# bcaitech1/p4-fr-sorry-math-but-love-you

Hardware: NVIDIA B200
Metric: EfficientSATRN greedy-decode images/sec (higher is better)
Workload: dtype bf16

## Files before the change

p4-fr-sorry-math-but-love-you_b200/csrc/common.cuh:

```cuda
#pragma once
#include <cuda_runtime.h>
#include <cuda_bf16.h>
#include <cuda_fp16.h>
#include <stdint.h>

#if defined(__CUDA_ARCH__) && (__CUDA_ARCH__ < 1000)
#error "frx is written for sm_100a (B200) only"
#endif

namespace frx {

enum Act : int { ACT_NONE = 0, ACT_RELU = 1, ACT_SILU = 2, ACT_SIGMOID = 3, ACT_GELU = 4 };

__device__ __forceinline__ float act_apply(float v, int act) {
  switch (act) {
    case ACT_RELU: return fmaxf(v, 0.f);
    case ACT_SILU: return v / (1.f + expf(-v));
    case ACT_SIGMOID: return 1.f / (1.f + expf(-v));
    case ACT_GELU: return 0.5f * v * (1.f + erff(v * 0.70710678118654752440f));
    default: return v;
  }
}

struct SmemOptIn {
  size_t bytes[64] = {};
  template <class Kernel>
  cudaError_t ensure(Kernel kernel, size_t smem, bool always = false) {
    int dev = 0;
    cudaGetDevice(&dev);
    dev &= 63;
    if ((!always && smem <= 48 * 1024) || (bytes[dev] != 0 && smem <= bytes[dev])) return cudaSuccess;
    cudaError_t e = cudaFuncSetAttribute(kernel, cudaFuncAttributeMaxDynamicSharedMemorySize, (int)smem);
    if (e == cudaSuccess) bytes[dev] = smem;
    return e;
  }
};

#ifndef FRX_ENC_FP16
#define FRX_ENC_FP16 1
#endif
#if FRX_ENC_FP16
typedef __half eh_t;
typedef __half2 eh2_t;
#define FRX_EH_PTX "f16"
__device__ __forceinline__ uint32_t eh2_pack(float lo, float hi) {
  uint32_t r;
  asm("cvt.rn.satfinite.f16x2.f32 %0, %1, %2;\n" : "=r"(r) : "f"(hi), "f"(lo));
  return r;
}
__device__ __forceinline__ eh_t eh_from_float(float f) {
  const uint32_t r = eh2_pack(f, 0.f);
  return __ushort_as_half((unsigned short)(r & 0xffffu));
}
__device__ __forceinline__ float eh_to_float(eh_t v) { return __half2float(v); }
__device__ __forceinline__ float2 eh2_unpack(uint32_t w) { return __half22float2(*reinterpret_cast<const __half2*>(&w)); }
#else
typedef __nv_bfloat16 eh_t;
typedef __nv_bfloat162 eh2_t;
#define FRX_EH_PTX "bf16"
__device__ __forceinline__ uint32_t eh2_pack(float lo, float hi) {
  __nv_bfloat162 t = __floats2bfloat162_rn(lo, hi);
  return *reinterpret_cast<uint32_t*>(&t);
}
__device__ __forceinline__ eh_t eh_from_float(float f) { return __float2bfloat16_rn(f); }
__device__ __forceinline__ float eh_to_float(eh_t v) { return __bfloat162float(v); }
__device__ __forceinline__ float2 eh2_unpack(uint32_t w) { return make_float2(__uint_as_float(w << 16), __uint_as_float(w & 0xffff0000u)); }
#endif

__device__ __forceinline__ float warp_sum(float v) {
#pragma unroll
  for (int o = 16; o > 0; o >>= 1) v += __shfl_xor_sync(0xffffffffu, v, o);
  return v;
}
__device__ __forceinline__ float warp_max(float v) {
#pragma unroll
  for (int o = 16; o > 0; o >>= 1) v = fmaxf(v, __shfl_xor_sync(0xffffffffu, v, o));
  return v;
}

struct GemmP {
  const float* A;
  const float* W;
  float* C;
  int M, N, K;
  int lda, ldc;
  int conv;
  int H, Wd, Cin, OH, OW, KH, KW, stride, pad_t, pad_l;
  const float* gate;
  int rows_per_img;
  const float* scale;
  const float* shift;
  int act;
  const float* res;
  int ldr;
  float* ws;
  long long ws_floats;
  int splitk, k_chunk;
};

struct DwP {
  const float* in;
  const float* w;
  const float* scale;
  const float* shift;
  float* out;
  int B, H, Wd, C, OH, OW, stride, pad_t, pad_l, act;
};

struct Seg {
  int n_begin, n_end;
  float* dst;
  long long row_stride;
  long long slot_stride;
};

struct DecGemmP {
  const float* A;
  const float* Wt;
  const float* bias;
// ... 108 lines not shown
```

p4-fr-sorry-math-but-love-you_b200/csrc/kernels_bf16.cu:

```cuda
#include <cuda_fp16.h>

#include "common.cuh"
#include "kernels.h"

#ifndef FRX_DW_ACC32
#define FRX_DW_ACC32 2
#endif

namespace frx {

namespace {
__device__ __forceinline__ void unpack8(const uint4& u, float (&f)[8]) {
  const uint32_t w[4] = {u.x, u.y, u.z, u.w};
#pragma unroll
  for (int i = 0; i < 4; ++i) {
    const float2 t = eh2_unpack(w[i]);
    f[2 * i] = t.x;
    f[2 * i + 1] = t.y;
  }
}
__device__ __forceinline__ uint4 pack8(const float (&f)[8]) {
  uint32_t w[4];
#pragma unroll
  for (int i = 0; i < 4; ++i) w[i] = eh2_pack(f[2 * i], f[2 * i + 1]);
  return make_uint4(w[0], w[1], w[2], w[3]);
}
}

__global__ void __launch_bounds__(256) stem_conv_bf16_kernel(const float* __restrict__ in, const float* __restrict__ w,
                                                             const float* __restrict__ scale, const float* __restrict__ shift,
                                                             eh_t* __restrict__ out, int B, int Cin, int H, int W,
                                                             int OH, int OW, int Cout) {
  extern __shared__ float ws[];
  for (int i = threadIdx.x; i < Cout * Cin * 9; i += blockDim.x) ws[i] = w[i];
  float* ssc = ws + Cout * Cin * 9;
  float* ssh = ssc + Cout;
  for (int i = threadIdx.x; i < Cout; i += blockDim.x) { ssc[i] = scale[i]; ssh[i] = shift[i]; }
  __syncthreads();
  const int C8 = Cout / 8;
  long long total = (long long)B * OH * OW * C8;
  long long idx = (long long)blockIdx.x * blockDim.x + threadIdx.x;
  if (idx >= total) return;
  const int co0 = (int)(idx % C8) * 8;
  long long pix = idx / C8;
  const int ow = (int)(pix % OW), oh = (int)((pix / OW) % OH), n = (int)(pix / ((long long)OW * OH));
  float acc[8];
#pragma unroll
  for (int j = 0; j < 8; ++j) acc[j] = 0.f;
  for (int ci = 0; ci < Cin; ++ci) {
    const float* ip = in + (((long long)n * Cin + ci) * H + oh * 2) * W + ow * 2;
    float x[9];
#pragma unroll
    for (int kh = 0; kh < 3; ++kh)
#pragma unroll
      for (int kw = 0; kw < 3; ++kw) x[kh * 3 + kw] = __ldg(ip + kh * W + kw);
#pragma unroll
    for (int j = 0; j < 8; ++j) {
      const float* wp = ws + ((co0 + j) * Cin + ci) * 9;
#pragma unroll
      for (int t = 0; t < 9; ++t) acc[j] = fmaf(x[t], wp[t], acc[j]);
    }
  }
  float o[8];
#pragma unroll
  for (int j = 0; j < 8; ++j) o[j] = act_apply(acc[j] * ssc[co0 + j] + ssh[co0 + j], ACT_SILU);
  *reinterpret_cast<uint4*>(out + pix * Cout + co0) = pack8(o);
}

template <int COUT>
__global__ void __launch_bounds__(128) stem_conv_px_bf16_kernel(const float* __restrict__ in, const float* __restrict__ w,
                                                                const float* __restrict__ scale, const float* __restrict__ shift,
                                                                eh_t* __restrict__ out, int B, int Cin, int H, int W,
                                                                int OH, int OW) {
  extern __shared__ __align__(16) float ws[];
  const int taps = Cin * 9;
  for (int i = threadIdx.x; i < COUT * taps; i += blockDim.x) {
    const int co = i / taps, r = i - co * taps;
    ws[r * COUT + co] = w[i];
  }
  float* ssc = ws + COUT * taps;
  float* ssh = ssc + COUT;
  uint4* stage = reinterpret_cast<uint4*>(ws + ((COUT * taps + 2 * COUT + 3) & ~3));
  for (int i = threadIdx.x; i < COUT; i += blockDim.x) { ssc[i] = scale[i]; ssh[i] = shift[i]; }
  __syncthreads();
  const long long npix = (long long)B * OH * OW, pix0 = (long long)blockIdx.x * blockDim.x;
  const long long pix = min(pix0 + threadIdx.x, npix - 1);
  const int ow = (int)(pix % OW), oh = (int)((pix / OW) % OH), n = (int)(pix / ((long long)OW * OH));
  float acc[COUT];
#pragma unroll
  for (int j = 0; j < COUT; ++j) acc[j] = 0.f;
  for (int ci = 0; ci < Cin; ++ci) {
    const float* ip = in + (((long long)n * Cin + ci) * H + oh * 2) * W + ow * 2;
    float x[9];
#pragma unroll
    for (int kh = 0; kh < 3; ++kh)
#pragma unroll
      for (int kw = 0; kw < 3; ++kw) x[kh * 3 + kw] = __ldg(ip + kh * W + kw);
#pragma unroll
    for (int t = 0; t < 9; ++t) {
      const float4* wp = reinterpret_cast<const float4*>(ws + (ci * 9 + t) * COUT);
#pragma unroll
      for (int j = 0; j < COUT / 4; ++j) {
        const float4 wv = wp[j];
        acc[4 * j] = fmaf(x[t], wv.x, acc[4 * j]);
        acc[4 * j + 1] = fmaf(x[t], wv.y, acc[4 * j + 1]);
        acc[4 * j + 2] = fmaf(x[t], wv.z, acc[4 * j + 2]);
        acc[4 * j + 3] = fmaf(x[t], wv.w, acc[4 * j + 3]);
      }
    }
  }
#pragma unroll
  for (int g = 0; g < COUT / 8; ++g) {
    float o[8];
#pragma unroll
    for (int j = 0; j < 8; ++j) o[j] = act_apply(acc[g * 8 + j] * ssc[g * 8 + j] + ssh[g * 8 + j], ACT_SILU);
    stage[threadIdx.x * (COUT / 8) + g] = pack8(o);
  }
  __syncthreads();
  const long long cta_vecs = min((long long)blockDim.x, npix - pix0) * (COUT / 8);
  uint4* op = reinterpret_cast<uint4*>(out + pix0 * COUT);
  for (int i = threadIdx.x; i < cta_vecs; i += blockDim.x) op[i] = stage[i];
}

void launch_stem_conv_bf16(const float* in, const float* w, const float* scale, const float* shift,
                           eh_t* out, int B, int Cin, int H, int W, int OH, int OW, int Cout, cudaStream_t st) {
  if (Cout == 24) {
    const long long pixels = (long long)B * OH * OW;
    const int smem24 = ((24 * Cin * 9 + 2 * 24 + 3) & ~3) * sizeof(float) + 128 * 3 * 16;
    stem_conv_px_bf16_kernel<24><<<(unsigned)((pixels + 127) / 128), 128, smem24, st>>>(in, w, scale, shift, out, B, Cin, H, W, OH, OW);
    return;
  }
  long long total = (long long)B * OH * OW * (Cout / 8);
  int smem = (Cout * Cin * 9 + 2 * Cout) * sizeof(float);
  stem_conv_bf16_kernel<<<(unsigned)((total + 255) / 256), 256, smem, st>>>(in, w, scale, shift, out, B, Cin, H, W, OH, OW, Cout);
}

__global__ void __launch_bounds__(256) dwconv3x3_bf16_kernel(const eh_t* __restrict__ in, const float* __restrict__ w,
                                                             const float* __restrict__ scale, const float* __restrict__ shift,
                                                             eh_t* __restrict__ out, int B, int H, int W, int C, int OH,
                                                             int OW, int stride, int pad_t, int pad_l, int act) {
  const int C8 = C >> 3;
  long long total = (long long)B * OH * OW * C8;
  long long idx = (long long)blockIdx.x * blockDim.x + threadIdx.x;
  if (idx >= total) return;
  const int c = (int)(idx % C8) * 8;
  long long pix = idx / C8;
  const int ow = (int)(pix % OW), oh = (int)((pix / OW) % OH), n = (int)(pix / ((long long)OW * OH));
  float acc[8];
#pragma unroll
  for (int j = 0; j < 8; ++j) acc[j] = 0.f;
#pragma unroll
  for (int kh = 0; kh < 3; ++kh) {
    const int ih = oh * stride - pad_t + kh;
    if (ih < 0 || ih >= H) continue;
#pragma unroll
    for (int kw = 0; kw < 3; ++kw) {
      const int iw = ow * stride - pad_l + kw;
      if (iw < 0 || iw >= W) continue;
      float x[8];
      unpack8(__ldg(reinterpret_cast<const uint4*>(in + (((long long)n * H + ih) * W + iw) * C + c)), x);
      const float4 w0 = __ldg(reinterpret_cast<const float4*>(w + (kh * 3 + kw) * C + c));
      const float4 w1 = __ldg(reinterpret_cast<const float4*>(w + (kh * 3 + kw) * C + c + 4));
      acc[0] = fmaf(x[0], w0.x, acc[0]); acc[1] = fmaf(x[1], w0.y, acc[1]);
      acc[2] = fmaf(x[2], w0.z, acc[2]); acc[3] = fmaf(x[3], w0.w, acc[3]);
      acc[4] = fmaf(x[4], w1.x, acc[4]); acc[5] = fmaf(x[5], w1.y, acc[5]);
      acc[6] = fmaf(x[6], w1.z, acc[6]); acc[7] = fmaf(x[7], w1.w, acc[7]);
    }
  }
  float o[8];
#pragma unroll
  for (int j = 0; j < 8; ++j) o[j] = act_apply(acc[j] * __ldg(scale + c + j) + __ldg(shift + c + j), act);
  *reinterpret_cast<uint4*>(out + pix * C + c) = pack8(o);
}

void launch_dwconv_bf16(const eh_t* in, const float* w, const float* scale, const float* shift,
                        eh_t* out, int B, int H, int W, int C, int OH, int OW, int stride, int pad_t,
                        int pad_l, int act, cudaStream_t st) {
  long long total = (long long)B * OH * OW * (C / 8);
  dwconv3x3_bf16_kernel<<<(unsigned)((total + 255) / 256), 256, 0, st>>>(in, w, scale, shift, out, B, H, W, C, OH, OW,
                                                                        stride, pad_t, pad_l, act);
}

__global__ void __launch_bounds__(256) se_scale_bf16_kernel(eh_t* __restrict__ x, const float* __restrict__ w1,
                                                            const float* __restrict__ b1, const float* __restrict__ w2,
                                                            const float* __restrict__ b2, int HW, int C, int R) {
  extern __shared__ float sm[];
  float* mean = sm;
  float* red = sm + C;
  float* gate = red + R;
  const int n = blockIdx.x;
  eh_t* xp = x + (long long)n * HW * C;
  const float inv = 1.f / (float)HW;
  for (int c8 = threadIdx.x; c8 < C / 8; c8 += blockDim.x) {
    float s[8];
#pragma unroll
    for (int j = 0; j < 8; ++j) s[j] = 0.f;
    for (int q = 0; q < HW; ++q) {
      float v[8];
      unpack8(*reinterpret_cast<const uint4*>(xp + (long long)q * C + c8 * 8), v);
#pragma unroll
      for (int j = 0; j < 8; ++j) s[j] += v[j];
    }
#pragma unroll
    for (int j = 0; j < 8; ++j) mean[c8 * 8 + j] = s[j] * inv;
  }
  __syncthreads();
  const int warp = threadIdx.x >> 5, lane = threadIdx.x & 31;
  for (int r = warp; r < R; r += 8) {
    float s = 0.f;
    for (int c = lane; c < C; c += 32) s = fmaf(__ldg(w1 + (long long)r * C + c), mean[c], s);
    s = warp_sum(s);
    if (lane == 0) red[r] = act_apply(s + __ldg(b1 + r), ACT_SILU);
  }
  __syncthreads();
  for (int c = threadIdx.x; c < C; c += blockDim.x) {
    float s = __ldg(b2 + c);
    const float* wr = w2 + (long long)c * R;
    for (int r = 0; r < R; ++r) s = fmaf(__ldg(wr + r), red[r], s);
    gate[c] = 1.f / (1.f + expf(-s));
  }
  __syncthreads();
  for (int i = threadIdx.x; i < HW * (C / 8); i += blockDim.x) {
    const int c8 = i % (C / 8);
    uint4* ptr = reinterpret_cast<uint4*>(xp + (long long)(i / (C / 8)) * C + c8 * 8);
    float v[8];
    unpack8(*ptr, v);
#pragma unroll
    for (int j = 0; j < 8; ++j) v[j] *= gate[c8 * 8 + j];
    *ptr = pack8(v);
  }
}

void launch_se_scale_bf16(eh_t* x, const float* w1, const float* b1, const float* w2, const float* b2,
                          int B, int HW, int C, int R, cudaStream_t st) {
  se_scale_bf16_kernel<<<B, 256, (2 * C + R) * sizeof(float), st>>>(x, w1, b1, w2, b2, HW, C, R);
}


__global__ void __launch_bounds__(256) dwconv_se_mean_kernel(const eh_t* __restrict__ in, const float* __restrict__ w,
                                                             const float* __restrict__ scale, const float* __restrict__ shift,
                                                             eh_t* __restrict__ out, float* __restrict__ mean,
                                                             int H, int W, int C, int OH, int OW, int stride, int pad_t,
                                                             int pad_l, const float* __restrict__ se_w1,
                                                             const float* __restrict__ se_w2, int se_floats) {
  extern __shared__ __align__(16) unsigned char dw_smem[];
  {
    const long long line = ((long long)(blockIdx.y * gridDim.x + blockIdx.x) * blockDim.x + threadIdx.x) * 32;
    if (line < se_floats) {
      asm volatile("prefetch.global.L2 [%0];\n" ::"l"(se_w1 + line));
      asm volatile("prefetch.global.L2 [%0];\n" ::"l"(se_w2 + line));
    }
  }
  uint4* tile = reinterpret_cast<uint4*>(dw_smem);
  float (*red)[64 + 1] = reinterpret_cast<float (*)[64 + 1]>(dw_smem + (size_t)H * W * 8 * 16);
  float* wsm = reinterpret_cast<float*>(dw_smem + (size_t)H * W * 8 * 16 + 32 * 65 * sizeof(float));
  const int n = blockIdx.x, c0 = blockIdx.y * 64;
  const int cg = threadIdx.x & 7, pl = threadIdx.x >> 3;
  const int c = c0 + cg * 8;
  const bool c_ok = c < C;
  const eh_t* ip = in + (long long)n * H * W * C;
  for (int i = threadIdx.x; i < H * W * 8; i += 256) {
    const int px = i >> 3, g = i & 7;
    tile[i] = (c0 + g * 8 < C) ? __ldg(reinterpret_cast<const uint4*>(ip + (long long)px * C + c0 + g * 8)) : make_uint4(0u, 0u, 0u, 0u);
  }
  float sum[8];
#pragma unroll
  for (int j = 0; j < 8; ++j) sum[j] = 0.f;
  for (int i = threadIdx.x; i < 11 * 64; i += 256) {
    const int t = i >> 6, cc = c0 + (i & 63);
    const float* src = t < 9 ? w + t * C : (t == 9 ? scale : shift);
    wsm[i] = cc < C ? __ldg(src + cc) : 0.f;
  }
  __syncthreads();
  auto ld8s = [&](int t, float (&dst)[8]) {
    const float4 a = *reinterpret_cast<const float4*>(wsm + t * 64 + cg * 8);
    const float4 b4 = *reinterpret_cast<const float4*>(wsm + t * 64 + cg * 8 + 4);
    dst[0] = a.x; dst[1] = a.y; dst[2] = a.z; dst[3] = a.w; dst[4] = b4.x; dst[5] = b4.y; dst[6] = b4.z; dst[7] = b4.w;
  };
  float sc[8], sh[8];
  ld8s(9, sc);
  ld8s(10, sh);
  eh_t* op = out + (long long)n * OH * OW * C;
  if (c_ok) {
    for (int px = pl; px < OH * OW; px += 32) {
      const int oh = px / OW, ow = px - oh * OW;
      float acc[8];
#pragma unroll
      for (int j = 0; j < 8; ++j) acc[j] = 0.f;
#pragma unroll
      for (int kh = 0; kh < 3; ++kh) {
        const int ih = oh * stride - pad_t + kh;
#pragma unroll
        for (int kw = 0; kw < 3; ++kw) {
          const int iw = ow * stride - pad_l + kw;
          if (ih >= 0 && ih < H && iw >= 0 && iw < W) {
            float x[8], wv[8];
            unpack8(tile[(ih * W + iw) * 8 + cg], x);
            ld8s(kh * 3 + kw, wv);
#pragma unroll
            for (int j = 0; j < 8; ++j) acc[j] = fmaf(x[j], wv[j], acc[j]);
          }
        }
      }
      float o[8];
#pragma unroll
      for (int j = 0; j < 8; ++j) {
        const float v = fmaf(acc[j], sc[j], sh[j]);
        o[j] = __fdividef(v, 1.f + __expf(-v));
      }
      const uint4 packed = pack8(o);
      *reinterpret_cast<uint4*>(op + (long long)px * C + c) = packed;
      float back[8];
      unpack8(packed, back);
#pragma unroll
      for (int j = 0; j < 8; ++j) sum[j] += back[j];
    }
  }
#pragma unroll
  for (int j = 0; j < 8; ++j) red[pl][cg * 8 + j] = sum[j];
  __syncthreads();
  if (threadIdx.x < 64 && c0 + threadIdx.x < C) {
    float s = 0.f;
#pragma unroll
    for (int i = 0; i < 32; ++i) s += red[i][threadIdx.x];
    mean[(long long)n * C + c0 + threadIdx.x] = s / (float)(OH * OW);
  }
}

template <int CH>
__global__ void __launch_bounds__(CH * 4) dwconv4_se_mean_kernel(const eh_t* __restrict__ in, const float* __restrict__ w,
                                                                 const float* __restrict__ scale, const float* __restrict__ shift,
                                                                 eh_t* __restrict__ out, float* __restrict__ mean,
                                                                 int H, int W, int C, int OH, int OW, int stride, int pad_t,
                                                                 int pad_l, const float* __restrict__ se_w1,
                                                                 const float* __restrict__ se_w2, int se_floats) {
  constexpr int NT = CH * 4, G8 = CH / 8, G4 = CH / 4;
  extern __shared__ __align__(16) unsigned char dw_smem[];
  {
    const long long line = ((long long)(blockIdx.y * gridDim.x + blockIdx.x) * NT + threadIdx.x) * 32;
    if (line < se_floats) {
      asm volatile("prefetch.global.L2 [%0];\n" ::"l"(se_w1 + line));
      asm volatile("prefetch.global.L2 [%0];\n" ::"l"(se_w2 + line));
    }
  }
  uint4* tile = reinterpret_cast<uint4*>(dw_smem);
  float (*red)[CH + 1] = reinterpret_cast<float (*)[CH + 1]>(dw_smem + (size_t)H * W * G8 * 16);
  const int n = blockIdx.x, c0 = blockIdx.y * CH;
  const eh_t* ip = in + (long long)n * H * W * C;
  for (int i = threadIdx.x; i < H * W * G8; i += NT) {
    const int px = i / G8, g = i - px * G8;
    uint4 v = make_uint4(0u, 0u, 0u, 0u);
    if (c0 + g * 8 < C) {
#if FRX_ENC_FP16
      v = __ldg(reinterpret_cast<const uint4*>(ip + (long long)px * C + c0 + g * 8));
#else
      float x[8];
      unpack8(__ldg(reinterpret_cast<const uint4*>(ip + (long long)px * C + c0 + g * 8)), x);
      const __half2 h0 = __floats2half2_rn(x[0], x[1]), h1 = __floats2half2_rn(x[2], x[3]);
      const __half2 h2 = __floats2half2_rn(x[4], x[5]), h3 = __floats2half2_rn(x[6], x[7]);
      v = make_uint4(*reinterpret_cast<const uint32_t*>(&h0), *reinterpret_cast<const uint32_t*>(&h1),
                     *reinterpret_cast<const uint32_t*>(&h2), *reinterpret_cast<const uint32_t*>(&h3));
#endif
    }
    tile[i] = v;
  }
  const int cg = threadIdx.x % G4, pl = threadIdx.x / G4;
  const int c = c0 + cg * 4;
  const bool c_ok = c < C;
#if FRX_DW_ACC32
  float4 wt[9], sc, sh;
#if FRX_DW_ACC32 == 2
  __half2 wh[9][2];
#endif
  {
    const float4 z = make_float4(0.f, 0.f, 0.f, 0.f);
#pragma unroll
    for (int t = 0; t < 9; ++t) wt[t] = c_ok ? __ldg(reinterpret_cast<const float4*>(w + t * C + c)) : z;
#if FRX_DW_ACC32 == 2
#pragma unroll
    for (int t = 0; t < 9; ++t) { wh[t][0] = __floats2half2_rn(wt[t].x, wt[t].y); wh[t][1] = __floats2half2_rn(wt[t].z, wt[t].w); }
#endif
    sc = c_ok ? __ldg(reinterpret_cast<const float4*>(scale + c)) : z;
    sh = c_ok ? __ldg(reinterpret_cast<const float4*>(shift + c)) : z;
  }
  __syncthreads();
  const uint2* tile2 = reinterpret_cast<const uint2*>(tile);
  float sum[4] = {0.f, 0.f, 0.f, 0.f};
  eh_t* op = out + (long long)n * OH * OW * C;
  if (c_ok) {
    for (int px = pl; px < OH * OW; px += 16) {
      const int oh = px / OW, ow = px - oh * OW;
      float4 acc = make_float4(0.f, 0.f, 0.f, 0.f);
#pragma unroll
      for (int kh = 0; kh < 3; ++kh) {
        const int ih = oh * stride - pad_t + kh;
#if FRX_DW_ACC32 == 2
        __half2 r0 = __floats2half2_rn(0.f, 0.f), r1 = r0;
#pragma unroll
        for (int kw = 0; kw < 3; ++kw) {
          const int iw = ow * stride - pad_l + kw;
          if (ih >= 0 && ih < H && iw >= 0 && iw < W) {
            const uint2 u = tile2[(ih * W + iw) * G4 + cg];
            r0 = __hfma2(*reinterpret_cast<const __half2*>(&u.x), wh[kh * 3 + kw][0], r0);
            r1 = __hfma2(*reinterpret_cast<const __half2*>(&u.y), wh[kh * 3 + kw][1], r1);
          }
        }
        const float2 a = __half22float2(r0), b = __half22float2(r1);
        acc.x += a.x; acc.y += a.y; acc.z += b.x; acc.w += b.y;
#else
#pragma unroll
        for (int kw = 0; kw < 3; ++kw) {
          const int iw = ow * stride - pad_l + kw;
          if (ih >= 0 && ih < H && iw >= 0 && iw < W) {
            const uint2 u = tile2[(ih * W + iw) * G4 + cg];
            const float2 a = __half22float2(*reinterpret_cast<const __half2*>(&u.x)), b = __half22float2(*reinterpret_cast<const __half2*>(&u.y));
            const float4 ww = wt[kh * 3 + kw];
            acc.x = fmaf(a.x, ww.x, acc.x); acc.y = fmaf(a.y, ww.y, acc.y); acc.z = fmaf(b.x, ww.z, acc.z); acc.w = fmaf(b.y, ww.w, acc.w);
          }
        }
#endif
      }
      float2 f0 = make_float2(fmaf(acc.x, sc.x, sh.x), fmaf(acc.y, sc.y, sh.y)), f1 = make_float2(fmaf(acc.z, sc.z, sh.z), fmaf(acc.w, sc.w, sh.w));
      f0.x = __fdividef(f0.x, 1.f + __expf(-f0.x)); f0.y = __fdividef(f0.y, 1.f + __expf(-f0.y));
      f1.x = __fdividef(f1.x, 1.f + __expf(-f1.x)); f1.y = __fdividef(f1.y, 1.f + __expf(-f1.y));
#else
  __half2 wt[9][2], sc[2], sh[2];
  {
    const float4 z = make_float4(0.f, 0.f, 0.f, 0.f);
#pragma unroll
    for (int t = 0; t < 9; ++t) {
      const float4 f = c_ok ? __ldg(reinterpret_cast<const float4*>(w + t * C + c)) : z;
      wt[t][0] = __floats2half2_rn(f.x, f.y); wt[t][1] = __floats2half2_rn(f.z, f.w);
    }
    const float4 a = c_ok ? __ldg(reinterpret_cast<const float4*>(scale + c)) : z;
    const float4 d = c_ok ? __ldg(reinterpret_cast<const float4*>(shift + c)) : z;
    sc[0] = __floats2half2_rn(a.x, a.y); sc[1] = __floats2half2_rn(a.z, a.w);
    sh[0] = __floats2half2_rn(d.x, d.y); sh[1] = __floats2half2_rn(d.z, d.w);
  }
  const __half2 half_ = __floats2half2_rn(0.5f, 0.5f);
  __syncthreads();
  const uint2* tile2 = reinterpret_cast<const uint2*>(tile);
  float sum[4] = {0.f, 0.f, 0.f, 0.f};
  eh_t* op = out + (long long)n * OH * OW * C;
  if (c_ok) {
    for (int px = pl; px < OH * OW; px += 16) {
      const int oh = px / OW, ow = px - oh * OW;
      __half2 acc0 = __floats2half2_rn(0.f, 0.f), acc1 = acc0;
#pragma unroll
      for (int kh = 0; kh < 3; ++kh) {
        const int ih = oh * stride - pad_t + kh;
#pragma unroll
        for (int kw = 0; kw < 3; ++kw) {
          const int iw = ow * stride - pad_l + kw;
          if (ih >= 0 && ih < H && iw >= 0 && iw < W) {
            const uint2 u = tile2[(ih * W + iw) * G4 + cg];
            acc0 = __hfma2(*reinterpret_cast<const __half2*>(&u.x), wt[kh * 3 + kw][0], acc0);
            acc1 = __hfma2(*reinterpret_cast<const __half2*>(&u.y), wt[kh * 3 + kw][1], acc1);
          }
        }
      }
      const __half2 v0 = __hfma2(acc0, sc[0], sh[0]), v1 = __hfma2(acc1, sc[1], sh[1]);
      const __half2 o0 = __hmul2(v0, __hfma2(h2tanh_approx(__hmul2(v0, half_)), half_, half_));
      const __half2 o1 = __hmul2(v1, __hfma2(h2tanh_approx(__hmul2(v1, half_)), half_, half_));
      const float2 f0 = __half22float2(o0), f1 = __half22float2(o1);
#endif
      uint2 packed;
      packed.x = eh2_pack(f0.x, f0.y);
      packed.y = eh2_pack(f1.x, f1.y);
      *reinterpret_cast<uint2*>(op + (long long)px * C + c) = packed;
      const float2 b0 = eh2_unpack(packed.x), b1 = eh2_unpack(packed.y);
      sum[0] += b0.x; sum[1] += b0.y; sum[2] += b1.x; sum[3] += b1.y;
    }
  }
#pragma unroll
  for (int j = 0; j < 4; ++j) red[pl][cg * 4 + j] = sum[j];
  __syncthreads();
  if (threadIdx.x < CH && c0 + threadIdx.x < C) {
    float s2 = 0.f;
#pragma unroll
    for (int i = 0; i < 16; ++i) s2 += red[i][threadIdx.x];
    mean[(long long)n * C + c0 + threadIdx.x] = s2 / (float)(OH * OW);
  }
}

constexpr int SE_IMGS = 4;
constexpr int SE_ROWS = 4;
__global__ void __launch_bounds__(512, 1) se_fc_kernel(const float* __restrict__ mean, const float* __restrict__ w1,
                                                       const float* __restrict__ b1, const float* __restrict__ w2,
                                                       const float* __restrict__ b2, float* __restrict__ gate, int B, int C,
                                                       int R) {
  extern __shared__ float sm[];
  float* mv = sm;
  float* red = sm + SE_IMGS * C;
  const int n0 = blockIdx.x * SE_IMGS;
  for (int i = threadIdx.x; i < SE_IMGS * C; i += blockDim.x) {
    const int im = i / C;
    mv[i] = n0 + im < B ? mean[(long long)n0 * C + i] : 0.f;
  }
  __syncthreads();
  const int warp = threadIdx.x >> 5, lane = threadIdx.x & 31;
  const int nwarps = blockDim.x >> 5;
  for (int r0 = warp * SE_ROWS; r0 < R; r0 += nwarps * SE_ROWS) {
    float s[SE_ROWS][SE_IMGS];
#pragma unroll
    for (int j = 0; j < SE_ROWS; ++j)
#pragma unroll
      for (int im = 0; im < SE_IMGS; ++im) s[j][im] = 0.f;
#pragma unroll 3
    for (int c4 = lane; c4 < C / 4; c4 += 32) {
      float4 wv[SE_ROWS], m4[SE_IMGS];
#pragma unroll
      for (int j = 0; j < SE_ROWS; ++j)
        wv[j] = r0 + j < R ? __ldg(reinterpret_cast<const float4*>(w1 + (long long)(r0 + j) * C) + c4) : make_float4(0.f, 0.f, 0.f, 0.f);
#pragma unroll
      for (int im = 0; im < SE_IMGS; ++im) m4[im] = *reinterpret_cast<const float4*>(mv + im * C + c4 * 4);
#pragma unroll
      for (int j = 0; j < SE_ROWS; ++j)
#pragma unroll
        for (int im = 0; im < SE_IMGS; ++im)
          s[j][im] = fmaf(wv[j].x, m4[im].x, fmaf(wv[j].y, m4[im].y, fmaf(wv[j].z, m4[im].z, fmaf(wv[j].w, m4[im].w, s[j][im]))));
    }
#pragma unroll
    for (int j = 0; j < SE_ROWS; ++j)
#pragma unroll
      for (int im = 0; im < SE_IMGS; ++im) {
        const float t = warp_sum(s[j][im]);
        if (lane == 0 && r0 + j < R) red[im * R + r0 + j] = act_apply(t + __ldg(b1 + r0 + j), ACT_SILU);
      }
  }
  __syncthreads();
  for (int c = blockIdx.y * blockDim.x + threadIdx.x; c < C; c += gridDim.y * blockDim.x) {
    float s[SE_IMGS];
    const float bb = __ldg(b2 + c);
#pragma unroll
    for (int im = 0; im < SE_IMGS; ++im) s[im] = bb;
#pragma unroll 32
    for (int r = 0; r < R; ++r) {
      const float wv = __ldg(w2 + (long long)r * C + c);
#pragma unroll
      for (int im = 0; im < SE_IMGS; ++im) s[im] = fmaf(wv, red[im * R + r], s[im]);
    }
#pragma unroll
    for (int im = 0; im < SE_IMGS; ++im)
      if (n0 + im < B) gate[(long long)(n0 + im) * C + c] = 1.f / (1.f + expf(-s[im]));
  }
}

__global__ void __launch_bounds__(256) se_apply_kernel(eh_t* __restrict__ x, const float* __restrict__ gate,
                                                       long long total8, int HW, int C) {
  long long i = (long long)blockIdx.x * blockDim.x + threadIdx.x;
  if (i >= total8) return;
  const int C8 = C >> 3;
  const int c = (int)(i % C8) * 8;
  const long long n = i / ((long long)C8 * HW);
  uint4* ptr = reinterpret_cast<uint4*>(x) + i;
  float v[8];
  unpack8(*ptr, v);
  const float4 g0 = __ldg(reinterpret_cast<const float4*>(gate + n * C + c));
  const float4 g1 = __ldg(reinterpret_cast<const float4*>(gate + n * C + c + 4));
  v[0] *= g0.x; v[1] *= g0.y; v[2] *= g0.z; v[3] *= g0.w;
  v[4] *= g1.x; v[5] *= g1.y; v[6] *= g1.z; v[7] *= g1.w;
  *ptr = pack8(v);
}

void launch_mbconv_dw_se_bf16(const eh_t* in, const float* w, const float* scale, const float* shift,
                              eh_t* out, float* mean, float* gate, const float* w1, const float* b1,
                              const float* w2, const float* b2, int B, int H, int W, int C, int OH, int OW, int stride,
                              int pad_t, int pad_l, int R, cudaStream_t st) {
  dim3 g(B, (C + 63) / 64);
  const size_t smem = (size_t)H * W * 8 * 16 + 32 * 65 * sizeof(float) + 11 * 64 * sizeof(float);
  static SmemOptIn opt;
  opt.ensure(dwconv_se_mean_kernel, smem);
  if (C % 8 == 0) {
    constexpr int CH = 32;
    const size_t sm4 = (size_t)H * W * (CH / 8) * 16 + 16 * (CH + 1) * sizeof(float);
    static SmemOptIn opt4;
    opt4.ensure(dwconv4_se_mean_kernel<CH>, sm4);
    dwconv4_se_mean_kernel<CH><<<dim3(B, (C + CH - 1) / CH), CH * 4, sm4, st>>>(in, w, scale, shift, out, mean, H, W, C, OH, OW,
                                                                             stride, pad_t, pad_l, w1, w2, R * C);
  } else {
    dwconv_se_mean_kernel<<<g, 256, smem, st>>>(in, w, scale, shift, out, mean, H, W, C, OH, OW, stride, pad_t, pad_l, w1, w2, R * C);
  }
  se_fc_kernel<<<dim3((B + SE_IMGS - 1) / SE_IMGS, 2), 512, SE_IMGS * (C + R) * sizeof(float), st>>>(mean, w1, b1, w2, b2, gate, B, C, R);
  long long total8 = (long long)B * OH * OW * (C / 8);
  se_apply_kernel<<<(unsigned)((total8 + 255) / 256), 256, 0, st>>>(out, gate, total8, OH * OW, C);
}

__device__ __forceinline__ uint32_t pack2(float lo, float hi) {
  return eh2_pack(lo, hi);
}
__device__ __forceinline__ void mma16816(float (&c)[4], const uint32_t (&a)[4], uint32_t b0, uint32_t b1) {
  asm("mma.sync.aligned.m16n8k16.row.col.f32." FRX_EH_PTX "." FRX_EH_PTX ".f32 {%0,%1,%2,%3}, {%4,%5,%6,%7}, {%8,%9}, {%0,%1,%2,%3};\n"
      : "+f"(c[0]), "+f"(c[1]), "+f"(c[2]), "+f"(c[3])
      : "r"(a[0]), "r"(a[1]), "r"(a[2]), "r"(a[3]), "r"(b0), "r"(b1));
}

template <int S>
__global__ void __launch_bounds__(S * 2) enc_attn_mma_kernel(const float* __restrict__ qkv,
                                                             eh_t* __restrict__ out,
                                                             int D, int heads, float inv_temp) {
  constexpr int HD = 64, NT = S / 8;
  const int b = blockIdx.x / heads, hh = blockIdx.x % heads;
  const int warp = threadIdx.x >> 5, lane = threadIdx.x & 31, gid = lane >> 2, tig = lane & 3;
  const int ld = 3 * D;
  const float* qb = qkv + (long long)b * S * ld + hh * HD;
  const int i0 = warp * 16;
  float sacc[NT][4];
#pragma unroll
  for (int nt = 0; nt < NT; ++nt)
#pragma unroll
    for (int e = 0; e < 4; ++e) sacc[nt][e] = 0.f;
#pragma unroll
  for (int ks = 0; ks < 4; ++ks) {
    const float* q0 = qb + (long long)(i0 + gid) * ld + 16 * ks + 2 * tig;
    const float* q1 = q0 + 8 * ld;
    const float2 a00 = __ldg(reinterpret_cast<const float2*>(q0)), a10 = __ldg(reinterpret_cast<const float2*>(q1));
    const float2 a01 = __ldg(reinterpret_cast<const float2*>(q0 + 8)), a11 = __ldg(reinterpret_cast<const float2*>(q1 + 8));
    const uint32_t a[4] = {pack2(a00.x, a00.y), pack2(a10.x, a10.y), pack2(a01.x, a01.y), pack2(a11.x, a11.y)};
#pragma unroll
    for (int nt = 0; nt < NT; ++nt) {
      const float* kp = qb + D + (long long)(8 * nt + gid) * ld + 16 * ks + 2 * tig;
      const float2 k0 = __ldg(reinterpret_cast<const float2*>(kp)), k1 = __ldg(reinterpret_cast<const float2*>(kp + 8));
      mma16816(sacc[nt], a, pack2(k0.x, k0.y), pack2(k1.x, k1.y));
    }
  }
  float mx0 = -INFINITY, mx1 = -INFINITY;
#pragma unroll
  for (int nt = 0; nt < NT; ++nt) {
#pragma unroll
    for (int e = 0; e < 4; ++e) sacc[nt][e] *= inv_temp;
    mx0 = fmaxf(mx0, fmaxf(sacc[nt][0], sacc[nt][1]));
    mx1 = fmaxf(mx1, fmaxf(sacc[nt][2], sacc[nt][3]));
  }
  mx0 = fmaxf(mx0, __shfl_xor_sync(0xffffffffu, mx0, 1)); mx0 = fmaxf(mx0, __shfl_xor_sync(0xffffffffu, mx0, 2));
  mx1 = fmaxf(mx1, __shfl_xor_sync(0xffffffffu, mx1, 1)); mx1 = fmaxf(mx1, __shfl_xor_sync(0xffffffffu, mx1, 2));
  float sum0 = 0.f, sum1 = 0.f;
#pragma unroll
  for (int nt = 0; nt < NT; ++nt) {
    sacc[nt][0] = __expf(sacc[nt][0] - mx0); sacc[nt][1] = __expf(sacc[nt][1] - mx0);
    sacc[nt][2] = __expf(sacc[nt][2] - mx1); sacc[nt][3] = __expf(sacc[nt][3] - mx1);
    sum0 += sacc[nt][0] + sacc[nt][1];
    sum1 += sacc[nt][2] + sacc[nt][3];
  }
  sum0 += __shfl_xor_sync(0xffffffffu, sum0, 1); sum0 += __shfl_xor_sync(0xffffffffu, sum0, 2);
  sum1 += __shfl_xor_sync(0xffffffffu, sum1, 1); sum1 += __shfl_xor_sync(0xffffffffu, sum1, 2);
  float oacc[8][4];
#pragma unroll
  for (int n = 0; n < 8; ++n)
#pragma unroll
    for (int e = 0; e < 4; ++e) oacc[n][e] = 0.f;
#pragma unroll
  for (int kk = 0; kk < S / 16; ++kk) {
    const uint32_t a[4] = {pack2(sacc[2 * kk][0], sacc[2 * kk][1]), pack2(sacc[2 * kk][2], sacc[2 * kk][3]),
                           pack2(sacc[2 * kk + 1][0], sacc[2 * kk + 1][1]), pack2(sacc[2 * kk + 1][2], sacc[2 * kk + 1][3])};
    const float* vp = qb + 2 * D + (long long)(16 * kk + 2 * tig) * ld + gid;
#pragma unroll
    for (int n = 0; n < 8; ++n) {
      const float v00 = __ldg(vp + 8 * n), v01 = __ldg(vp + ld + 8 * n);
      const float v10 = __ldg(vp + 8 * ld + 8 * n), v11 = __ldg(vp + 9 * ld + 8 * n);
      mma16816(oacc[n], a, pack2(v00, v01), pack2(v10, v11));
    }
  }
  const float r0 = __fdividef(1.f, sum0), r1 = __fdividef(1.f, sum1);
  eh_t* o0 = out + ((long long)b * S + i0 + gid) * D + hh * HD + 2 * tig;
  eh_t* o1 = o0 + (long long)8 * D;
#pragma unroll
  for (int n = 0; n < 8; ++n) {
    *reinterpret_cast<uint32_t*>(o0 + 8 * n) = pack2(oacc[n][0] * r0, oacc[n][1] * r0);
    *reinterpret_cast<uint32_t*>(o1 + 8 * n) = pack2(oacc[n][2] * r1, oacc[n][3] * r1);
  }
}

bool launch_enc_attn_mma_bf16(const float* qkv, eh_t* out, int B, int S, int D, int heads, cudaStream_t st) {
  if (D / heads != 64 || D % heads != 0) return false;
  const float inv_temp = 1.f / sqrtf((float)D);
  if (S == 32) enc_attn_mma_kernel<32><<<B * heads, 64, 0, st>>>(qkv, out, D, heads, inv_temp);
  else if (S == 128) enc_attn_mma_kernel<128><<<B * heads, 256, 0, st>>>(qkv, out, D, heads, inv_temp);
  else return false;
  return true;
}

constexpr int C24 = 24, C24_TH = 8, C24_TW = 32, C24_KS = 14;

__global__ void __launch_bounds__(256) conv3x3_c24_mma_kernel(const eh_t* __restrict__ in, const uint2* __restrict__ wfrag,
                                                              const float* __restrict__ scale, const float* __restrict__ shift,
                                                              eh_t* __restrict__ out, int H, int W, int add_res) {
  constexpr int PW = C24_TW + 2, PH = C24_TH + 2;
  __shared__ __align__(16) eh_t halo[PH * PW * C24];
  __shared__ uint2 wsm[C24_KS * 3 * 32];
  const int tiles_x = (W + C24_TW - 1) / C24_TW, tiles_y = (H + C24_TH - 1) / C24_TH;
  const int n = blockIdx.x / (tiles_x * tiles_y), t = blockIdx.x % (tiles_x * tiles_y);
  const int y0 = (t / tiles_x) * C24_TH, x0 = (t % tiles_x) * C24_TW;
  const eh_t* ip = in + (long long)n * H * W * C24;
  for (int i = threadIdx.x; i < PH * PW * 3; i += 256) {
    const int pix = i / 3, ch = i - pix * 3;
    const int py = pix / PW, px = pix - py * PW;
    const int y = y0 + py - 1, x = x0 + px - 1;
    uint4 v = make_uint4(0u, 0u, 0u, 0u);
    if (y >= 0 && y < H && x >= 0 && x < W) v = __ldg(reinterpret_cast<const uint4*>(ip + ((long long)y * W + x) * C24) + ch);
    reinterpret_cast<uint4*>(halo)[i] = v;
  }
  for (int i = threadIdx.x; i < C24_KS * 3 * 32; i += 256) wsm[i] = __ldg(wfrag + i);
  __syncthreads();
  const int warp = threadIdx.x >> 5, lane = threadIdx.x & 31, gid = lane >> 2, tig = lane & 3;
  float acc[2][3][4];
#pragma unroll
  for (int mt = 0; mt < 2; ++mt)
#pragma unroll
    for (int nt = 0; nt < 3; ++nt)
#pragma unroll
      for (int e = 0; e < 4; ++e) acc[mt][nt][e] = 0.f;
  const uint32_t* hw = reinterpret_cast<const uint32_t*>(halo);
#pragma unroll
  for (int s = 0; s < C24_KS; ++s) {
    const int klo = 16 * s, khi = 16 * s + 8;
    const int tap_lo = klo / C24, ch_lo = klo % C24, tap_hi = khi / C24, ch_hi = khi % C24;
    uint32_t a[2][4];
#pragma unroll
    for (int mt = 0; mt < 2; ++mt) {
      const int px = mt * 16 + gid;
      const int p_lo = ((warp + tap_lo / 3) * PW + px + tap_lo % 3) * 12 + (ch_lo >> 1) + tig;
      a[mt][0] = hw[p_lo];
      a[mt][1] = hw[p_lo + 8 * 12];
      if (tap_hi < 9) {
        const int p_hi = ((warp + tap_hi / 3) * PW + px + tap_hi % 3) * 12 + (ch_hi >> 1) + tig;
        a[mt][2] = hw[p_hi];
        a[mt][3] = hw[p_hi + 8 * 12];
      } else {
        a[mt][2] = 0u; a[mt][3] = 0u;
      }
    }
#pragma unroll
    for (int nt = 0; nt < 3; ++nt) {
      const uint2 b = wsm[(s * 3 + nt) * 32 + lane];
      mma16816(acc[0][nt], a[0], b.x, b.y);
      mma16816(acc[1][nt], a[1], b.x, b.y);
    }
  }
  const int y = y0 + warp;
  if (y >= H) return;
  eh_t* op = out + ((long long)n * H + y) * W * C24;
#pragma unroll
  for (int nt = 0; nt < 3; ++nt) {
    const int ch = nt * 8 + 2 * tig;
    const float s0 = __ldg(scale + ch), s1 = __ldg(scale + ch + 1), h0 = __ldg(shift + ch), h1 = __ldg(shift + ch + 1);
#pragma unroll
    for (int mt = 0; mt < 2; ++mt)
#pragma unroll
      for (int hr = 0; hr < 2; ++hr) {
        const int px = mt * 16 + gid + hr * 8, x = x0 + px;
        if (x >= W) continue;
        float v0 = fmaf(acc[mt][nt][2 * hr], s0, h0), v1 = fmaf(acc[mt][nt][2 * hr + 1], s1, h1);
        v0 = __fdividef(v0, 1.f + __expf(-v0));
        v1 = __fdividef(v1, 1.f + __expf(-v1));
        if (add_res) {
          const uint32_t r = hw[((warp + 1) * PW + px + 1) * 12 + (ch >> 1)];
          const float2 rf = eh2_unpack(r);
          v0 += rf.x;
          v1 += rf.y;
        }
        *reinterpret_cast<uint32_t*>(op + (long long)x * C24 + ch) = pack2(v0, v1);
      }
  }
}

void launch_conv3x3_c24_bf16(const eh_t* in, const void* wfrag, const float* scale, const float* shift,
                             eh_t* out, int B, int H, int W, int add_res, cudaStream_t st) {
  const int tiles = ((W + C24_TW - 1) / C24_TW) * ((H + C24_TH - 1) / C24_TH);
  conv3x3_c24_mma_kernel<<<B * tiles, 256, 0, st>>>(in, reinterpret_cast<const uint2*>(wfrag), scale, shift, out, H, W, add_res);
}

__global__ void __launch_bounds__(256) lite_conv0_pool_bf16_kernel(const float* __restrict__ in, const float* __restrict__ w,
                                                                   const float* __restrict__ scale, const float* __restrict__ shift,
                                                                   eh_t* __restrict__ out, int B, int Cin, int H, int W, int Cout) {
  extern __shared__ float ws0[];
  for (int i = threadIdx.x; i < Cout * Cin * 9; i += blockDim.x) ws0[i] = w[i];
  float* ssc = ws0 + Cout * Cin * 9;
  float* ssh = ssc + Cout;
  for (int i = threadIdx.x; i < Cout; i += blockDim.x) { ssc[i] = scale[i]; ssh[i] = shift[i]; }
  __syncthreads();
  const int OH = H / 2, OW = W / 2, C8 = Cout / 8;
  const long long total = (long long)B * OH * OW * C8;
  const long long idx = (long long)blockIdx.x * blockDim.x + threadIdx.x;
  if (idx >= total) return;
  const int co0 = (int)(idx % C8) * 8;
  const long long pix = idx / C8;
  const int ow = (int)(pix % OW), oh = (int)((pix / OW) % OH), n = (int)(pix / ((long long)OW * OH));
  float acc[4][8];
#pragma unroll
  for (int q = 0; q < 4; ++q)
#pragma unroll
    for (int j = 0; j < 8; ++j) acc[q][j] = 0.f;
  for (int ci = 0; ci < Cin; ++ci) {
    float x[4][4];
#pragma unroll
    for (int a = 0; a < 4; ++a)
#pragma unroll
      for (int b = 0; b < 4; ++b) {
        const int ih = 2 * oh - 1 + a, iw = 2 * ow - 1 + b;
        x[a][b] = (ih >= 0 && ih < H && iw >= 0 && iw < W) ? __ldg(in + (((long long)n * Cin + ci) * H + ih) * W + iw) : 0.f;
      }
#pragma unroll
    for (int j = 0; j < 8; ++j) {
      const float* wp = ws0 + ((co0 + j) * Cin + ci) * 9;
#pragma unroll
      for (int kh = 0; kh < 3; ++kh)
#pragma unroll
        for (int kw = 0; kw < 3; ++kw) {
          const float wv = wp[kh * 3 + kw];
          acc[0][j] = fmaf(x[kh][kw], wv, acc[0][j]);
          acc[1][j] = fmaf(x[kh][kw + 1], wv, acc[1][j]);
          acc[2][j] = fmaf(x[kh + 1][kw], wv, acc[2][j]);
          acc[3][j] = fmaf(x[kh + 1][kw + 1], wv, acc[3][j]);
        }
    }
  }
  float o[8];
#pragma unroll
  for (int j = 0; j < 8; ++j) {
    const float s = ssc[co0 + j], t = ssh[co0 + j];
    const float m = fmaxf(fmaxf(fmaf(acc[0][j], s, t), fmaf(acc[1][j], s, t)), fmaxf(fmaf(acc[2][j], s, t), fmaf(acc[3][j], s, t)));
    o[j] = fmaxf(m, 0.f);
  }
  *reinterpret_cast<uint4*>(out + pix * Cout + co0) = pack8(o);
}

template <int KS, int Cout>
__global__ void __launch_bounds__(256) lite_conv0_pool_mma_kernel(const float* __restrict__ in, const float* __restrict__ w,
                                                                  const float* __restrict__ scale, const float* __restrict__ shift,
                                                                  eh_t* __restrict__ out, int B, int Cin, int H, int W) {
  constexpr int NT = Cout / 8;
  const int lane = threadIdx.x & 31, gid = lane >> 2, tig = lane & 3;
  const int OH = H / 2, OW = W / 2, K = 9 * Cin;
  const long long tiles = (long long)B * OH * (OW / 4);
  const long long tile = (long long)blockIdx.x * 8 + (threadIdx.x >> 5);
  if (tile >= tiles) return;
  uint32_t bf[KS][NT][2];
#pragma unroll
  for (int ks = 0; ks < KS; ++ks)
#pragma unroll
    for (int nt = 0; nt < NT; ++nt)
#pragma unroll
      for (int h2 = 0; h2 < 2; ++h2) {
        const int k = 16 * ks + 8 * h2 + 2 * tig, n = 8 * nt + gid;
        const float lo = k < K ? __ldg(w + (long long)n * K + k) : 0.f, hi = k + 1 < K ? __ldg(w + (long long)n * K + k + 1) : 0.f;
        bf[ks][nt][h2] = pack2(lo, hi);
      }
  const int owq = (int)(tile % (OW / 4));
  const long long t2 = tile / (OW / 4);
  const int oh = (int)(t2 % OH), n = (int)(t2 / OH);
  const int pp = gid & 3, pos0 = gid >> 2;
  const int ow = owq * 4 + pp;
// ... 85 lines not shown
```

p4-fr-sorry-math-but-love-you_b200/csrc/kernels_f32.cu:

```cuda
#include "common.cuh"
#include "kernels.h"

namespace frx {

__global__ void __launch_bounds__(256) stem_conv_kernel(const float* __restrict__ in,
                                                        const float* __restrict__ w,
                                                        const float* __restrict__ scale,
                                                        const float* __restrict__ shift,
                                                        float* __restrict__ out, int B, int Cin, int H,
                                                        int W, int OH, int OW, int Cout, int stride, int pad,
                                                        int act) {
  extern __shared__ float ws[];
  for (int i = threadIdx.x; i < Cout * Cin * 9; i += blockDim.x) ws[i] = w[i];
  float* ssc = ws + Cout * Cin * 9;
  float* ssh = ssc + Cout;
  for (int i = threadIdx.x; i < Cout; i += blockDim.x) { ssc[i] = scale[i]; ssh[i] = shift[i]; }
  __syncthreads();
  long long total = (long long)B * OH * OW * Cout;
  long long idx = (long long)blockIdx.x * blockDim.x + threadIdx.x;
  if (idx >= total) return;
  int co = (int)(idx % Cout);
  long long pix = idx / Cout;
  int ow = (int)(pix % OW);
  int oh = (int)((pix / OW) % OH);
// ... 288 lines not shown

__global__ void __launch_bounds__(256) se_gate_f32_kernel(const float* __restrict__ x,
                                                          const float* __restrict__ w1,
                                                          const float* __restrict__ b1,
                                                          const float* __restrict__ w2,
                                                          const float* __restrict__ b2,
                                                          float* __restrict__ gate,
                                                          int HW, int C, int R) {
  extern __shared__ float sm[];
  float* mean = sm;
  float* red = sm + C;
  const int n = blockIdx.x;
  const float* xp = x + (long long)n * HW * C;
  const float inv = 1.f / (float)HW;
  for (int c = threadIdx.x; c < C; c += blockDim.x) {
    float s = 0.f;
    for (int q = 0; q < HW; ++q) s += __ldg(xp + (long long)q * C + c);
    mean[c] = s * inv;
  }
  __syncthreads();
  const int warp = threadIdx.x >> 5, lane = threadIdx.x & 31;
  for (int r = warp; r < R; r += 8) {
    float s = 0.f;
    for (int c = lane; c < C; c += 32) s = fmaf(__ldg(w1 + (long long)r * C + c), mean[c], s);
    s = warp_sum(s);
    if (lane == 0) red[r] = act_apply(s + __ldg(b1 + r), ACT_SILU);
  }
  __syncthreads();
  for (int c = threadIdx.x; c < C; c += blockDim.x) {
    float s = __ldg(b2 + c);
    const float* wr = w2 + (long long)c * R;
    for (int r = 0; r < R; ++r) s = fmaf(__ldg(wr + r), red[r], s);
    gate[(long long)n * C + c] = 1.f / (1.f + expf(-s));
  }
}

void launch_se_gate_f32(const float* x, const float* w1, const float* b1, const float* w2,
                        const float* b2, float* gate, int B, int HW, int C, int R, cudaStream_t st) {
  se_gate_f32_kernel<<<B, 256, (C + R) * sizeof(float), st>>>(x, w1, b1, w2, b2, gate, HW, C, R);
}

__global__ void __launch_bounds__(256) maxpool2_f32_kernel(const float* __restrict__ in,
                                                           float* __restrict__ out, int B, int H, int W,
                                                           int C) {
  const int OH = H / 2, OW = W / 2, C4 = C / 4;
  long long total = (long long)B * OH * OW * C4;
  long long idx = (long long)blockIdx.x * blockDim.x + threadIdx.x;
  if (idx >= total) return;
  int c = (int)(idx % C4) * 4;
  long long pix = idx / C4;
  int ow = (int)(pix % OW);
  int oh = (int)((pix / OW) % OH);
  int n = (int)(pix / ((long long)OW * OH));
  const float* base = in + (((long long)n * H + oh * 2) * W + ow * 2) * C + c;
  float4 a = __ldg(reinterpret_cast<const float4*>(base));
  float4 b = __ldg(reinterpret_cast<const float4*>(base + C));
  float4 d = __ldg(reinterpret_cast<const float4*>(base + (long long)W * C));
  float4 e = __ldg(reinterpret_cast<const float4*>(base + (long long)W * C + C));
  float4 o;
  o.x = fmaxf(fmaxf(a.x, b.x), fmaxf(d.x, e.x));
  o.y = fmaxf(fmaxf(a.y, b.y), fmaxf(d.y, e.y));
  o.z = fmaxf(fmaxf(a.z, b.z), fmaxf(d.z, e.z));
  o.w = fmaxf(fmaxf(a.w, b.w), fmaxf(d.w, e.w));
  *reinterpret_cast<float4*>(out + (((long long)n * OH + oh) * OW + ow) * C + c) = o;
}

void launch_maxpool2_f32(const float* in, float* out, int B, int H, int W, int C, cudaStream_t st) {
  long long total = (long long)B * (H / 2) * (W / 2) * (C / 4);
  maxpool2_f32_kernel<<<(unsigned)((total + 255) / 256), 256, 0, st>>>(in, out, B, H, W, C);
}

__global__ void __launch_bounds__(1024) pe2d_f32_kernel(const float* __restrict__ x,
                                                       const float* __restrict__ w0,
                                                       const float* __restrict__ b0,
                                                       const float* __restrict__ w1,
                                                       const float* __restrict__ b1,
                                                       const float* __restrict__ peh,
                                                       const float* __restrict__ pew,
                                                       float* __restrict__ out, int h, int w, int C) {
  extern __shared__ float sm[];
  float* mean = sm;
  float* hid = sm + C;
  float* g = hid + C / 2;
  const int S = h * w, n = blockIdx.x;
  const float* xp = x + (long long)n * S * C;
  const float inv = 1.f / (float)S;
  for (int c = threadIdx.x; c < C; c += blockDim.x) {
    float s = 0.f;
    for (int q = 0; q < S; ++q) s += __ldg(xp + (long long)q * C + c);
    mean[c] = s * inv;
  }
  __syncthreads();
  const int warp = threadIdx.x >> 5, lane = threadIdx.x & 31;
  const int nwarps = blockDim.x >> 5;
  for (int r = warp; r < C / 2; r += nwarps) {
    float s = 0.f;
    for (int c = lane; c < C; c += 32) s = fmaf(__ldg(w0 + (long long)r * C + c), mean[c], s);
    s = warp_sum(s);
    if (lane == 0) hid[r] = fmaxf(s + __ldg(b0 + r), 0.f);
  }
  __syncthreads();
  for (int r = warp; r < 2 * C; r += nwarps) {
    float s = 0.f;
    for (int c = lane; c < C / 2; c += 32) s = fmaf(__ldg(w1 + (long long)r * (C / 2) + c), hid[c], s);
    s = warp_sum(s);
    if (lane == 0) g[r] = 1.f / (1.f + expf(-(s + __ldg(b1 + r))));
  }
  __syncthreads();
  float* op = out + (long long)n * S * C;
  for (int i = threadIdx.x; i < S * C; i += blockDim.x) {
    int c = i % C, q = i / C;
    int row = q / w, col = q % w;
    float pos = g[c] * __ldg(peh + row * C + c) + g[C + c] * __ldg(pew + col * C + c);
    op[i] = pos + __ldg(xp + i);
  }
}

void launch_pe2d_f32(const float* x, const float* w0, const float* b0, const float* w1, const float* b1,
                     const float* peh, const float* pew, float* out, int B, int h, int w, int C,
                     cudaStream_t st) {
  int smem = (C + C / 2 + 2 * C) * sizeof(float);
  pe2d_f32_kernel<<<B, 1024, smem, st>>>(x, w0, b0, w1, b1, peh, pew, out, h, w, C);
}

__device__ __forceinline__ void store_as(float* p, float v) { *p = v; }
__device__ __forceinline__ void store_as(eh_t* p, float v) { *p = eh_from_float(v); }

template <typename OutT>
__global__ void __launch_bounds__(256) layernorm_f32_generic_kernel(const float* __restrict__ x,
                                                            const float* __restrict__ res,
                                                            const float* __restrict__ gamma,
                                                            const float* __restrict__ beta,
                                                            OutT* __restrict__ out, int M, int C,
                                                            int scramble_S) {
  const int warp = threadIdx.x >> 5, lane = threadIdx.x & 31;
  const int m = blockIdx.x * 8 + warp;
  if (m >= M) return;
  const float* xp = x + (long long)m * C;
  const float* rp = res ? res + (long long)m * C : nullptr;
  float v[64];
  const int per = C / 32;
  float s = 0.f;
#pragma unroll
  for (int i = 0; i < 64; ++i) {
    if (i < per) {
      float t = __ldg(xp + i * 32 + lane);
      if (rp) t += __ldg(rp + i * 32 + lane);
      v[i] = t;
      s += t;
    }
  }
  const float mean = warp_sum(s) / (float)C;
  float q = 0.f;
#pragma unroll
  for (int i = 0; i < 64; ++i)
    if (i < per) { float d = v[i] - mean; q = fmaf(d, d, q); }
  const float rstd = rsqrtf(warp_sum(q) / (float)C + 1e-5f);
#pragma unroll
  for (int i = 0; i < 64; ++i) {
    if (i < per) {
      int ch = i * 32 + lane;
      float o = (v[i] - mean) * rstd * __ldg(gamma + ch) + __ldg(beta + ch);
      if (scramble_S > 0) {
        int b = m / scramble_S, qd = m % scramble_S;
        long long f = (long long)qd * C + ch;
        int pp = (int)(f % scramble_S), cc = (int)(f / scramble_S);
        store_as(out + ((long long)b * scramble_S + pp) * C + cc, o);
      } else {
        store_as(out + (long long)m * C + ch, o);
      }
    }
  }
}

template <typename OutT, int PER>
__global__ void __launch_bounds__(256) layernorm_f32_kernel(const float* __restrict__ x,
                                                            const float* __restrict__ res,
                                                            const float* __restrict__ gamma,
                                                            const float* __restrict__ beta,
                                                            OutT* __restrict__ out, int M, int C,
                                                            int scramble_S) {
  const int warp = threadIdx.x >> 5, lane = threadIdx.x & 31;
  const int m = blockIdx.x * 8 + warp;
  if (m >= M) return;
  const float* xp = x + (long long)m * C;
  const float* rp = res ? res + (long long)m * C : nullptr;
  float v[PER];
  float s = 0.f;
#pragma unroll
  for (int i = 0; i < PER; ++i) {
    float t = __ldg(xp + i * 32 + lane);
    if (rp) t += __ldg(rp + i * 32 + lane);
    v[i] = t;
    s += t;
  }
  const float mean = warp_sum(s) / (float)C;
  float q = 0.f;
#pragma unroll
  for (int i = 0; i < PER; ++i) { float d = v[i] - mean; q = fmaf(d, d, q); }
  const float rstd = rsqrtf(warp_sum(q) / (float)C + 1e-5f);
#pragma unroll
  for (int i = 0; i < PER; ++i) {
    int ch = i * 32 + lane;
    float o = (v[i] - mean) * rstd * __ldg(gamma + ch) + __ldg(beta + ch);
    if (scramble_S > 0) {
      int b = m / scramble_S, qd = m % scramble_S;
      long long f = (long long)qd * C + ch;
      int pp = (int)(f % scramble_S), cc = (int)(f / scramble_S);
      store_as(out + ((long long)b * scramble_S + pp) * C + cc, o);
    } else {
      store_as(out + (long long)m * C + ch, o);
    }
  }
}

template <typename OutT>
static void layernorm_launch(const float* x, const float* res, const float* gamma, const float* beta, OutT* out, int M, int C,
                             int scramble_S, cudaStream_t st) {
  const dim3 g((M + 7) / 8);
  const int per = C / 32;
  if (per <= 4 && per * 32 == C) {
    if (per == 4) layernorm_f32_kernel<OutT, 4><<<g, 256, 0, st>>>(x, res, gamma, beta, out, M, C, scramble_S);
    else if (per == 2) layernorm_f32_kernel<OutT, 2><<<g, 256, 0, st>>>(x, res, gamma, beta, out, M, C, scramble_S);
    else if (per == 1) layernorm_f32_kernel<OutT, 1><<<g, 256, 0, st>>>(x, res, gamma, beta, out, M, C, scramble_S);
    else layernorm_f32_kernel<OutT, 3><<<g, 256, 0, st>>>(x, res, gamma, beta, out, M, C, scramble_S);
  } else if (per == 8) layernorm_f32_kernel<OutT, 8><<<g, 256, 0, st>>>(x, res, gamma, beta, out, M, C, scramble_S);
  else if (per == 16) layernorm_f32_kernel<OutT, 16><<<g, 256, 0, st>>>(x, res, gamma, beta, out, M, C, scramble_S);
  else if (per == 32) layernorm_f32_kernel<OutT, 32><<<g, 256, 0, st>>>(x, res, gamma, beta, out, M, C, scramble_S);
  else if (per == 64) layernorm_f32_kernel<OutT, 64><<<g, 256, 0, st>>>(x, res, gamma, beta, out, M, C, scramble_S);
  else layernorm_f32_generic_kernel<OutT><<<g, 256, 0, st>>>(x, res, gamma, beta, out, M, C, scramble_S);
}

void launch_layernorm_f32(const float* x, const float* res, const float* gamma, const float* beta,
                          float* out, int M, int C, int scramble_S, cudaStream_t st) {
  layernorm_launch<float>(x, res, gamma, beta, out, M, C, scramble_S, st);
}

__global__ void __launch_bounds__(256) layernorm_scramble_bf16_kernel(const float* __restrict__ x, const float* __restrict__ res,
                                                                      const float* __restrict__ gamma,
                                                                      const float* __restrict__ beta,
                                                                      eh_t* __restrict__ out, int S, int C) {
  extern __shared__ eh_t ln_tile[];
  const int b = blockIdx.x, warp = threadIdx.x >> 5, lane = threadIdx.x & 31;
  const int per = C / 32, LD = S + 2;
  for (int qd = warp; qd < S; qd += 8) {
    const float* xp = x + ((long long)b * S + qd) * C;
    const float* rp = res ? res + ((long long)b * S + qd) * C : nullptr;
    float v[16];
    float s = 0.f;
#pragma unroll
    for (int i = 0; i < 16; ++i)
      if (i < per) {
        float t = __ldg(xp + i * 32 + lane);
        if (rp) t += __ldg(rp + i * 32 + lane);
        v[i] = t;
        s += t;
      }
    const float mean = warp_sum(s) / (float)C;
    float q = 0.f;
#pragma unroll
    for (int i = 0; i < 16; ++i)
      if (i < per) { float d = v[i] - mean; q = fmaf(d, d, q); }
    const float rstd = rsqrtf(warp_sum(q) / (float)C + 1e-5f);
#pragma unroll
    for (int i = 0; i < 16; ++i)
      if (i < per) {
        const int ch = i * 32 + lane;
        const int f = qd * C + ch;
        ln_tile[(f / S) * LD + f % S] = eh_from_float((v[i] - mean) * rstd * __ldg(gamma + ch) + __ldg(beta + ch));
      }
  }
  __syncthreads();
  eh_t* op = out + (long long)b * S * C;
  for (int g = threadIdx.x; g < S * C; g += 256) {
    const int pp = g / C, cc = g - pp * C;
    op[g] = ln_tile[cc * LD + pp];
  }
}

void launch_layernorm_bf16out(const float* x, const float* res, const float* gamma, const float* beta,
                              eh_t* out, int M, int C, int scramble_S, cudaStream_t st) {
  const size_t scr_smem = (size_t)C * (scramble_S + 2) * 2;
  static SmemOptIn scr_opt;
  if (scramble_S > 0 && C <= 512 && C % 32 == 0 && M % scramble_S == 0 && scr_smem <= 160 * 1024 &&
      scr_opt.ensure(layernorm_scramble_bf16_kernel, scr_smem) == cudaSuccess) {
    layernorm_scramble_bf16_kernel<<<M / scramble_S, 256, scr_smem, st>>>(x, res, gamma, beta, out,
                                                                                               scramble_S, C);
    return;
  }
  layernorm_launch<eh_t>(x, res, gamma, beta, out, M, C, scramble_S, st);
}

template <typename OutT>
__global__ void __launch_bounds__(128) enc_attn_f32_kernel(const float* __restrict__ qkv,
                                                           OutT* __restrict__ out,
                                                           int S, int D, int heads, float temperature) {
  extern __shared__ float sm[];
  const int HD = D / heads;
  const int LDS_ = HD + 1;
  float* Q = sm;
  float* K = Q + S * LDS_;
  float* V = K + S * LDS_;
  float* P = V + S * LDS_;
  const int b = blockIdx.x / heads, hh = blockIdx.x % heads;
  const float* base = qkv + (long long)b * S * 3 * D + hh * HD;
  for (int i = threadIdx.x; i < S * HD; i += blockDim.x) {
    int r = i / HD, c = i % HD;
    const float* rp = base + (long long)r * 3 * D + c;
    Q[r * LDS_ + c] = __ldg(rp);
    K[r * LDS_ + c] = __ldg(rp + D);
    V[r * LDS_ + c] = __ldg(rp + 2 * D);
  }
  __syncthreads();
  const int warp = threadIdx.x >> 5, lane = threadIdx.x & 31;
  float* Pw = P + warp * S;
  for (int i = warp; i < S; i += 4) {
    float mx = -INFINITY;
    for (int j = lane; j < S; j += 32) {
      float s = 0.f;
      for (int c = 0; c < HD; ++c) s = fmaf(Q[i * LDS_ + c], K[j * LDS_ + c], s);
      s = s / temperature;
      Pw[j] = s;
      mx = fmaxf(mx, s);
    }
    mx = warp_max(mx);
    float sum = 0.f;
    for (int j = lane; j < S; j += 32) {
      float e = expf(Pw[j] - mx);
      Pw[j] = e;
      sum += e;
    }
    sum = warp_sum(sum);
    __syncwarp();
    for (int c = lane; c < HD; c += 32) {
      float acc = 0.f;
      for (int j = 0; j < S; ++j) acc = fmaf(Pw[j] / sum, V[j * LDS_ + c], acc);
      store_as(out + ((long long)b * S + i) * D + hh * HD + c, acc);
    }
    __syncwarp();
  }
}

template <typename OutT>
static void enc_attn_launch(const float* qkv, OutT* out, int B, int S, int D, int heads, cudaStream_t st) {
  int HD = D / heads;
  size_t smem = (size_t)(3 * S * (HD + 1) + 4 * S) * sizeof(float);
  static SmemOptIn opt;
  opt.ensure(enc_attn_f32_kernel<OutT>, smem);
  enc_attn_f32_kernel<OutT><<<B * heads, 128, smem, st>>>(qkv, out, S, D, heads, sqrtf((float)D));
}
void launch_enc_attn_f32(const float* qkv, float* out, int B, int S, int D, int heads, cudaStream_t st) {
  enc_attn_launch<float>(qkv, out, B, S, D, heads, st);
}
void launch_enc_attn_bf16out(const float* qkv, eh_t* out, int B, int S, int D, int heads, cudaStream_t st) {
  enc_attn_launch<eh_t>(qkv, out, B, S, D, heads, st);
}

constexpr int DG_BM = 32, DG_BN = 32, DG_KC = 512;

__global__ void __launch_bounds__(256) dec_gemm_f32_kernel(const DecGemmP p) {
  extern __shared__ __align__(16) float smem_raw[];
  float (*As)[DG_KC + 4] = reinterpret_cast<float (*)[DG_KC + 4]>(smem_raw);
  float (*red)[DG_BM][DG_BN] = reinterpret_cast<float (*)[DG_BM][DG_BN]>(smem_raw);
  static_assert(8 * DG_BM * DG_BN <= DG_BM * (DG_KC + 4), "partials must fit in the A buffer");
  const int tid = threadIdx.x, warp = tid >> 5, lane = tid & 31;
  const int m0 = blockIdx.x * DG_BM, n0 = blockIdx.y * DG_BN;
  const int n = n0 + lane;
  const bool n_ok = n < p.N;
  float acc[DG_BM];
#pragma unroll
// ... 319 lines not shown
```

p4-fr-sorry-math-but-love-you_b200/csrc/kernels_tc.cu:

```cuda
#include <cuda.h>
#include <cuda_fp16.h>
#include <cudaTypedefs.h>

#include <cstdio>
#include <cstdlib>

#include "common.cuh"
#include "kernels.h"

namespace frx {

namespace {

constexpr int TC_BM = 128;
constexpr int TC_BK = 64;
constexpr int TC_STAGES = 3;
constexpr int TC_A_BYTES = TC_BM * TC_BK * 2;

__device__ __forceinline__ uint32_t smem_u32(const void* p) { return (uint32_t)__cvta_generic_to_shared(p); }

__device__ __forceinline__ void cp_async16(uint32_t dst, const void* src, uint32_t src_bytes) {
  asm volatile("cp.async.cg.shared.global [%0], [%1], 16, %2;\n" ::"r"(dst), "l"(src), "r"(src_bytes) : "memory");
}
__device__ __forceinline__ void cp_async_commit() { asm volatile("cp.async.commit_group;\n" ::: "memory"); }
// ... 175 lines not shown
              if (nb + i < p.N) v[i] += __ldg(rp + i);
          }
        } else {
          const eh_t* rp = reinterpret_cast<const eh_t*>(p.res) + (size_t)m * p.ldr + nb;
          if (full) {
            const uint4 r0 = __ldg(reinterpret_cast<const uint4*>(rp)), r1 = __ldg(reinterpret_cast<const uint4*>(rp + 8));
            const uint32_t rw[8] = {r0.x, r0.y, r0.z, r0.w, r1.x, r1.y, r1.z, r1.w};
#pragma unroll
            for (int i = 0; i < 8; ++i) {
              const float2 rf = eh2_unpack(rw[i]);
              v[2 * i] += rf.x;
              v[2 * i + 1] += rf.y;
            }
          } else {
            for (int i = 0; i < 16; ++i)
              if (nb + i < p.N) v[i] += eh_to_float(rp[i]);
          }
        }
      }
      if (p.out_f32) {
        float* cp = reinterpret_cast<float*>(p.C) + (size_t)m * p.ldc + nb;
        if (full && (p.ldc & 7) == 0 && (reinterpret_cast<uintptr_t>(p.C) & 31) == 0) {
#pragma unroll
          for (int i = 0; i < 16; i += 8)
            asm volatile("st.global.v8.f32 [%0], {%1, %2, %3, %4, %5, %6, %7, %8};\n" ::"l"(cp + i), "f"(v[i]), "f"(v[i + 1]),
                         "f"(v[i + 2]), "f"(v[i + 3]), "f"(v[i + 4]), "f"(v[i + 5]), "f"(v[i + 6]), "f"(v[i + 7]) : "memory");
        } else if (full && (p.ldc & 3) == 0) {
#pragma unroll
          for (int i = 0; i < 16; i += 4) *reinterpret_cast<float4*>(cp + i) = make_float4(v[i], v[i + 1], v[i + 2], v[i + 3]);
        } else {
          for (int i = 0; i < 16; ++i)
            if (nb + i < p.N) cp[i] = v[i];
        }
      } else {
        eh_t* cp = reinterpret_cast<eh_t*>(p.C) + (size_t)m * p.ldc + nb;
        if (full && (p.ldc & 7) == 0) {
          uint32_t w[8];
#pragma unroll
          for (int i = 0; i < 8; ++i) w[i] = eh2_pack(v[2 * i], v[2 * i + 1]);
          if ((p.ldc & 15) == 0 && (reinterpret_cast<uintptr_t>(p.C) & 31) == 0) {
            asm volatile("st.global.v8.b32 [%0], {%1, %2, %3, %4, %5, %6, %7, %8};\n" ::"l"(cp), "r"(w[0]), "r"(w[1]), "r"(w[2]),
                         "r"(w[3]), "r"(w[4]), "r"(w[5]), "r"(w[6]), "r"(w[7]) : "memory");
          } else {
            *reinterpret_cast<uint4*>(cp) = make_uint4(w[0], w[1], w[2], w[3]);
            *reinterpret_cast<uint4*>(cp + 8) = make_uint4(w[4], w[5], w[6], w[7]);
          }
        } else {
          for (int i = 0; i < 16; ++i)
            if (nb + i < p.N) cp[i] = eh_from_float(v[i]);
        }
      }
}

template <int NCOLS>
__global__ void __launch_bounds__(256) tc_igemm_kernel(const TcGemmP p) {
  extern __shared__ unsigned char dyn_smem[];
  __shared__ __align__(8) uint64_t mma_done[TC_STAGES];
  __shared__ __align__(8) uint64_t acc_done;
  __shared__ uint32_t tmem_base_s;

  const int tid = threadIdx.x, warp = tid >> 5, lane = tid & 31;
  const int BN = p.BN;
  const uint32_t b_bytes = (uint32_t)BN * (TC_BK * 2);
  const uint32_t stage_bytes = TC_A_BYTES + b_bytes;
  const int NS = p.stages;
  const uint32_t smem0 = (smem_u32(dyn_smem) + 1023u) & ~1023u;
  const int m0 = blockIdx.x * TC_BM, n0 = blockIdx.y * BN;
  const int KB = (p.K + TC_BK - 1) / TC_BK;

  if (warp == 0) {
    asm volatile("tcgen05.alloc.cta_group::1.sync.aligned.shared::cta.b32 [%0], %1;\n" ::"r"(smem_u32(&tmem_base_s)), "n"(NCOLS) : "memory");
    asm volatile("tcgen05.relinquish_alloc_permit.cta_group::1.sync.aligned;\n" ::: "memory");
  }
  if (tid == 32) {
#pragma unroll
    for (int s = 0; s < TC_STAGES; ++s) mbar_init(&mma_done[s], 1);
    mbar_init(&acc_done, 1);
    asm volatile("fence.mbarrier_init.release.cluster;\n" ::: "memory");
  }
  tc_fence_before();
  __syncthreads();
  tc_fence_after();
  const uint32_t tmem = tmem_base_s;

  const int c = tid & 7, rbase = tid >> 3;
  const eh_t* a_ptr[4];
  int a_ih0[4], a_iw0[4];
  bool a_ok[4];
#pragma unroll
  for (int i = 0; i < 4; ++i) {
    const int m = m0 + rbase + 32 * i;
    a_ok[i] = m < p.M;
    a_ih0[i] = a_iw0[i] = 0;
    a_ptr[i] = p.A;
    if (a_ok[i]) {
      if (p.conv) {
        const int ow = m % p.OW;
        const int t = m / p.OW;
        const int oh = t % p.OH;
        const int n = t / p.OH;
        a_ptr[i] = p.A + (size_t)n * p.H * p.Wd * p.Cin;
        a_ih0[i] = oh * p.stride - p.pad_t;
        a_iw0[i] = ow * p.stride - p.pad_l;
      } else {
        a_ptr[i] = p.A + (size_t)m * p.lda;
      }
    }
  }
  const int nb_rows = (BN + 31) / 32;

  auto load_stage = [&](int kb, int stage) {
    const uint32_t sa = smem0 + (uint32_t)stage * stage_bytes;
    const uint32_t sb = sa + TC_A_BYTES;
    const int k = kb * TC_BK + c * 8;
    int tap = 0, ci = k, kh = 0, kw = 0;
    if (p.conv) {
      tap = k / p.Cin;
      ci = k - tap * p.Cin;
      kh = tap / p.KW;
      kw = tap - kh * p.KW;
    }
#pragma unroll
    for (int i = 0; i < 4; ++i) {
      const int row = rbase + 32 * i;
      const uint32_t dst = sa + (uint32_t)(row >> 3) * 1024u + (uint32_t)(row & 7) * 128u + (uint32_t)((c ^ (row & 7)) << 4);
      const eh_t* src = p.A;
      uint32_t bytes = 0;
      if (a_ok[i] && k < p.K) {
        if (p.conv) {
          const int ih = a_ih0[i] + kh, iw = a_iw0[i] + kw;
          if (ih >= 0 && ih < p.H && iw >= 0 && iw < p.Wd) {
            src = a_ptr[i] + ((size_t)ih * p.Wd + iw) * p.Cin + ci;
            bytes = 16;
          }
        } else {
          src = a_ptr[i] + k;
          bytes = 16;
        }
      }
      cp_async16(dst, src, bytes);
    }
    for (int j = 0; j < nb_rows; ++j) {
      const int row = rbase + 32 * j;
      if (row < BN) {
        const uint32_t dst = sb + (uint32_t)(row >> 3) * 1024u + (uint32_t)(row & 7) * 128u + (uint32_t)((c ^ (row & 7)) << 4);
        const int n = n0 + row;
        const bool ok = n < p.N && k < p.K;
        cp_async16(dst, ok ? p.W + (size_t)n * p.ldw + k : p.W, ok ? 16u : 0u);
      }
    }
  };

  for (int s = 0; s < NS - 1; ++s) {
    if (s < KB) load_stage(s, s);
    cp_async_commit();
  }
  const uint32_t idesc = make_idesc(BN);
  for (int kb = 0; kb < KB; ++kb) {
    if (NS == 3) cp_async_wait<1>(); else cp_async_wait<0>();
    asm volatile("fence.proxy.async.shared::cta;\n" ::: "memory");
    __syncthreads();
    const int stage = kb % NS;
    if (tid == 0) {
      tc_fence_after();
      const uint32_t sa = smem0 + (uint32_t)stage * stage_bytes;
      const uint64_t adesc = make_smem_desc(sa), bdesc = make_smem_desc(sa + TC_A_BYTES);
#pragma unroll
      for (int j = 0; j < TC_BK / 16; ++j)
        umma_f16(tmem, adesc + (uint64_t)(2 * j), bdesc + (uint64_t)(2 * j), idesc, (kb | j) ? 1u : 0u);
      umma_commit(&mma_done[stage]);
      if (kb == KB - 1) umma_commit(&acc_done);
    }
    const int nk = kb + NS - 1;
    if (nk < KB) {
      if (kb >= 1) mbar_wait(&mma_done[(kb - 1) % NS], (uint32_t)(((kb - 1) / NS) & 1));
      load_stage(nk, nk % NS);
    }
    cp_async_commit();
  }
  cp_async_wait<0>();
  mbar_wait(&acc_done, 0);
  tc_fence_after();

  {
    const int q = warp & 3;
    const int m = m0 + q * 32 + lane;
    const bool m_ok = m < p.M;
    for (int cc = (warp >> 2); cc * 16 < BN; cc += 2) {
      uint32_t r[16];
      tmem_ld16(tmem + ((uint32_t)(q * 32) << 16) + (uint32_t)(cc * 16), r);
      const int nb = n0 + cc * 16;
      if (m_ok && nb < p.N) epilogue_store16<false>(p, r, m, nb);
    }
  }
  tc_fence_before();
  __syncthreads();
  if (warp == 0) {
    asm volatile("tcgen05.dealloc.cta_group::1.sync.aligned.b32 %0, %1;\n" ::"r"(tmem), "n"(NCOLS) : "memory");
  }
}


constexpr int WS_STAGES = 4;
constexpr int WS_LAG = 2;
constexpr int WS_PROD_WARPS = 8;
constexpr int WS_EPI_WARPS = 8;
constexpr int WS_MMA_WARP = WS_PROD_WARPS + WS_EPI_WARPS;
constexpr int WS_TMA_WARP = WS_MMA_WARP + 1;
constexpr int WS_THREADS = (WS_TMA_WARP + 1) * 32;
constexpr int WS_PROD_THREADS = WS_PROD_WARPS * 32;
constexpr int WS_ROWS_PER_PASS = WS_PROD_THREADS / 8;
constexpr int WS_A_PASSES = TC_BM / WS_ROWS_PER_PASS;

template <int NCOLS, bool GELU>
__global__ void __launch_bounds__(WS_THREADS, NCOLS >= 256 ? 1 : 2) tc_igemm_ws_kernel(const TcGemmP p, const __grid_constant__ CUtensorMap tmA,
                                                                  const __grid_constant__ CUtensorMap tmW) {
  extern __shared__ unsigned char dyn_smem[];
  __shared__ __align__(8) uint64_t full_bar[WS_STAGES], empty_bar[WS_STAGES], acc_full[2], acc_empty[2];
  __shared__ uint32_t tmem_base_s;

  const int tid = threadIdx.x, warp = tid >> 5, lane = tid & 31;
  const int BN = p.BN;
  const uint32_t stage_bytes = TC_A_BYTES + (uint32_t)BN * (TC_BK * 2);
  const uint32_t smem0 = (smem_u32(dyn_smem) + 1023u) & ~1023u;
  const int KB = p.im2col ? p.KW * p.KW : (p.K + TC_BK - 1) / TC_BK;
  const int tiles_n = (p.N + BN - 1) / BN;
  const int tiles_m = (p.M + TC_BM - 1) / TC_BM;
  const int num_tiles = tiles_m * tiles_n;
  const bool gather = p.conv && !p.im2col;

  if (warp == WS_MMA_WARP) {
    asm volatile("tcgen05.alloc.cta_group::1.sync.aligned.shared::cta.b32 [%0], %1;\n" ::"r"(smem_u32(&tmem_base_s)), "n"(NCOLS) : "memory");
    asm volatile("tcgen05.relinquish_alloc_permit.cta_group::1.sync.aligned;\n" ::: "memory");
  }
  if (tid == 0) {
#pragma unroll
    for (int s = 0; s < WS_STAGES; ++s) { mbar_init(&full_bar[s], (gather ? WS_PROD_THREADS : 0) + 1); mbar_init(&empty_bar[s], 1); }
    mbar_init(&acc_full[0], 1); mbar_init(&acc_full[1], 1);
    const int epi_threads = (WS_EPI_WARPS + (gather ? 0 : WS_PROD_WARPS)) * 32;
    mbar_init(&acc_empty[0], epi_threads); mbar_init(&acc_empty[1], epi_threads);
    asm volatile("fence.mbarrier_init.release.cluster;\n" ::: "memory");
  }
  tc_fence_before();
  __syncthreads();
  tc_fence_after();
  const uint32_t tmem = tmem_base_s;

  if (gather ? warp < WS_PROD_WARPS : warp == WS_TMA_WARP) {
    const bool tma_thread = gather ? tid == 0 : lane == 0;
    const uint32_t tma_bytes = (uint32_t)BN * (TC_BK * 2) + (gather ? 0u : (uint32_t)TC_A_BYTES);
    if (!gather && !tma_thread) {
    } else {
    const int c = tid & 7, rbase = tid >> 3;
    int it = 0;
    for (int tile = blockIdx.x; tile < num_tiles; tile += gridDim.x) {
      const int m0 = (tile / tiles_n) * TC_BM, n0 = (tile % tiles_n) * BN;
      const eh_t* a_ptr[WS_A_PASSES];
      int a_ih0[WS_A_PASSES], a_iw0[WS_A_PASSES];
      bool a_ok[WS_A_PASSES];
      int bw = 0, bh = 0, bn = 0;
      if (p.im2col) {
        const int ow = m0 % p.OW, tq = m0 / p.OW;
        bw = ow * p.stride - p.pad_l;
        bh = (tq % p.OH) * p.stride - p.pad_t;
        bn = tq / p.OH;
      }
      if (gather) {
#pragma unroll
        for (int i = 0; i < WS_A_PASSES; ++i) {
          const int m = m0 + rbase + WS_ROWS_PER_PASS * i;
          a_ok[i] = m < p.M;
          a_ih0[i] = a_iw0[i] = 0;
          a_ptr[i] = p.A;
          if (a_ok[i]) {
            const int ow = m % p.OW;
            const int tq = m / p.OW;
            const int oh = tq % p.OH;
            const int n = tq / p.OH;
            a_ptr[i] = p.A + (size_t)n * p.H * p.Wd * p.Cin;
            a_ih0[i] = oh * p.stride - p.pad_t;
            a_iw0[i] = ow * p.stride - p.pad_l;
          }
        }
      }
      for (int kb = 0; kb < KB; ++kb, ++it) {
        const int stage = it % WS_STAGES;
        mbar_wait(&empty_bar[stage], (uint32_t)(((it / WS_STAGES) & 1) ^ 1));
        const uint32_t sa = smem0 + (uint32_t)stage * stage_bytes, sb = sa + TC_A_BYTES;
        if (tma_thread) {
          mbar_arrive_expect_tx(&full_bar[stage], tma_bytes);
          tma_load_2d(sb, &tmW, kb * TC_BK, n0, &full_bar[stage]);
          if (p.im2col) tma_load_im2col(sa, &tmA, 0, bw, bh, bn, (uint16_t)(kb % p.KW), (uint16_t)(kb / p.KW), &full_bar[stage]);
          else if (!p.conv) tma_load_2d(sa, &tmA, kb * TC_BK, m0, &full_bar[stage]);
        }
        if (gather) {
          const int k = kb * TC_BK + c * 8;
          const int tap = k / p.Cin;
          const int ci = k - tap * p.Cin;
          const int kh = tap / p.KW;
          const int kw = tap - kh * p.KW;
#pragma unroll
          for (int i = 0; i < WS_A_PASSES; ++i) {
            const int row = rbase + WS_ROWS_PER_PASS * i;
            const uint32_t dst = sa + (uint32_t)(row >> 3) * 1024u + (uint32_t)(row & 7) * 128u + (uint32_t)((c ^ (row & 7)) << 4);
            const eh_t* src = p.A;
            uint32_t bytes = 0;
            if (a_ok[i] && k < p.K) {
              const int ih = a_ih0[i] + kh, iw = a_iw0[i] + kw;
              if (ih >= 0 && ih < p.H && iw >= 0 && iw < p.Wd) {
                src = a_ptr[i] + ((size_t)ih * p.Wd + iw) * p.Cin + ci;
                bytes = 16;
              }
            }
            cp_async16(dst, src, bytes);
          }
          cp_async_commit();
          if (it >= WS_LAG) {
            cp_async_wait<WS_LAG>();
            asm volatile("fence.proxy.async.shared::cta;\n" ::: "memory");
            mbar_arrive(&full_bar[(it - WS_LAG) % WS_STAGES]);
          }
        }
      }
    }
    if (gather) {
      cp_async_wait<0>();
      asm volatile("fence.proxy.async.shared::cta;\n" ::: "memory");
      for (int j = (it >= WS_LAG ? it - WS_LAG : 0); j < it; ++j) mbar_arrive(&full_bar[j % WS_STAGES]);
    }
    }
  } else if (warp == WS_MMA_WARP) {
    if (lane == 0) {
      const uint32_t idesc = make_idesc(BN);
      int it = 0, ti = 0;
      for (int tile = blockIdx.x; tile < num_tiles; tile += gridDim.x, ++ti) {
        const int a = ti & 1;
        mbar_wait(&acc_empty[a], (uint32_t)(((ti >> 1) & 1) ^ 1));
        tc_fence_after();
        const uint32_t tacc = tmem + (uint32_t)(a * (NCOLS / 2));
        for (int kb = 0; kb < KB; ++kb, ++it) {
          const int stage = it % WS_STAGES;
          mbar_wait(&full_bar[stage], (uint32_t)((it / WS_STAGES) & 1));
          tc_fence_after();
          const uint32_t sa = smem0 + (uint32_t)stage * stage_bytes;
          const uint64_t adesc = make_smem_desc(sa), bdesc = make_smem_desc(sa + TC_A_BYTES);
#pragma unroll
          for (int j = 0; j < TC_BK / 16; ++j)
            umma_f16(tacc, adesc + (uint64_t)(2 * j), bdesc + (uint64_t)(2 * j), idesc, (kb | j) ? 1u : 0u);
          umma_commit(&empty_bar[stage]);
          if (kb == KB - 1) umma_commit(&acc_full[a]);
        }
      }
    }
  } else if (warp < WS_MMA_WARP) {
    const int q = warp & 3;
    const int nsub = (WS_EPI_WARPS + (gather ? 0 : WS_PROD_WARPS)) / 4;
    const int sub = (gather ? warp - WS_PROD_WARPS : warp) >> 2;
    int ti = 0;
    for (int tile = blockIdx.x; tile < num_tiles; tile += gridDim.x, ++ti) {
      const int a = ti & 1;
      const int m0 = (tile / tiles_n) * TC_BM, n0 = (tile % tiles_n) * BN;
      mbar_wait(&acc_full[a], (uint32_t)((ti >> 1) & 1));
      tc_fence_after();
      const int m = m0 + q * 32 + lane;
      const bool m_ok = m < p.M;
      const uint32_t tacc = tmem + (uint32_t)(a * (NCOLS / 2)) + ((uint32_t)(q * 32) << 16);
      for (int cc = sub; cc * 16 < BN; cc += nsub) {
        uint32_t r[16];
        tmem_ld16(tacc + (uint32_t)(cc * 16), r);
        const int nb = n0 + cc * 16;
        if (m_ok && nb < p.N) epilogue_store16<GELU>(p, r, m, nb);
      }
      tc_fence_before();
      mbar_arrive(&acc_empty[a]);
    }
  }
  tc_fence_before();
  __syncthreads();
  if (warp == WS_MMA_WARP) {
    asm volatile("tcgen05.dealloc.cta_group::1.sync.aligned.b32 %0, %1;\n" ::"r"(tmem), "n"(NCOLS) : "memory");
  }
}

static int tc_pick_bn(int N) {
  if (N <= 256) return (N + 15) / 16 * 16;
  for (int bn = 256; bn >= 128; bn -= 16)
    if (N % bn == 0) return bn;
  return 256;
}

template <int NCOLS>
static int tc_launch(const TcGemmP& p, cudaStream_t st) {
  const size_t smem = (size_t)p.stages * (TC_A_BYTES + (size_t)p.BN * TC_BK * 2) + 1024;
  static SmemOptIn opt;
  {
    cudaError_t e = opt.ensure(tc_igemm_kernel<NCOLS>, smem, true);
    if (e != cudaSuccess) return (int)e;
  }
  dim3 grid((p.M + TC_BM - 1) / TC_BM, (p.N + p.BN - 1) / p.BN);
  tc_igemm_kernel<NCOLS><<<grid, 256, smem, st>>>(p);
  return 0;
}

static PFN_cuTensorMapEncodeTiled_v12000 tensor_map_encoder() {
  static PFN_cuTensorMapEncodeTiled_v12000 fn = nullptr;
  if (!fn) {
    void* ptr = nullptr;
    cudaDriverEntryPointQueryResult qres;
    if (cudaGetDriverEntryPoint("cuTensorMapEncodeTiled", &ptr, cudaEnableDefault, &qres) == cudaSuccess &&
        qres == cudaDriverEntryPointSuccess)
      fn = reinterpret_cast<PFN_cuTensorMapEncodeTiled_v12000>(ptr);
  }
  return fn;
}

static int make_tmap_2d(CUtensorMap* tm, const void* base, long long rows, long long cols, long long ld, int box_rows) {
  PFN_cuTensorMapEncodeTiled_v12000 enc = tensor_map_encoder();
  if (!enc) return (int)cudaErrorNotSupported;
  cuuint64_t dims[2] = {(cuuint64_t)cols, (cuuint64_t)rows};
  cuuint64_t strides[1] = {(cuuint64_t)ld * 2};
  cuuint32_t box[2] = {(cuuint32_t)TC_BK, (cuuint32_t)box_rows};
  cuuint32_t estr[2] = {1, 1};
  CUresult r = enc(tm, (FRX_ENC_FP16 ? CU_TENSOR_MAP_DATA_TYPE_FLOAT16 : CU_TENSOR_MAP_DATA_TYPE_BFLOAT16), 2, const_cast<void*>(base), dims, strides, box, estr,
                   CU_TENSOR_MAP_INTERLEAVE_NONE, CU_TENSOR_MAP_SWIZZLE_128B, CU_TENSOR_MAP_L2_PROMOTION_L2_128B,
                   CU_TENSOR_MAP_FLOAT_OOB_FILL_NONE);
  return r == CUDA_SUCCESS ? 0 : (int)cudaErrorInvalidValue;
}

static PFN_cuTensorMapEncodeIm2col_v12000 im2col_map_encoder() {
  static PFN_cuTensorMapEncodeIm2col_v12000 fn = nullptr;
  if (!fn) {
    void* ptr = nullptr;
    cudaDriverEntryPointQueryResult qres;
    if (cudaGetDriverEntryPoint("cuTensorMapEncodeIm2col", &ptr, cudaEnableDefault, &qres) == cudaSuccess &&
        qres == cudaDriverEntryPointSuccess)
      fn = reinterpret_cast<PFN_cuTensorMapEncodeIm2col_v12000>(ptr);
  }
  return fn;
}

static int make_tmap_im2col(CUtensorMap* tm, const TcGemmP& p) {
  PFN_cuTensorMapEncodeIm2col_v12000 enc = im2col_map_encoder();
  if (!enc) return (int)cudaErrorNotSupported;
  const int B = p.M / (p.OH * p.OW), k = p.KW;
  const int pad_r = (p.OW - 1) * p.stride + k - p.Wd - p.pad_l, pad_b = (p.OH - 1) * p.stride + k - p.H - p.pad_t;
  cuuint64_t dims[4] = {(cuuint64_t)p.Cin, (cuuint64_t)p.Wd, (cuuint64_t)p.H, (cuuint64_t)B};
  cuuint64_t strides[3] = {(cuuint64_t)p.Cin * 2, (cuuint64_t)p.Wd * p.Cin * 2, (cuuint64_t)p.H * p.Wd * p.Cin * 2};
  int lower[2] = {-p.pad_l, -p.pad_t};
  int upper[2] = {pad_r - (k - 1), pad_b - (k - 1)};
  cuuint32_t estr[4] = {1, (cuuint32_t)p.stride, (cuuint32_t)p.stride, 1};
  CUresult r = enc(tm, (FRX_ENC_FP16 ? CU_TENSOR_MAP_DATA_TYPE_FLOAT16 : CU_TENSOR_MAP_DATA_TYPE_BFLOAT16), 4, const_cast<eh_t*>(p.A), dims, strides, lower, upper,
                   (cuuint32_t)TC_BK, (cuuint32_t)TC_BM, estr, CU_TENSOR_MAP_INTERLEAVE_NONE, CU_TENSOR_MAP_SWIZZLE_128B,
                   CU_TENSOR_MAP_L2_PROMOTION_L2_128B, CU_TENSOR_MAP_FLOAT_OOB_FILL_NONE);
  return r == CUDA_SUCCESS ? 0 : (int)cudaErrorInvalidValue;
}

template <int NCOLS>
static int tc_launch_ws(const TcGemmP& p_in, int num_sms, cudaStream_t st) {
  TcGemmP p = p_in;
  const size_t smem = (size_t)WS_STAGES * (TC_A_BYTES + (size_t)p.BN * TC_BK * 2) + 1024;
  static SmemOptIn opt, opt_gelu;
  {
    cudaError_t e = opt.ensure(tc_igemm_ws_kernel<NCOLS, false>, smem, true);
    if (e == cudaSuccess) e = opt_gelu.ensure(tc_igemm_ws_kernel<NCOLS, true>, smem, true);
    if (e != cudaSuccess) return (int)e;
  }
  const int tiles = ((p.M + TC_BM - 1) / TC_BM) * ((p.N + p.BN - 1) / p.BN);
  int per_sm = (int)((227 * 1024) / (smem + 2048));
  if (per_sm > 512 / NCOLS) per_sm = 512 / NCOLS;
  if (per_sm > 4) per_sm = 4;
  if (per_sm < 1) per_sm = 1;
  const int grid = tiles < num_sms * per_sm ? tiles : num_sms * per_sm;
  CUtensorMap tmA, tmW;
  int rc;
  p.im2col = 0;
  if (p.conv && p.Wpad && p.Cin <= TC_BK && p.M % (p.OH * p.OW) == 0 && make_tmap_im2col(&tmA, p) == 0) {
    p.im2col = 1;
    rc = make_tmap_2d(&tmW, p.Wpad, p.N, (long long)p.KW * p.KW * TC_BK, (long long)p.KW * p.KW * TC_BK, p.BN);
  } else {
    rc = make_tmap_2d(&tmW, p.W, p.N, p.K, p.ldw, p.BN);
    if (rc) return rc;
    if (!p.conv) rc = make_tmap_2d(&tmA, p.A, p.M, p.K, p.lda, TC_BM);
    else tmA = tmW;
  }
  if (rc) return rc;
  if (getenv("FRX_DEBUG"))
    fprintf(stderr, "[frx] tc gemm M=%d N=%d K=%d BN=%d conv=%d Cin=%d stride=%d -> %s, grid %d\n", p.M, p.N, p.K, p.BN, p.conv,
            p.Cin, p.stride, p.im2col ? "TMA im2col" : (p.conv ? "cp.async gather" : "TMA dense"), grid);
  if (p.act == ACT_GELU) tc_igemm_ws_kernel<NCOLS, true><<<grid, WS_THREADS, smem, st>>>(p, tmA, tmW);
  else tc_igemm_ws_kernel<NCOLS, false><<<grid, WS_THREADS, smem, st>>>(p, tmA, tmW);
  return 0;
}

int launch_tc_igemm_ws(TcGemmP p, int num_sms, cudaStream_t st) {
  if (p.BN == 0) {
    p.BN = tc_pick_bn(p.N);
    const int tiles_m = (p.M + TC_BM - 1) / TC_BM;
    while (p.BN > 64 && p.BN % 32 == 0 && p.N % (p.BN / 2) == 0 && tiles_m * ((p.N + p.BN - 1) / p.BN) < num_sms) p.BN /= 2;
  }
  if (p.BN <= 32) { p.BN = 32; return tc_launch_ws<64>(p, num_sms, st); }
  if (p.BN <= 64) return tc_launch_ws<128>(p, num_sms, st);
  if (p.BN <= 128) return tc_launch_ws<256>(p, num_sms, st);
  return tc_launch_ws<512>(p, num_sms, st);
}

int launch_tc_igemm(TcGemmP p, cudaStream_t st) {
  if (p.act == ACT_GELU) {
    int dev = 0, sms = 148;
    cudaGetDevice(&dev);
    cudaDeviceGetAttribute(&sms, cudaDevAttrMultiProcessorCount, dev);
    return launch_tc_igemm_ws(p, sms, st);
  }
  if (p.BN == 0) p.BN = tc_pick_bn(p.N);
  {
    const int kb = (p.K + TC_BK - 1) / TC_BK;
    const size_t stage = TC_A_BYTES + (size_t)p.BN * TC_BK * 2;
    p.stages = (kb > 3 && 3 * stage <= 72 * 1024) ? 3 : 2;
  }
  if (p.BN <= 32) { p.BN = 32; return tc_launch<32>(p, st); }
  if (p.BN <= 64) return tc_launch<64>(p, st);
  if (p.BN <= 128) return tc_launch<128>(p, st);
  return tc_launch<256>(p, st);
}

__global__ void __launch_bounds__(256) f32_to_h16_kernel(const float* __restrict__ in, eh_t* __restrict__ out, long long n) {
  long long i = ((long long)blockIdx.x * blockDim.x + threadIdx.x) * 4;
  if (i + 3 < n) {
    float4 v = __ldg(reinterpret_cast<const float4*>(in + i));
    *reinterpret_cast<uint2*>(out + i) = make_uint2(eh2_pack(v.x, v.y), eh2_pack(v.z, v.w));
  } else {
    for (; i < n; ++i) out[i] = eh_from_float(in[i]);
  }
}

void launch_f32_to_h16(const float* in, eh_t* out, long long n, cudaStream_t st) {
  f32_to_h16_kernel<<<(unsigned)((n / 4 + 256) / 256), 256, 0, st>>>(in, out, n);
}


__global__ void __launch_bounds__(256) h16_to_f32_kernel(const eh_t* __restrict__ in, float* __restrict__ out, long long n) {
  long long i = (long long)blockIdx.x * blockDim.x + threadIdx.x;
  if (i < n) out[i] = eh_to_float(in[i]);
}
void launch_h16_to_f32(const eh_t* in, float* out, long long n, cudaStream_t st) {
  h16_to_f32_kernel<<<(unsigned)((n + 255) / 256), 256, 0, st>>>(in, out, n);
}


__global__ void __launch_bounds__(256) pad_conv_weights_kernel(const eh_t* __restrict__ in, eh_t* __restrict__ out,
                                                               long long rows, int Cin) {
  long long i = (long long)blockIdx.x * blockDim.x + threadIdx.x;
  if (i >= rows * 64) return;
  const int ci = (int)(i & 63);
  out[i] = ci < Cin ? in[(i >> 6) * Cin + ci] : eh_from_float(0.f);
}
void launch_pad_conv_weights(const eh_t* in, eh_t* out, long long rows, int Cin, cudaStream_t st) {
  pad_conv_weights_kernel<<<(unsigned)((rows * 64 + 255) / 256), 256, 0, st>>>(in, out, rows, Cin);
}

}
```

p4-fr-sorry-math-but-love-you_b200/csrc/runtime.cu:

```cuda
#include <cmath>
#include <cstdarg>
#include <cstdio>
#include <cstring>
#include <map>
#include <string>
#include <vector>

#include "../../include/frx.h"
#include "kernels.h"
#include "runtime.h"

using namespace frx;

static int fail(frx_handle* h, const char* fmt, ...) {
  char buf[1024];
  va_list ap;
  va_start(ap, fmt);
  vsnprintf(buf, sizeof buf, fmt, ap);
  va_end(ap);
  if (h) h->err = buf;
  return 1;
}

#define CK(expr)                                                                          \
// ... 130 lines not shown
    {2, 6, 3, 2, 4, 128, 25}, {2, 9, 3, 1, 6, 160, 25}, {2, 15, 3, 2, 6, 256, 25}};

extern "C" const char* frx_version(void) { return "frx 0.1 sm_100a"; }

extern "C" const char* frx_last_error(const frx_handle* h) { return h ? h->err.c_str() : "null handle"; }

extern "C" int frx_create(const frx_config* cfg, frx_handle** out) {
  if (!cfg || !out) return 1;
  frx_handle* h = new frx_handle();
  h->cfg = *cfg;
  *out = h;
  int ndev = 0;
  cudaError_t e = cudaGetDeviceCount(&ndev);
  if (e != cudaSuccess || ndev == 0)
    return fail(h, "no CUDA device available (%s): frx has no CPU fallback", cudaGetErrorString(e));
  if (cfg->device < 0 || cfg->device >= ndev) return fail(h, "device %d out of range", cfg->device);
  ON_DEVICE(cfg->device);
  cudaDeviceProp prop;
  CK(cudaGetDeviceProperties(&prop, cfg->device));
  if (prop.major != 10) return fail(h, "device is sm_%d%d; frx is built for sm_100a (B200) only", prop.major, prop.minor);
  h->num_sms = prop.multiProcessorCount;
  if (cfg->network != FRX_NET_EFFICIENT_SATRN && cfg->network != FRX_NET_LITE_SATRN && cfg->network != FRX_NET_SWIN)
    return fail(h, "unknown network %d", cfg->network);
  if (cfg->network == FRX_NET_SWIN && (cfg->height != 384 || cfg->width != 384 || cfg->in_ch != 3 || cfg->enc_hidden != 1024))
    return fail(h, "SWIN is fixed to Swin-B/384: 384x384x3 input, 1024-wide memory (networks/SWIN.py:1028-1031)");
  if (cfg->dec_hidden % cfg->dec_heads || (cfg->dec_hidden / cfg->dec_heads != 32 && cfg->dec_hidden / cfg->dec_heads != 64))
    return fail(h, "decoder head_dim must be 32 or 64");
  if (cfg->dec_hidden > 512) return fail(h, "decoder hidden_dim > 512 not supported");
  if (cfg->max_batch <= 0 || cfg->max_steps <= 0) return fail(h, "max_batch/max_steps must be positive");
  return 0;
}

extern "C" void frx_destroy(frx_handle* h) {
  if (!h) return;
  DeviceGuard guard;
  guard.enter(h->cfg.device);
  frx_train_destroy(h);
  for (auto& kv : h->graphs) cudaGraphExecDestroy(kv.second.exec);
  for (void* p : h->allocs) cudaFree(p);
  for (auto& kv : h->taps) cudaFree(kv.second.data);
  if (h->ev[0]) for (int i = 0; i < 5; ++i) cudaEventDestroy(h->ev[i]);
  for (auto& sl : h->pipe) {
    if (sl.h2d) { cudaEventDestroy(sl.h2d); cudaEventDestroy(sl.enc); cudaEventDestroy(sl.done); cudaEventDestroy(sl.d2h); }
  }
  if (h->pipe_h2d) { cudaStreamDestroy(h->pipe_h2d); cudaStreamDestroy(h->pipe_d2h); cudaStreamDestroy(h->pipe_enc); }
  delete h;
}

extern "C" int frx_load_tensor(frx_handle* h, const char* name, const void* data, const int64_t* shape,
                               int32_t ndim, int32_t dtype) {
  if (!h || !name || !data) return fail(h, "frx_load_tensor: null argument");
  HostTensor t;
  size_t n = 1;
  for (int i = 0; i < ndim; ++i) { t.shape.push_back(shape[i]); n *= (size_t)shape[i]; }
  if (dtype == FRX_DTYPE_F32) {
    t.f.resize(n);
    CK(cudaMemcpy(t.f.data(), data, n * sizeof(float), cudaMemcpyDefault));
  } else if (dtype == FRX_DTYPE_I64) {
    std::vector<int64_t> tmp(n);
    CK(cudaMemcpy(tmp.data(), data, n * sizeof(int64_t), cudaMemcpyDefault));
    t.f.resize(n);
    for (size_t i = 0; i < n; ++i) t.f[i] = (float)tmp[i];
  } else {
    return fail(h, "frx_load_tensor('%s'): unsupported dtype %d", name, dtype);
  }
  h->raw[name] = std::move(t);
  h->finalized = false;
  return 0;
}

extern "C" int frx_set_option(frx_handle* h, const char* key, int64_t value) {
  if (!h || !key) return 1;
  ON_DEVICE(h->cfg.device);
  std::string k(key);
  if (k == "taps") h->opt_taps = value != 0;
  else if (k == "graphs") h->opt_graphs = value != 0;
  else if (k == "step16") h->opt_step16 = value != 0;
  else if (k == "pipe_enc") h->opt_pipe_enc = value != 0;
  else if (k == "timing") h->opt_timing = value != 0;
  else if (k == "cluster_images") {}
  else if (k == "dec_hpc") h->opt_dec_hpc = (value == 1 || value == 2) ? (int)value : 0;
  else if (k == "conv24") h->opt_conv24 = value != 0;
  else if (k == "enc_fp32") h->opt_enc_fp32 = value != 0;
  else if (k == "tc_ws") h->opt_tc_ws = value != 0;
  else if (k == "train_splitk") h->opt_train_splitk = value != 0;
  else if (k == "tc_im2col") h->opt_tc_im2col = value != 0;
  else if (k == "prof") {
    h->opt_prof = value != 0;
    if (h->opt_prof && !h->prof) { void* p; if (dev_alloc(h, &p, 16 * 8)) return 1; h->prof = (long long*)p; }
  }
  else if (k == "parts") {
    if (h->ws_ready && ((int)value & 3) != h->opt_parts)
      return fail(h, "option 'parts' cannot change after the first frx_finalize_weights (create a new handle)");
    h->opt_parts = (int)value & 3;
    h->finalized = false;
  }
  else return fail(h, "unknown option '%s'", key);
  return 0;
}

extern "C" int64_t frx_launch_count(const frx_handle* h) { return h ? h->launches : 0; }
extern "C" int64_t frx_device_bytes(const frx_handle* h) { return h ? h->device_bytes : 0; }

extern "C" int frx_read_prof(frx_handle* h, int64_t* out16) {
  if (!h || !out16 || !h->prof) return fail(h, "profiling not enabled (frx_set_option(h, \"prof\", 1))");
  ON_DEVICE(h->cfg.device);
  CK(cudaMemcpy(out16, h->prof, 16 * 8, cudaMemcpyDeviceToHost));
  return 0;
}

extern "C" int frx_last_timing(const frx_handle* h, float* ms4) {
  if (!h || !ms4) return 1;
  for (int i = 0; i < 4; ++i) ms4[i] = h->last_ms[i];
  return 0;
}

static int pack_trunk_efficientnet(frx_handle* h, ArenaBuilder& ab) {
  const frx_config& c = h->cfg;
  const std::string e = "encoder.shallow_cnn.";
  const HostTensor* w;
  if (need(h, e + "conv_stem.weight", {24, c.in_ch, 3, 3}, &w)) return 1;
  h->stem_w = ab.add(w->f.data(), w->f.size());
  if (fold_bn(h, ab, e + "bn1", 24, 1e-3f, nullptr, &h->stem_sc, &h->stem_sh)) return 1;
  int cin = 24;
  h->blocks.clear();
  for (int s = 0; s < 6; ++s) {
    for (int r = 0; r < kArch[s][1]; ++r) {
      BlockW b{};
      b.kind = kArch[s][0];
      b.k = kArch[s][2];
      b.stride = r == 0 ? kArch[s][3] : 1;
      b.cin = cin;
      b.cout = kArch[s][5];
      b.mid = cin * kArch[s][4];
      b.se_r = cin * kArch[s][6] / 100;
      b.residual = (b.cin == b.cout && b.stride == 1);
      std::string p = e + "eff_block." + std::to_string(s) + "." + std::to_string(r);
      b.name = "eff_block." + std::to_string(s) + "." + std::to_string(r);
      if (b.kind == 0) {
        if (pack_conv(h, ab, p + ".conv.weight", b.cout, b.cin, b.k, &b.w_a)) return 1;
        if (fold_bn(h, ab, p + ".bn1", b.cout, 1e-3f, nullptr, &b.sc_a, &b.sh_a)) return 1;
      } else if (b.kind == 1) {
        if (pack_conv(h, ab, p + ".conv_exp.weight", b.mid, b.cin, b.k, &b.w_a)) return 1;
        if (fold_bn(h, ab, p + ".bn1", b.mid, 1e-3f, nullptr, &b.sc_a, &b.sh_a)) return 1;
        if (pack_conv(h, ab, p + ".conv_pwl.weight", b.cout, b.mid, 1, &b.w_b)) return 1;
        if (fold_bn(h, ab, p + ".bn2", b.cout, 1e-3f, nullptr, &b.sc_b, &b.sh_b)) return 1;
      } else {
        if (pack_conv(h, ab, p + ".conv_pw.weight", b.mid, b.cin, 1, &b.w_a)) return 1;
        if (fold_bn(h, ab, p + ".bn1", b.mid, 1e-3f, nullptr, &b.sc_a, &b.sh_a)) return 1;
        if (pack_dw(h, ab, p + ".conv_dw.weight", b.mid, &b.w_dw)) return 1;
        if (fold_bn(h, ab, p + ".bn2", b.mid, 1e-3f, nullptr, &b.sc_dw, &b.sh_dw)) return 1;
        const HostTensor *w1, *b1, *w2, *b2;
        if (need(h, p + ".se.conv_reduce.weight", {b.se_r, b.mid, 1, 1}, &w1) ||
            need(h, p + ".se.conv_reduce.bias", {b.se_r}, &b1) ||
            need(h, p + ".se.conv_expand.weight", {b.mid, b.se_r, 1, 1}, &w2) ||
            need(h, p + ".se.conv_expand.bias", {b.mid}, &b2))
          return 1;
        b.se_w1 = ab.add(w1->f.data(), w1->f.size());
        b.se_b1 = ab.add(b1->f.data(), b1->f.size());
        b.se_w2 = ab.add(w2->f.data(), w2->f.size());
        b.se_w2t = ab.add(nullptr, w2->f.size());
        for (int cc = 0; cc < b.mid; ++cc)
          for (int rr = 0; rr < b.se_r; ++rr) ab.at(b.se_w2t)[(size_t)rr * b.mid + cc] = w2->f[(size_t)cc * b.se_r + rr];
        b.se_b2 = ab.add(b2->f.data(), b2->f.size());
        if (pack_conv(h, ab, p + ".conv_pwl.weight", b.cout, b.mid, 1, &b.w_b)) return 1;
        if (fold_bn(h, ab, p + ".bn3", b.cout, 1e-3f, nullptr, &b.sc_b, &b.sh_b)) return 1;
      }
      h->blocks.push_back(b);
      cin = b.cout;
    }
  }
  if (pack_conv(h, ab, e + "conv_last.weight", c.enc_hidden, 256, 1, &h->last_w)) return 1;
  if (fold_bn(h, ab, e + "bn2", c.enc_hidden, 1e-5f, nullptr, &h->last_sc, &h->last_sh)) return 1;
  return 0;
}

static int pack_trunk_lite(frx_handle* h, ArenaBuilder& ab) {
  const frx_config& c = h->cfg;
  const std::string e = "encoder.shallow_cnn.";
  int H = c.enc_hidden;
// ... 438 lines not shown
      cudaFree(h->arena);
      h->device_bytes -= (int64_t)h->arena_bytes;
      h->arena = nullptr;
    }
    void* p;
    if (dev_alloc(h, &p, bytes)) return 1;
    h->arena = (float*)p;
    h->arena_bytes = bytes;
  }
  CK(cudaMemcpy(h->arena, ab.host.data(), bytes, cudaMemcpyHostToDevice));

  if (!h->ws_ready) {
    const size_t B = c.max_batch;
    size_t act_max = 0, mid_max = 0;
    if (c.network == FRX_NET_EFFICIENT_SATRN) {
      int H = (c.height - 3) / 2 + 1, W = (c.width - 3) / 2 + 1;
      act_max = (size_t)H * W * 24;
      for (const BlockW& b : h->blocks) {
        int OH, OW, pl;
        same_pad(H, b.k, b.stride, &OH, &pl);
        same_pad(W, b.k, b.stride, &OW, &pl);
        size_t mid = b.kind == 1 ? (size_t)OH * OW * b.mid : (b.kind == 2 ? (size_t)H * W * b.mid : 0);
        if (mid > mid_max) mid_max = mid;
        H = OH; W = OW;
        if ((size_t)H * W * b.cout > act_max) act_max = (size_t)H * W * b.cout;
      }
    } else {
      act_max = (size_t)c.height * c.width * (c.enc_hidden / 2);
      mid_max = act_max;
    }
    size_t S = (size_t)h->feat_h * h->feat_w, C = c.enc_hidden;
    size_t enc_act = S * 3 * C;
    if (enc_act > mid_max) mid_max = enc_act;
    if (S * C > act_max) act_max = S * C;
    void* p;
    if (want_enc && c.network == FRX_NET_SWIN) {
      const size_t tok = 96 * 96;
      for (int i = 0; i < 2; ++i) { if (dev_alloc(h, &p, B * tok * 128 * 4)) return 1; h->sw_x[i] = (float*)p; }
      if (dev_alloc(h, &p, B * tok * 128 * 4)) return 1; h->sw_a = (float*)p;
      if (dev_alloc(h, &p, B * tok * 384 * 4)) return 1; h->sw_qkv = (float*)p;
      if (dev_alloc(h, &p, B * tok * 512 * 4)) return 1; h->sw_hid = (float*)p;
      if (c.precision == FRX_PREC_BF16) {
        if (dev_alloc(h, &p, B * tok * 128 * 2)) return 1; h->sw_ab = p;
        if (dev_alloc(h, &p, B * tok * 512 * 2)) return 1; h->sw_hidb = p;
      }
    } else if (want_enc) {
      for (int i = 0; i < 2; ++i) { if (dev_alloc(h, &p, B * act_max * 4)) return 1; h->act[i] = (float*)p; }
      for (int i = 0; i < 2; ++i) { if (dev_alloc(h, &p, B * mid_max * 4)) return 1; h->mid[i] = (float*)p; }
      if (dev_alloc(h, &p, B * 2048 * 4 * 2)) return 1;
      h->gate = (float*)p;
    }
    const size_t D = c.dec_hidden, F = c.dec_filter, L = c.dec_layers, T = c.max_steps, V = c.num_classes;
    if (want_dec) {
    if (dev_alloc(h, &p, L * B * T * D * 4)) return 1; h->kself = (float*)p;
    if (dev_alloc(h, &p, L * B * T * D * 4)) return 1; h->vself = (float*)p;
    if (dev_alloc(h, &p, B * S * L * 2 * D * 4)) return 1; h->cross = (float*)p;
    float** small[] = {&h->dx, &h->datt, &h->dpre1, &h->dpre2, &h->du, &h->dw, &h->dq2};
    for (float** q : small) { if (dev_alloc(h, &p, B * D * 4)) return 1; *q = (float*)p; }
    if (dev_alloc(h, &p, B * 3 * D * 4)) return 1; h->dqkv = (float*)p;
    if (dev_alloc(h, &p, B * F * 4)) return 1; h->dff = (float*)p;
    if (dev_alloc(h, &p, B * T * V * 4)) return 1; h->logits_int = (float*)p;
    if (dev_alloc(h, &p, B * T * 8)) return 1; h->tokens_int = (long long*)p;
    if (dev_alloc(h, &p, B * T * 8)) return 1; h->forced_int = (long long*)p;
    if (dev_alloc(h, &p, B * 4)) return 1; h->cur_tok = (int*)p;
    if (c.precision == FRX_PREC_BF16) {
      if (dev_alloc(h, &p, L * B * T * D * 2)) return 1; h->kself_bf = p;
      if (dev_alloc(h, &p, L * B * T * D * 2)) return 1; h->vself_bf = p;
      if (dev_alloc(h, &p, L * B * S * D * 2)) return 1; h->kcross_bf = p;
      if (dev_alloc(h, &p, L * B * S * D * 2)) return 1; h->vcross_bf = p;
      if (dev_alloc(h, &p, B * S * (size_t)c.dec_src * 2)) return 1; h->mem_bf = p;
    }
    }
    if (dev_alloc(h, &p, B * S * C * 4)) return 1; h->memory_int = (float*)p;
    if (dev_alloc(h, &p, (size_t)c.in_ch * c.height * c.width * B * 4)) return 1; h->images_int = (float*)p;
    for (int i = 0; i < 5; ++i) CK(cudaEventCreate(&h->ev[i]));
    h->ws_ready = true;
  }
  for (auto& kv : h->graphs) cudaGraphExecDestroy(kv.second.exec);
  h->graphs.clear();
  h->finalized = true;
  return 0;
}

static int tap(frx_handle* h, const std::string& name, const float* src, int B, int H, int W, int C,
               cudaStream_t st) {
  if (!h->opt_taps) return 0;
  Tap& t = h->taps[name];
  size_t n = (size_t)B * H * W * C;
  if (t.capacity < n) {
    if (t.data) cudaFree(t.data);
    CK(cudaMalloc((void**)&t.data, n * 4));
    t.capacity = n;
  }
  t.shape[0] = B; t.shape[1] = H; t.shape[2] = W; t.shape[3] = C;
  CK(cudaMemcpyAsync(t.data, src, n * 4, cudaMemcpyDeviceToDevice, st));
  return 0;
}

extern "C" int frx_read_tap(frx_handle* h, const char* name, float* out, int64_t capacity, int64_t* count,
                            int32_t* shape4, void* stream) {
  if (!h || !name) return 1;
  auto it = h->taps.find(name);
  if (it == h->taps.end()) return fail(h, "no tap named '%s' (enable with frx_set_option(h,\"taps\",1))", name);
  const Tap& t = it->second;
  int64_t n = (int64_t)t.shape[0] * t.shape[1] * t.shape[2] * t.shape[3];
  if (count) *count = n;
  if (shape4) for (int i = 0; i < 4; ++i) shape4[i] = t.shape[i];
  if (out) {
    if (capacity < n) return fail(h, "tap '%s' needs %lld floats", name, (long long)n);
    CK(cudaMemcpyAsync(out, t.data, n * 4, cudaMemcpyDeviceToDevice, (cudaStream_t)stream));
  }
  return 0;
}

static int tap_bf16(frx_handle* h, const std::string& name, const void* src, int B, int H, int W, int C, cudaStream_t st) {
  if (!h->opt_taps) return 0;
  Tap& t = h->taps[name];
  size_t n = (size_t)B * H * W * C;
  if (t.capacity < n) {
    if (t.data) cudaFree(t.data);
    CK(cudaMalloc((void**)&t.data, n * 4));
    t.capacity = n;
  }
  t.shape[0] = B; t.shape[1] = H; t.shape[2] = W; t.shape[3] = C;
  launch_h16_to_f32((const eh_t*)src, t.data, (long long)n, st);
  CKL();
  return 0;
}

static GemmP dense_gemm(const float* A, int M, int K, const float* W, int N, float* C, int ldc) {
  GemmP g{};
  g.A = A; g.W = W; g.C = C; g.M = M; g.N = N; g.K = K; g.lda = K; g.ldc = ldc; g.conv = 0; g.rows_per_img = 1;
  return g;
}

static GemmP conv_gemm(const float* A, int B, int H, int W, int Cin, const float* Wt, int Cout, int k,
                       int stride, float* C, int* OH, int* OW) {
  GemmP g{};
  int pt, pl;
  same_pad(H, k, stride, OH, &pt);
  same_pad(W, k, stride, OW, &pl);
  g.A = A; g.W = Wt; g.C = C;
  g.M = B * (*OH) * (*OW); g.N = Cout; g.K = k * k * Cin; g.lda = 0; g.ldc = Cout;
  g.conv = 1; g.H = H; g.Wd = W; g.Cin = Cin; g.OH = *OH; g.OW = *OW; g.KH = k; g.KW = k;
  g.stride = stride; g.pad_t = pt; g.pad_l = pl; g.rows_per_img = 1;
  return g;
}

static int run_trunk_efficientnet(frx_handle* h, const float* images, int B, float** out, cudaStream_t st) {
  const frx_config& c = h->cfg;
  const float* A = h->arena;
  int H = (c.height - 3) / 2 + 1, W = (c.width - 3) / 2 + 1;
  float* x = h->act[0];
  float* y = h->act[1];
  launch_stem_conv(images, A + h->stem_w, A + h->stem_sc, A + h->stem_sh, x, B, c.in_ch, c.height, c.width, H, W, 24, st);
  CKL();
  if (tap(h, "stem", x, B, H, W, 24, st)) return 1;
  for (const BlockW& b : h->blocks) {
    int OH, OW;
    if (b.kind == 0) {
      GemmP g = conv_gemm(x, B, H, W, b.cin, A + b.w_a, b.cout, b.k, b.stride, y, &OH, &OW);
      g.scale = A + b.sc_a; g.shift = A + b.sh_a; g.act = ACT_SILU;
      if (b.residual) { g.res = x; g.ldr = b.cout; }
      launch_igemm_f32(g, st); CKL();
    } else if (b.kind == 1) {
      GemmP g = conv_gemm(x, B, H, W, b.cin, A + b.w_a, b.mid, b.k, b.stride, h->mid[0], &OH, &OW);
// ... 25 lines not shown
    if (tap(h, b.name, x, B, H, W, b.cout, st)) return 1;
  }
  GemmP g = dense_gemm(x, B * H * W, 256, A + h->last_w, c.enc_hidden, y, c.enc_hidden);
  g.scale = A + h->last_sc; g.shift = A + h->last_sh; g.act = ACT_SILU;
  launch_igemm_f32(g, st); CKL();
  if (H != h->feat_h || W != h->feat_w) return fail(h, "trunk output %dx%d != expected %dx%d", H, W, h->feat_h, h->feat_w);
  *out = y;
  return 0;
}

static TcGemmP tc_dense(const void* A, int M, int K, const float* arena, size_t w_off, int N, void* C, int out_f32) {
  TcGemmP g{};
  g.A = (const eh_t*)A; g.W = (const eh_t*)(arena + w_off); g.C = C;
  g.M = M; g.N = N; g.K = K; g.lda = K; g.ldw = K; g.ldc = N; g.out_f32 = out_f32;
  return g;
}

static TcGemmP tc_conv(const void* A, int B, int H, int W, int Cin, const float* arena, size_t w_off, int Cout, int k,
                       int stride, void* C, int* OH, int* OW) {
  TcGemmP g{};
  int pt, pl;
  same_pad(H, k, stride, OH, &pt);
  same_pad(W, k, stride, OW, &pl);
  g.A = (const eh_t*)A; g.W = (const eh_t*)(arena + w_off); g.C = C;
  g.M = B * (*OH) * (*OW); g.N = Cout; g.K = k * k * Cin; g.ldw = g.K; g.ldc = Cout;
  g.conv = 1; g.H = H; g.Wd = W; g.Cin = Cin; g.OH = *OH; g.OW = *OW; g.KW = k; g.stride = stride; g.pad_t = pt; g.pad_l = pl;
  return g;
}

#define TCL(g)                                                                                         \
  do {                                                                                                 \
    int rc__ = h->opt_tc_ws ? launch_tc_igemm_ws(g, h->num_sms, st) : launch_tc_igemm(g, st);          \
    if (rc__) return fail(h, "tcgen05 GEMM configuration failed: %s", cudaGetErrorString((cudaError_t)rc__)); \
    CKL();                                                                                             \
  } while (0)

static int encoder_layers_16(frx_handle* h, float* tf, float* xf, eh_t* m0, eh_t* m1, int B, float* memory, cudaStream_t st) {
  typedef eh_t bf;
  const frx_config& c = h->cfg;
  const float* A = h->arena;
  const int fh = h->feat_h, fw = h->feat_w, S = fh * fw, C = c.enc_hidden, F = c.enc_filter, M = B * S;
  float* other = tf;
  for (int i = 0; i < c.enc_layers; ++i) {
    const EncLayerW& L = h->enc[i];
    launch_layernorm_bf16out(xf, nullptr, A + L.ln_g, A + L.ln_b, m0, M, C, 0, st); CKL();
    float* qkv = (float*)m1;
    TcGemmP g = tc_dense(m0, M, C, A, L.wb_qkv, 3 * C, qkv, 1);
    g.shift = A + L.b_qkv;
    TCL(g);
    if (!launch_enc_attn_mma_bf16(qkv, m0, B, S, C, c.enc_heads, st)) launch_enc_attn_bf16out(qkv, m0, B, S, C, c.enc_heads, st);
    CKL();
    float* proj = (float*)m1;
    TcGemmP go = tc_dense(m0, M, C, A, L.wb_o, C, proj, 1);
    go.shift = A + L.b_o;
    TCL(go);
    launch_layernorm_bf16out(proj, xf, A + L.ln_g, A + L.ln_b, m0, M, C, S, st); CKL();
    TcGemmP g0 = tc_dense(m0, M, C, A, L.wb_c0, F, m1, 0);
    g0.scale = A + L.sc_c0; g0.shift = A + L.sh_c0; g0.act = ACT_RELU;
    TCL(g0);
    launch_dwconv_bf16(m1, A + L.w_dw, A + L.sc_dw, A + L.sh_dw, m0, B, fh, fw, F, fh, fw, 1, 1, 1, ACT_RELU, st); CKL();
    float* dst = (i == c.enc_layers - 1) ? memory : other;
    TcGemmP g1 = tc_dense(m0, M, F, A, L.wb_c1, C, dst, 1);
    g1.scale = A + L.sc_c1; g1.shift = A + L.sh_c1; g1.act = ACT_RELU; g1.res = xf; g1.res_f32 = 1; g1.ldr = C;
    TCL(g1);
    if (tap(h, "enc_layer" + std::to_string(i), dst, B, fh, fw, C, st)) return 1;
    other = xf;
    xf = dst;
  }
  return 0;
}


static int encode_bf16(frx_handle* h, const float* images, int B, float* memory, cudaStream_t st) {
  const frx_config& c = h->cfg;
  const float* A = h->arena;
  typedef eh_t bf;
  int H = (c.height - 3) / 2 + 1, W = (c.width - 3) / 2 + 1;
  bf* x = (bf*)h->act[0];
  bf* y = (bf*)h->act[1];
  bf* m0 = (bf*)h->mid[0];
  bf* m1 = (bf*)h->mid[1];
  launch_stem_conv_bf16(images, A + h->stem_w, A + h->stem_sc, A + h->stem_sh, x, B, c.in_ch, c.height, c.width, H, W, 24, st);
  CKL();
  if (tap_bf16(h, "stem", x, B, H, W, 24, st)) return 1;
  for (const BlockW& b : h->blocks) {
    int OH, OW;
    if (b.kind == 0 && b.w_frag24 && h->opt_conv24) {
      OH = H; OW = W;
      launch_conv3x3_c24_bf16(x, A + b.w_frag24, A + b.sc_a, A + b.sh_a, y, B, H, W, b.residual ? 1 : 0, st);
      CKL();
    } else if (b.kind == 0) {
      TcGemmP g = tc_conv(x, B, H, W, b.cin, A, b.wb_a, b.cout, b.k, b.stride, y, &OH, &OW);
      if (b.wb_a_pad && h->opt_tc_im2col) g.Wpad = (const eh_t*)(A + b.wb_a_pad);
      g.scale = A + b.sc_a; g.shift = A + b.sh_a; g.act = ACT_SILU;
      if (b.residual) { g.res = x; g.ldr = b.cout; }
      TCL(g);
    } else if (b.kind == 1) {
      TcGemmP g = tc_conv(x, B, H, W, b.cin, A, b.wb_a, b.mid, b.k, b.stride, m0, &OH, &OW);
      if (b.wb_a_pad && h->opt_tc_im2col) g.Wpad = (const eh_t*)(A + b.wb_a_pad);
      g.scale = A + b.sc_a; g.shift = A + b.sh_a; g.act = ACT_SILU;
      TCL(g);
      TcGemmP g2 = tc_dense(m0, B * OH * OW, b.mid, A, b.wb_b, b.cout, y, 0);
      g2.scale = A + b.sc_b; g2.shift = A + b.sh_b;
      if (b.residual) { g2.res = x; g2.ldr = b.cout; }
      TCL(g2);
    } else {
      TcGemmP g = tc_dense(x, B * H * W, b.cin, A, b.wb_a, b.mid, m0, 0);
      g.scale = A + b.sc_a; g.shift = A + b.sh_a; g.act = ACT_SILU;
      TCL(g);
      int pt, pl;
      same_pad(H, b.k, b.stride, &OH, &pt);
      same_pad(W, b.k, b.stride, &OW, &pl);
      launch_mbconv_dw_se_bf16(m0, A + b.w_dw, A + b.sc_dw, A + b.sh_dw, m1, h->gate, h->gate + (size_t)B * 2048,
                               A + b.se_w1, A + b.se_b1, A + b.se_w2t, A + b.se_b2, B, H, W, b.mid, OH, OW, b.stride, pt, pl,
                               b.se_r, st);
      CKL(); h->launches += 2;
      TcGemmP g2 = tc_dense(m1, B * OH * OW, b.mid, A, b.wb_b, b.cout, y, 0);
      g2.scale = A + b.sc_b; g2.shift = A + b.sh_b;
      if (b.residual) { g2.res = x; g2.ldr = b.cout; }
      TCL(g2);
    }
    H = OH; W = OW;
    bf* t = x; x = y; y = t;
    if (tap_bf16(h, b.name, x, B, H, W, b.cout, st)) return 1;
  }
  if (H != h->feat_h || W != h->feat_w) return fail(h, "trunk output %dx%d != expected %dx%d", H, W, h->feat_h, h->feat_w);
  const int fh = h->feat_h, fw = h->feat_w, S = fh * fw, C = c.enc_hidden, F = c.enc_filter, M = B * S;
  float* tf = (float*)y;
  {
    TcGemmP g = tc_dense(x, M, 256, A, h->last_wb, C, tf, 1);
    g.scale = A + h->last_sc; g.shift = A + h->last_sh; g.act = ACT_SILU;
    TCL(g);
  }
  if (tap(h, "trunk", tf, B, fh, fw, C, st)) return 1;
  float* xf = (float*)x;
  launch_pe2d_f32(tf, A + h->pe_w0, A + h->pe_b0, A + h->pe_w1, A + h->pe_b1, A + h->pe_h, A + h->pe_w, xf, B, fh, fw, C, st);
  CKL();
  if (tap(h, "pe2d", xf, B, fh, fw, C, st)) return 1;
  return encoder_layers_16(h, tf, xf, m0, m1, B, memory, st);
}

static int encode_swin(frx_handle* h, const float* images, int B, float* memory, cudaStream_t st) {
  const float* A = h->arena;
  float* x = h->sw_x[0];
  float* y = h->sw_x[1];
  launch_swin_patch_embed(images, A + h->sw_pe_w, A + h->sw_pe_b, A + h->sw_pe_g, A + h->sw_pe_beta, A + h->sw_ape, x, B, 384,
                          96, 128, st);
  CKL();
  if (tap(h, "embed", x, B, 96, 96, 128, st)) return 1;
  size_t bi = 0;
  const int depths[4] = {2, 2, 18, 2};
  for (int i = 0; i < 4; ++i) {
    for (int j = 0; j < depths[i]; ++j, ++bi) {
      const SwinBlockW& b = h->sw_blocks[bi];
      const int M = B * b.res * b.res, C = b.dim;
      if (h->cfg.precision == FRX_PREC_BF16) {
        eh_t* ab16 = (eh_t*)h->sw_ab;
        launch_layernorm_bf16out(x, nullptr, A + b.n1_g, A + b.n1_b, ab16, M, C, 0, st); CKL();
        { TcGemmP g = tc_dense(ab16, M, C, A, b.qkv_wb, 3 * C, h->sw_qkv, 1); g.shift = A + b.qkv_b; TCL(g); }
        if (!launch_swin_window_attn_mma(h->sw_qkv, A + b.bias_table, ab16, B, b.res, C, b.heads, b.ws, b.shift, st)) {
          launch_swin_window_attn(h->sw_qkv, A + b.bias_table, h->sw_a, B, b.res, C, b.heads, b.ws, b.shift, st); CKL();
          launch_f32_to_h16(h->sw_a, ab16, (long long)M * C, st);
        }
        CKL();
        { TcGemmP g = tc_dense(ab16, M, C, A, b.proj_wb, C, y, 1); g.shift = A + b.proj_b; g.res = x; g.res_f32 = 1; g.ldr = C; TCL(g); }
        launch_layernorm_bf16out(y, nullptr, A + b.n2_g, A + b.n2_b, ab16, M, C, 0, st); CKL();
// ... 19 lines not shown
      launch_igemm_f32(g2, st); CKL();
      if (tap(h, "block" + std::to_string(i) + "." + std::to_string(j), x, B, b.res, b.res, C, st)) return 1;
    }
    if (i < 3) {
      const SwinMergeW& m = h->sw_merges[i];
      const int M2 = B * (m.res / 2) * (m.res / 2);
      launch_swin_patch_merge(x, h->sw_hid, B, m.res, m.dim, st); CKL();
      if (h->cfg.precision == FRX_PREC_BF16) {
        launch_layernorm_bf16out(h->sw_hid, nullptr, A + m.n_g, A + m.n_b, (eh_t*)h->sw_hidb, M2, 4 * m.dim, 0, st); CKL();
        TcGemmP g = tc_dense(h->sw_hidb, M2, 4 * m.dim, A, m.red_wb, 2 * m.dim, x, 1);
        TCL(g);
        if (tap(h, "merge" + std::to_string(i), x, B, m.res / 2, m.res / 2, 2 * m.dim, st)) return 1;
        continue;
      }
      launch_layernorm_f32(h->sw_hid, nullptr, A + m.n_g, A + m.n_b, h->sw_qkv, M2, 4 * m.dim, 0, st); CKL();
      GemmP g = dense_gemm(h->sw_qkv, M2, 4 * m.dim, A + m.red_w, 2 * m.dim, x, 2 * m.dim);
      launch_igemm_f32(g, st); CKL();
      if (tap(h, "merge" + std::to_string(i), x, B, m.res / 2, m.res / 2, 2 * m.dim, st)) return 1;
    }
  }
  launch_layernorm_f32(x, nullptr, A + h->sw_norm_g, A + h->sw_norm_b, memory, B * 144, 1024, 0, st); CKL();
  return 0;
}

static int run_trunk_lite(frx_handle* h, const float* images, int B, float** out, cudaStream_t st) {
  const frx_config& c = h->cfg;
  const float* A = h->arena;
  int H = c.height, W = c.width;
  float* x = h->act[0];
  float* y = h->act[1];
  if (c.precision == FRX_PREC_BF16 && !h->opt_enc_fp32 && h->lite[1].wb) {
    typedef eh_t bf;
    bf* xb = (bf*)h->act[0];
    bf* yb = (bf*)h->act[1];
    const LiteConvW& L0 = h->lite[0];
    launch_lite_conv0_pool_bf16(images, A + L0.w, A + L0.sc, A + L0.sh, yb, B, L0.cin, H, W, L0.cout, st); CKL();
    H /= 2; W /= 2;
    for (int i = 1; i < 4; ++i) {
      const LiteConvW& L = h->lite[i];
      int OH, OW;
      TcGemmP g = tc_conv(yb, B, H, W, L.cin, A, L.wb, L.cout, 3, 1, xb, &OH, &OW);
      g.scale = A + L.sc; g.shift = A + L.sh; g.act = ACT_RELU;
      TCL(g);
      const bool last = i == 3;
      float* f32_out = last ? h->act[1] + (size_t)B * (H / 2) * (W / 2) * L.cout : nullptr;
      launch_maxpool2_bf16(xb, yb, f32_out, B, H, W, L.cout, st); CKL();
      H /= 2; W /= 2;
      if (last) y = f32_out;
    }
    if (H != h->feat_h || W != h->feat_w) return fail(h, "trunk output %dx%d != expected %dx%d", H, W, h->feat_h, h->feat_w);
    if (tap(h, "lite_conv3", y, B, H, W, h->lite[3].cout, st)) return 1;
    *out = y;
    return 0;
  }
  for (int i = 0; i < 4; ++i) {
    const LiteConvW& L = h->lite[i];
    if (i == 0) {
      launch_direct_conv3x3(images, A + L.w, A + L.sc, A + L.sh, x, B, L.cin, H, W, H, W, L.cout, 1, 1, ACT_RELU, st);
      CKL();
    } else {
      int OH, OW;
      GemmP g = conv_gemm(y, B, H, W, L.cin, A + L.w, L.cout, 3, 1, x, &OH, &OW);
      g.scale = A + L.sc; g.shift = A + L.sh; g.act = ACT_RELU;
      launch_igemm_f32(g, st); CKL();
    }
    launch_maxpool2_f32(x, y, B, H, W, L.cout, st); CKL();
    H /= 2; W /= 2;
    if (tap(h, "lite_conv" + std::to_string(i), y, B, H, W, L.cout, st)) return 1;
  }
  if (H != h->feat_h || W != h->feat_w) return fail(h, "trunk output %dx%d != expected %dx%d", H, W, h->feat_h, h->feat_w);
  *out = y;
  return 0;
}

extern "C" int frx_encode(frx_handle* h, const float* images, int32_t B, float* memory, void* stream) {
  if (!h) return 1;
  if (!h->finalized) return fail(h, "frx_encode: weights not finalized");
  if (!(h->opt_parts & 1)) return fail(h, "frx_encode: handle was created without the encoder part");
  if (B <= 0 || B > h->cfg.max_batch) return fail(h, "frx_encode: batch %d outside (0, %d]", B, h->cfg.max_batch);
  const frx_config& c = h->cfg;
  cudaStream_t st = (cudaStream_t)stream;
  ON_DEVICE(c.device);
  if (c.network == FRX_NET_SWIN) return encode_swin(h, images, B, memory, st);
  if (c.precision == FRX_PREC_BF16 && !h->opt_enc_fp32 && c.network == FRX_NET_EFFICIENT_SATRN)
    return encode_bf16(h, images, B, memory, st);
  const float* A = h->arena;
  float* t = nullptr;
  if (c.network == FRX_NET_LITE_SATRN) {
    if (run_trunk_lite(h, images, B, &t, st)) return 1;
  } else if (run_trunk_efficientnet(h, images, B, &t, st)) {
    return 1;
  }
  const int fh = h->feat_h, fw = h->feat_w, S = fh * fw, C = c.enc_hidden, F = c.enc_filter;
  if (tap(h, "trunk", t, B, fh, fw, C, st)) return 1;
  float* x = (t == h->act[0]) ? h->act[1] : h->act[0];
  launch_pe2d_f32(t, A + h->pe_w0, A + h->pe_b0, A + h->pe_w1, A + h->pe_b1, A + h->pe_h, A + h->pe_w, x, B, fh, fw, C, st);
  CKL();
  if (tap(h, "pe2d", x, B, fh, fw, C, st)) return 1;
  if (c.network == FRX_NET_LITE_SATRN && c.precision == FRX_PREC_BF16 && !h->opt_enc_fp32 && h->enc[0].wb_qkv)
    return encoder_layers_16(h, t, x, (eh_t*)h->mid[0], (eh_t*)h->mid[1], B, memory, st);
  float* other = t;
  const int M = B * S;
  for (int i = 0; i < c.enc_layers; ++i) {
    const EncLayerW& L = h->enc[i];
    float* ln = h->mid[0];
    float* qkv = h->mid[1];
    launch_layernorm_f32(x, nullptr, A + L.ln_g, A + L.ln_b, ln, M, C, 0, st); CKL();
    GemmP g = dense_gemm(ln, M, C, A + L.w_qkv, 3 * C, qkv, 3 * C);
    g.shift = A + L.b_qkv;
    launch_igemm_f32(g, st); CKL();
    float* att = h->mid[0];
    launch_enc_attn_f32(qkv, att, B, S, C, c.enc_heads, st); CKL();
    float* proj = h->mid[1];
    GemmP go = dense_gemm(att, M, C, A + L.w_o, C, proj, C);
    go.shift = A + L.b_o;
    launch_igemm_f32(go, st); CKL();
    float* scr = h->mid[0];
    launch_layernorm_f32(proj, x, A + L.ln_g, A + L.ln_b, scr, M, C, S, st); CKL();
    float* c0 = h->mid[1];
    GemmP g0 = dense_gemm(scr, M, C, A + L.w_c0, F, c0, F);
    g0.scale = A + L.sc_c0; g0.shift = A + L.sh_c0; g0.act = ACT_RELU;
    launch_igemm_f32(g0, st); CKL();
    float* dwo = h->mid[0];
    DwP d{c0, A + L.w_dw, A + L.sc_dw, A + L.sh_dw, dwo, B, fh, fw, F, fh, fw, 1, 1, 1, ACT_RELU};
    launch_dwconv_f32(d, st); CKL();
    float* dst = (i == c.enc_layers - 1) ? memory : other;
    GemmP g1 = dense_gemm(dwo, M, F, A + L.w_c1, C, dst, C);
    g1.scale = A + L.sc_c1; g1.shift = A + L.sh_c1; g1.act = ACT_RELU; g1.res = x; g1.ldr = C;
    launch_igemm_f32(g1, st); CKL();
    if (tap(h, "enc_layer" + std::to_string(i), dst, B, fh, fw, C, st)) return 1;
    other = x;
    x = dst;
  }
  return 0;
}

static int run_cross_kv(frx_handle* h, const float* memory, int B, cudaStream_t st) {
  const frx_config& c = h->cfg;
  const int S = h->feat_h * h->feat_w;
  if (c.precision == FRX_PREC_BF16) {
    launch_f32_to_h16(memory, (eh_t*)h->mem_bf, (long long)B * S * c.dec_src, st); CKL();
    TcGemmP t = tc_dense(h->mem_bf, B * S, c.dec_src, h->arena, h->cross_wb, c.dec_layers * 2 * c.dec_hidden, h->cross, 1);
    t.shift = h->arena + h->b_cross;
    TCL(t);
    return 0;
  }
  GemmP g = dense_gemm(memory, B * S, c.dec_src, h->arena + h->w_cross, c.dec_layers * 2 * c.dec_hidden, h->cross,
                       c.dec_layers * 2 * c.dec_hidden);
  g.shift = h->arena + h->b_cross;
  launch_igemm_f32(g, st); CKL();
  return 0;
}

struct StepRows {
  const int* hist_len = nullptr;
  const int* slot = nullptr;
  const int* chain = nullptr;
};

static int run_decode_step(frx_handle* h, int B, int t, float* logits_dst, long long ld_logits, cudaStream_t st,
                           const StepRows& rows = StepRows()) {
  const frx_config& c = h->cfg;
  const float* A = h->arena;
  const int D = c.dec_hidden, F = c.dec_filter, L = c.dec_layers, V = c.num_classes, T = c.max_steps;
  const int S = h->feat_h * h->feat_w, HD = D / c.dec_heads;
  const float temp = sqrtf((float)D);
  auto base_gemm = [&](const float* Ain, int K, const float* Wt, const float* bias, int N) {
    DecGemmP p{};
// ... 106 lines not shown

struct ClusterStep {
  const int* hist_len = nullptr;
  const int* chain = nullptr;
  const int* slot = nullptr;
  const int* tok32 = nullptr;
  const long long* tok64 = nullptr;
};

static int cross_kv_to_bf16(frx_handle* h, int B, cudaStream_t st) {
  const frx_config& c = h->cfg;
  launch_cross_to_bf16(h->cross, (__nv_bfloat16*)h->kcross_bf, (__nv_bfloat16*)h->vcross_bf, B, h->feat_h * h->feat_w, c.dec_layers,
                       c.dec_hidden, c.dec_hidden / c.dec_heads, st);
  CKL();
  return 0;
}

static int decode_greedy_bf16(frx_handle* h, int B, int steps, float* logits, long long* tokens,
                              const long long* forced, cudaStream_t st, const ClusterStep* sm = nullptr, bool managed = false) {
  const frx_config& c = h->cfg;
  const float* A = h->arena;
  const int S = h->feat_h * h->feat_w, L = c.dec_layers, D = c.dec_hidden;
  if (steps > DEC_TMAX) return fail(h, "bf16 decode kernel supports at most %d steps", DEC_TMAX);
  if (!sm && cross_kv_to_bf16(h, B, st)) return 1;
  DecClusterP p{};
  if (sm) { p.hist_len = sm->hist_len; p.chain = sm->chain; p.slot = sm->slot; p.first_tok32 = sm->tok32; p.first_tok64 = sm->tok64; }
  if (managed) {
    p.sift_flags = h->sift_flags; p.sift_limit = h->sift_limit;
    p.sift_ids = SiftIds{h->sift_ids[0], h->sift_ids[1], h->sift_ids[2], h->sift_ids[3], h->sift_ids[4], h->sift_ids[5]};
  }
  p.B = B; p.steps = steps; p.T = c.max_steps; p.L = L; p.V = c.num_classes; p.S = S; p.sos = c.sos_id;
  const int clusters = (B + DEC_IMG - 1) / DEC_IMG;
  const int want_hpc = h->opt_dec_hpc ? h->opt_dec_hpc : (clusters > 15 ? 2 : 1);
  const bool p2 = D == 256 && want_hpc == 2 && !h->dpack2.empty();
  const std::vector<DecPackW>& dpk = p2 ? h->dpack2 : h->dpack;
  p.w_first = reinterpret_cast<const uint4*>(A + (p2 ? h->dpack2_first : h->dpack_first));
  p.b_first = A + h->fused[0].b;
  for (int l = 0; l < L; ++l) {
    const DecPackW& P = dpk[l];
    const DecLayerW& W = h->dec[l];
    DecClusterLayer& Q = p.layer[l];
    Q.w_o = reinterpret_cast<const uint4*>(A + P.w_o);   Q.w_q2 = reinterpret_cast<const uint4*>(A + P.w_q2);
    Q.w_o2 = reinterpret_cast<const uint4*>(A + P.w_o2); Q.w_f0 = reinterpret_cast<const uint4*>(A + P.w_f0);
    Q.w_f1 = reinterpret_cast<const uint4*>(A + P.w_f1); Q.w_next = reinterpret_cast<const uint4*>(A + P.w_next);
    Q.b_o = A + W.b_o; Q.b_q2 = A + W.b_q2; Q.b_o2 = A + W.b_o2; Q.b_f0 = A + W.b_f0; Q.b_f1 = A + W.b_f1;
    Q.b_next = A + h->fused[l + 1].b;
    Q.ln1_g = A + W.ln1_g; Q.ln1_b = A + W.ln1_b; Q.ln2_g = A + W.ln2_g; Q.ln2_b = A + W.ln2_b;
    Q.ln3_g = A + W.ln3_g; Q.ln3_b = A + W.ln3_b;
  }
  p.emb = A + h->emb; p.pe = A + h->pe1d;
  p.kself = (__nv_bfloat16*)h->kself_bf; p.vself = (__nv_bfloat16*)h->vself_bf;
  p.kcross = (const __nv_bfloat16*)h->kcross_bf; p.vcross = (const __nv_bfloat16*)h->vcross_bf;
  p.logits = logits; p.tokens = tokens; p.forced = forced;
  p.prof = h->opt_prof ? h->prof : nullptr;
  if (p.prof) CK(cudaMemsetAsync(h->prof, 0, 16 * 8, st));
  if (h->opt_timing) CK(cudaEventRecord(h->ev[3], st));
  int rc = D == 128 ? launch_dec_cluster_bf16_d128(p, st)
                    : D == 512 ? launch_dec_cluster_bf16_d512(p, st) : (p2 ? launch_dec_cluster_bf16_p2(p, st) : launch_dec_cluster_bf16(p, st));
  if (rc) return fail(h, "decode cluster kernel configuration failed: %s", cudaGetErrorString((cudaError_t)rc));
  CKL();
  if (h->opt_timing) CK(cudaEventRecord(h->ev[4], st));
  h->timed_kernel = h->opt_timing;
  return 0;
}

static int decode_greedy_impl(frx_handle* h, const float* memory, int B, int steps, float* logits,
                              int64_t* tokens, const int64_t* forced, cudaStream_t st, bool managed = false) {
  const frx_config& c = h->cfg;
  if (!h->finalized) return fail(h, "decode: weights not finalized");
  if (!(h->opt_parts & 2)) return fail(h, "decode: handle was created without the decoder part");
  if (B <= 0 || B > c.max_batch) return fail(h, "decode: batch %d outside (0, %d]", B, c.max_batch);
  if (steps <= 0 || steps > c.max_steps) return fail(h, "decode: steps %d outside (0, %d]", steps, c.max_steps);
  if (steps > 500) return fail(h, "decode: steps exceed the 1-D positional table (500)");
  ON_DEVICE(c.device);
  if (run_cross_kv(h, memory, B, st)) return 1;
  if (managed && !h->have_rules) return fail(h, "managed decode: frx_set_decoding_rules has not been called");
  if (managed && forced) return fail(h, "managed decode: forced tokens are not supported");
  const int mode = managed ? 2 : (forced ? 1 : 0);
  if (c.precision == FRX_PREC_BF16 && h->dec_cluster_ok && steps <= DEC_TMAX && (!managed || h->opt_step16))
    return decode_greedy_bf16(h, B, steps, logits, (long long*)(tokens ? tokens : (int64_t*)h->tokens_int),
                              (const long long*)forced, st, nullptr, managed);
  if (forced) CK(cudaMemcpyAsync(h->forced_int, forced, (size_t)B * steps * 8, cudaMemcpyDeviceToDevice, st));
  if (h->opt_graphs) {
    GraphKey key{B, steps, mode};
    auto it = h->graphs.find(key);
    if (it == h->graphs.end()) {
      cudaStream_t cs;
      CK(cudaStreamCreateWithFlags(&cs, cudaStreamNonBlocking));
      int64_t before = h->launches;
      CK(cudaStreamBeginCapture(cs, cudaStreamCaptureModeThreadLocal));
      int rc = run_greedy_loop(h, B, steps, mode, cs);
      cudaGraph_t graph = nullptr;
      cudaError_t e = cudaStreamEndCapture(cs, &graph);
      cudaStreamDestroy(cs);
      if (rc) { if (graph) cudaGraphDestroy(graph); return 1; }
      if (e != cudaSuccess) return fail(h, "graph capture failed: %s", cudaGetErrorString(e));
      GraphEntry ge{};
      ge.nodes = h->launches - before;
      h->launches = before;
      e = cudaGraphInstantiate(&ge.exec, graph, 0);
      cudaGraphDestroy(graph);
      if (e != cudaSuccess) return fail(h, "graph instantiate failed: %s", cudaGetErrorString(e));
      if (h->graphs.size() >= FRX_MAX_GRAPHS) {
        auto victim = h->graphs.begin();
        for (auto g = h->graphs.begin(); g != h->graphs.end(); ++g)
          if (g->second.last_use < victim->second.last_use) victim = g;
        CK(cudaStreamSynchronize(st));
        cudaGraphExecDestroy(victim->second.exec);
        h->graphs.erase(victim);
      }
      it = h->graphs.emplace(key, ge).first;
    }
    it->second.last_use = ++h->graph_clock;
    CK(cudaGraphLaunch(it->second.exec, st));
    h->launches += it->second.nodes;
  } else if (run_greedy_loop(h, B, steps, mode, st)) {
    return 1;
  }
  if (logits) CK(cudaMemcpyAsync(logits, h->logits_int, (size_t)B * steps * c.num_classes * 4, cudaMemcpyDeviceToDevice, st));
  if (tokens) CK(cudaMemcpyAsync(tokens, h->tokens_int, (size_t)B * steps * 8, cudaMemcpyDeviceToDevice, st));
  return 0;
}

extern "C" int frx_decode_greedy(frx_handle* h, const float* memory, int32_t B, int32_t steps, float* logits,
                                 int64_t* tokens, const int64_t* forced, void* stream) {
  if (!h) return 1;
  return decode_greedy_impl(h, memory, B, steps, logits, tokens, forced, (cudaStream_t)stream);
}

extern "C" int frx_set_decoding_rules(frx_handle* h, const int32_t* flags, const int32_t* limit, int32_t num_classes,
                                      const int32_t* ids6) {
  if (!h) return 1;
  const frx_config& c = h->cfg;
  if (num_classes != c.num_classes) return fail(h, "decoding rules: %d classes, the model has %d", num_classes, c.num_classes);
  for (int i = 0; i < 6; ++i)
    if (ids6[i] < 0 || ids6[i] >= num_classes) return fail(h, "decoding rules: special token id %d out of range", ids6[i]);
  ON_DEVICE(c.device);
  if (!h->sift_flags) {
    void* p;
    if (dev_alloc(h, &p, (size_t)num_classes * 4)) return 1; h->sift_flags = (int*)p;
    if (dev_alloc(h, &p, (size_t)num_classes * 4)) return 1; h->sift_limit = (int*)p;
    if (dev_alloc(h, &p, (size_t)c.max_batch * sizeof(int4))) return 1; h->sift_state = (int4*)p;
  }
  CK(cudaMemcpy(h->sift_flags, flags, (size_t)num_classes * 4, cudaMemcpyHostToDevice));
  CK(cudaMemcpy(h->sift_limit, limit, (size_t)num_classes * 4, cudaMemcpyHostToDevice));
  for (int i = 0; i < 6; ++i) h->sift_ids[i] = ids6[i];
  h->have_rules = true;
  for (auto it = h->graphs.begin(); it != h->graphs.end();) {
    if (std::get<2>(it->first) == 2) { cudaGraphExecDestroy(it->second.exec); it = h->graphs.erase(it); }
    else ++it;
  }
  return 0;
}

extern "C" int frx_decode_greedy_managed(frx_handle* h, const float* memory, int32_t B, int32_t steps, float* probs,
                                         int64_t* tokens, void* stream) {
  if (!h) return 1;
  return decode_greedy_impl(h, memory, B, steps, probs, tokens, nullptr, (cudaStream_t)stream, true);
}

extern "C" int frx_forward_greedy_managed(frx_handle* h, const float* images, int32_t B, int32_t steps, float* probs,
                                          int64_t* tokens, void* stream) {
  if (!h) return 1;
  if (frx_encode(h, images, B, h->memory_int, stream)) return 1;
  return decode_greedy_impl(h, h->memory_int, B, steps, probs, tokens, nullptr, (cudaStream_t)stream, true);
}

extern "C" int frx_forward_greedy(frx_handle* h, const float* images, int32_t B, int32_t steps, float* logits,
                                  int64_t* tokens, void* stream) {
  if (!h) return 1;
  cudaStream_t st = (cudaStream_t)stream;
  if (h->opt_timing) CK(cudaEventRecord(h->ev[0], st));
  if (frx_encode(h, images, B, h->memory_int, stream)) return 1;
  if (h->opt_timing) CK(cudaEventRecord(h->ev[1], st));
  if (decode_greedy_impl(h, h->memory_int, B, steps, logits, tokens, nullptr, st)) return 1;
  if (h->opt_timing) {
    CK(cudaEventRecord(h->ev[2], st));
    CK(cudaEventSynchronize(h->ev[2]));
    CK(cudaEventElapsedTime(&h->last_ms[0], h->ev[0], h->ev[1]));
    CK(cudaEventElapsedTime(&h->last_ms[1], h->ev[1], h->ev[2]));
    CK(cudaEventElapsedTime(&h->last_ms[2], h->ev[0], h->ev[2]));
    h->last_ms[3] = 0.f;
    if (h->timed_kernel) CK(cudaEventElapsedTime(&h->last_ms[3], h->ev[3], h->ev[4]));
  }
  return 0;
}

extern "C" int frx_forward_greedy_host(frx_handle* h, const float* images_host, int32_t B, int32_t steps,
                                       float* logits_host, int64_t* tokens_host, void* stream) {
  if (!h) return 1;
  if (!h->finalized) return fail(h, "forward: weights not finalized");
  const frx_config& c = h->cfg;
  if (B <= 0 || B > c.max_batch) return fail(h, "forward: batch %d outside (0, %d]", B, c.max_batch);
  cudaStream_t st = (cudaStream_t)stream;
  ON_DEVICE(c.device);
  size_t img_bytes = (size_t)B * c.in_ch * c.height * c.width * 4;
  CK(cudaMemcpyAsync(h->images_int, images_host, img_bytes, cudaMemcpyHostToDevice, st));
  if (frx_forward_greedy(h, h->images_int, B, steps,
// ... 320 lines not shown
```

p4-fr-sorry-math-but-love-you_b200/csrc/runtime.h:

```cpp
#pragma once
#include <cuda_runtime.h>
#include <stdint.h>

#include <map>
#include <string>
#include <tuple>
#include <vector>

#include "../../include/frx.h"

struct HostTensor {
  std::vector<int64_t> shape;
  std::vector<float> f;
};

struct BlockW {
  int kind;
  int cin, cout, k, stride, mid, se_r;
  bool residual;
  std::string name;
  size_t w_a, sc_a, sh_a;
  size_t w_dw, sc_dw, sh_dw;
  size_t se_w1, se_b1, se_w2, se_b2, se_w2t = 0;
  size_t w_b, sc_b, sh_b;
  size_t wb_a = 0, wb_b = 0;
  size_t wb_a_pad = 0;
  size_t w_frag24 = 0;
};
struct LiteConvW { int cin, cout; size_t w, sc, sh; size_t wb = 0; };
struct EncLayerW {
  size_t ln_g, ln_b, w_qkv, b_qkv, w_o, b_o;
  size_t w_c0, sc_c0, sh_c0, w_dw, sc_dw, sh_dw, w_c1, sc_c1, sh_c1;
  size_t wb_qkv = 0, wb_o = 0, wb_c0 = 0, wb_c1 = 0;
};
struct DecLayerW {
  size_t wt_o, b_o, wt_q2, b_q2, wt_o2, b_o2, wt_f0, b_f0, wt_f1, b_f1;
  size_t w_o, w_q2, w_o2, w_f0, w_f1, w_sqkv, b_sqkv;
  size_t wb_o = 0, wb_q2 = 0, wb_o2 = 0, wb_f0 = 0, wb_f1 = 0, wb_sqkv = 0;
  size_t ln1_g, ln1_b, ln2_g, ln2_b, ln3_g, ln3_b;
};
struct FusedW { size_t wt, b; int N; };
struct SwinBlockW {
  int dim, res, heads, ws, shift;
  size_t n1_g, n1_b, bias_table, qkv_w, qkv_b, proj_w, proj_b, n2_g, n2_b, fc1_w, fc1_b, fc2_w, fc2_b;
  size_t qkv_wb = 0, proj_wb = 0, fc1_wb = 0, fc2_wb = 0;
};
struct SwinMergeW { int dim, res; size_t red_w, n_g, n_b; size_t red_wb = 0; };
struct DecPackW { size_t w_o, w_q2, w_o2, w_f0, w_f1, w_next; };
struct Tap { float* data = nullptr; size_t capacity = 0; int shape[4] = {0, 0, 0, 0}; };
typedef std::tuple<int, int, int> GraphKey;
struct GraphEntry { cudaGraphExec_t exec; int64_t nodes; int64_t last_use = 0; };
constexpr size_t FRX_MAX_GRAPHS = 4;

struct BeamWs {
  double *hscore = nullptr, *nlogp = nullptr;
  int *hnode = nullptr, *nprev = nullptr, *ntok = nullptr, *nlen = nullptr, *nkv = nullptr, *chain = nullptr, *small = nullptr;
  float* logits = nullptr;
  int* host_flag = nullptr;
};
struct TfWs {
  float *x = nullptr, *y = nullptr, *z = nullptr, *qkv = nullptr, *ff = nullptr;
  unsigned char* mask = nullptr;
  void *xb = nullptr, *ffb = nullptr;
};

struct frx_handle {
  frx_config cfg{};
  std::string err;
  int num_sms = 0;
  std::map<std::string, HostTensor> raw;
  bool finalized = false, ws_ready = false;
  bool opt_taps = false, opt_graphs = true, opt_timing = false, opt_step16 = true, opt_pipe_enc = true;
  int* step_hist = nullptr;
  bool opt_prof = false;
  bool opt_tc_im2col = true;
  void* hook_wpad = nullptr; size_t hook_wpad_bytes = 0;
  bool opt_tc_ws = true;
  int opt_dec_hpc = 0;
  bool opt_conv24 = true;
  bool opt_enc_fp32 = false;
  long long* prof = nullptr;
  int opt_parts = 3;
  int feat_h = 0, feat_w = 0;
  std::vector<void*> allocs;
  int64_t device_bytes = 0, launches = 0;

  float* arena = nullptr;
  size_t arena_bytes = 0;
  size_t stem_w = 0, stem_sc = 0, stem_sh = 0, last_w = 0, last_sc = 0, last_sh = 0;
  std::vector<BlockW> blocks;
  LiteConvW lite[4]{};
  size_t pe_w0 = 0, pe_b0 = 0, pe_w1 = 0, pe_b1 = 0, pe_h = 0, pe_w = 0;
  std::vector<EncLayerW> enc;
  size_t sw_pe_w = 0, sw_pe_b = 0, sw_pe_g = 0, sw_pe_beta = 0, sw_ape = 0, sw_norm_g = 0, sw_norm_b = 0;
  std::vector<SwinBlockW> sw_blocks;
  std::vector<SwinMergeW> sw_merges;
  float *sw_x[2] = {nullptr, nullptr}, *sw_a = nullptr, *sw_qkv = nullptr, *sw_hid = nullptr;
  size_t emb = 0, pe1d = 0, gen_w = 0, gen_b = 0, w_cross = 0, b_cross = 0;
  size_t gen_wb = 0;
  size_t last_wb = 0, cross_wb = 0;
  std::vector<DecLayerW> dec;
  std::vector<FusedW> fused;
  std::vector<DecPackW> dpack;
  size_t dpack_first = 0;
  std::vector<DecPackW> dpack2;
  size_t dpack2_first = 0;

  float *act[2] = {nullptr, nullptr}, *mid[2] = {nullptr, nullptr}, *gate = nullptr;
  float *kself = nullptr, *vself = nullptr, *cross = nullptr;
  float *dx = nullptr, *dqkv = nullptr, *datt = nullptr, *dpre1 = nullptr, *dpre2 = nullptr, *du = nullptr,
        *dw = nullptr, *dq2 = nullptr, *dff = nullptr;
  float *logits_int = nullptr, *memory_int = nullptr, *images_int = nullptr;
  long long *tokens_int = nullptr, *forced_int = nullptr;
  int* cur_tok = nullptr;
  void* mem_bf = nullptr;
  void *kself_bf = nullptr, *vself_bf = nullptr, *kcross_bf = nullptr, *vcross_bf = nullptr;

  std::map<GraphKey, GraphEntry> graphs;
  int64_t graph_clock = 0;
  std::map<std::string, Tap> taps;
  cudaEvent_t ev[5] = {nullptr, nullptr, nullptr, nullptr, nullptr};
  struct PipeSlot {
    float *img = nullptr, *mem = nullptr;
    long long* tok = nullptr;
    cudaEvent_t h2d = nullptr, enc = nullptr, done = nullptr, d2h = nullptr;
    bool busy = false;
  };
  PipeSlot pipe[2];
  cudaStream_t pipe_h2d = nullptr, pipe_d2h = nullptr, pipe_enc = nullptr;
  float last_ms[4] = {0, 0, 0, 0};
  BeamWs beam;
  TfWs tf;
  int step_idx = 0, step_batch = 0;
  int *sift_flags = nullptr, *sift_limit = nullptr;
  int4* sift_state = nullptr;
  int sift_ids[6] = {0, 0, 0, 0, 0, 0};
  bool have_rules = false;
  bool timed_kernel = false;
  bool opt_train_splitk = true;
  bool dec_cluster_ok = false;
  void* train = nullptr;
  void *sw_ab = nullptr, *sw_hidb = nullptr;
};
```

Baseline: 12950.

## Add programmatic dependent launch to encoder kernels and capture encoder in CUDA graph

Adds griddepcontrol wait/launch_dependents to the encoder kernels and routes their launches through cudaLaunchKernelEx with programmatic stream serialization, so each kernel's prologue (TMEM alloc, weight TMA prefetch, smem weight loads) can overlap the tail of the previous kernel. The bf16 encoder is also captured into a CUDA graph keyed by batch, the PDL setting and the input/output pointers, and replayed on later calls to remove per-kernel launch overhead. The graph capture logic is factored into shared helpers and the graph cache limit is raised. Risks: stale graphs if buffers or options change beyond the invalidated ones, and PDL ordering bugs if any kernel reads predecessor output before its wait.

```diff
diff --git a/p4-fr-sorry-math-but-love-you_b200/csrc/common.cuh b/p4-fr-sorry-math-but-love-you_b200/csrc/common.cuh
--- a/p4-fr-sorry-math-but-love-you_b200/csrc/common.cuh
+++ b/p4-fr-sorry-math-but-love-you_b200/csrc/common.cuh
@@ -35,6 +35,34 @@
     return e;
   }
 };
+
+__device__ __forceinline__ void pdl_wait() { asm volatile("griddepcontrol.wait;\n" ::: "memory"); }
+__device__ __forceinline__ void pdl_launch_dependents() { asm volatile("griddepcontrol.launch_dependents;\n" ::: "memory"); }
+
+inline bool& pdl_enabled() {
+  static thread_local bool on = false;
+  return on;
+}
+struct PdlScope {
+  bool prev;
+  explicit PdlScope(bool on) : prev(pdl_enabled()) { pdl_enabled() = on; }
+  ~PdlScope() { pdl_enabled() = prev; }
+};
+
+template <typename... KArgs, typename... Args>
+inline void launch_k(void (*kernel)(KArgs...), dim3 grid, dim3 block, size_t smem, cudaStream_t st, Args... args) {
+  cudaLaunchConfig_t cfg = {};
+  cfg.gridDim = grid;
+  cfg.blockDim = block;
+  cfg.dynamicSmemBytes = smem;
+  cfg.stream = st;
+  cudaLaunchAttribute attr[1];
+  attr[0].id = cudaLaunchAttributeProgrammaticStreamSerialization;
+  attr[0].val.programmaticStreamSerializationAllowed = 1;
+  cfg.attrs = attr;
+  cfg.numAttrs = pdl_enabled() ? 1 : 0;
+  cudaLaunchKernelEx(&cfg, kernel, args...);
+}
 
 #ifndef FRX_ENC_FP16
 #define FRX_ENC_FP16 1
diff --git a/p4-fr-sorry-math-but-love-you_b200/csrc/kernels_bf16.cu b/p4-fr-sorry-math-but-love-you_b200/csrc/kernels_bf16.cu
--- a/p4-fr-sorry-math-but-love-you_b200/csrc/kernels_bf16.cu
+++ b/p4-fr-sorry-math-but-love-you_b200/csrc/kernels_bf16.cu
@@ -32,6 +32,8 @@
                                                              eh_t* __restrict__ out, int B, int Cin, int H, int W,
                                                              int OH, int OW, int Cout) {
   extern __shared__ float ws[];
+  pdl_launch_dependents();
+  pdl_wait();
   for (int i = threadIdx.x; i < Cout * Cin * 9; i += blockDim.x) ws[i] = w[i];
   float* ssc = ws + Cout * Cin * 9;
   float* ssh = ssc + Cout;
@@ -73,6 +75,8 @@
                                                                 eh_t* __restrict__ out, int B, int Cin, int H, int W,
                                                                 int OH, int OW) {
   extern __shared__ __align__(16) float ws[];
+  pdl_launch_dependents();
+  pdl_wait();
   const int taps = Cin * 9;
   for (int i = threadIdx.x; i < COUT * taps; i += blockDim.x) {
     const int co = i / taps, r = i - co * taps;
@@ -127,18 +131,22 @@
   if (Cout == 24) {
     const long long pixels = (long long)B * OH * OW;
     const int smem24 = ((24 * Cin * 9 + 2 * 24 + 3) & ~3) * sizeof(float) + 128 * 3 * 16;
-    stem_conv_px_bf16_kernel<24><<<(unsigned)((pixels + 127) / 128), 128, smem24, st>>>(in, w, scale, shift, out, B, Cin, H, W, OH, OW);
+    launch_k(stem_conv_px_bf16_kernel<24>, dim3((unsigned)((pixels + 127) / 128)), dim3(128), smem24, st, in, w, scale, shift, out, B,
+             Cin, H, W, OH, OW);
     return;
   }
   long long total = (long long)B * OH * OW * (Cout / 8);
   int smem = (Cout * Cin * 9 + 2 * Cout) * sizeof(float);
-  stem_conv_bf16_kernel<<<(unsigned)((total + 255) / 256), 256, smem, st>>>(in, w, scale, shift, out, B, Cin, H, W, OH, OW, Cout);
+  launch_k(stem_conv_bf16_kernel, dim3((unsigned)((total + 255) / 256)), dim3(256), smem, st, in, w, scale, shift, out, B, Cin, H, W,
+           OH, OW, Cout);
 }
 
 __global__ void __launch_bounds__(256) dwconv3x3_bf16_kernel(const eh_t* __restrict__ in, const float* __restrict__ w,
                                                              const float* __restrict__ scale, const float* __restrict__ shift,
                                                              eh_t* __restrict__ out, int B, int H, int W, int C, int OH,
                                                              int OW, int stride, int pad_t, int pad_l, int act) {
+  pdl_launch_dependents();
+  pdl_wait();
   const int C8 = C >> 3;
   long long total = (long long)B * OH * OW * C8;
   long long idx = (long long)blockIdx.x * blockDim.x + threadIdx.x;
@@ -177,8 +185,8 @@
                         eh_t* out, int B, int H, int W, int C, int OH, int OW, int stride, int pad_t,
                         int pad_l, int act, cudaStream_t st) {
   long long total = (long long)B * OH * OW * (C / 8);
-  dwconv3x3_bf16_kernel<<<(unsigned)((total + 255) / 256), 256, 0, st>>>(in, w, scale, shift, out, B, H, W, C, OH, OW,
-                                                                        stride, pad_t, pad_l, act);
+  launch_k(dwconv3x3_bf16_kernel, dim3((unsigned)((total + 255) / 256)), dim3(256), 0, st, in, w, scale, shift, out, B, H, W, C, OH,
+           OW, stride, pad_t, pad_l, act);
 }
 
 __global__ void __launch_bounds__(256) se_scale_bf16_kernel(eh_t* __restrict__ x, const float* __restrict__ w1,
@@ -343,6 +351,8 @@
       asm volatile("prefetch.global.L2 [%0];\n" ::"l"(se_w2 + line));
     }
   }
+  pdl_launch_dependents();
+  pdl_wait();
   uint4* tile = reinterpret_cast<uint4*>(dw_smem);
   float (*red)[CH + 1] = reinterpret_cast<float (*)[CH + 1]>(dw_smem + (size_t)H * W * G8 * 16);
   const int n = blockIdx.x, c0 = blockIdx.y * CH;
@@ -492,6 +502,8 @@
   extern __shared__ float sm[];
   float* mv = sm;
   float* red = sm + SE_IMGS * C;
+  pdl_launch_dependents();
+  pdl_wait();
   const int n0 = blockIdx.x * SE_IMGS;
   for (int i = threadIdx.x; i < SE_IMGS * C; i += blockDim.x) {
     const int im = i / C;
@@ -548,6 +560,8 @@
 
 __global__ void __launch_bounds__(256) se_apply_kernel(eh_t* __restrict__ x, const float* __restrict__ gate,
                                                        long long total8, int HW, int C) {
+  pdl_launch_dependents();
+  pdl_wait();
   long long i = (long long)blockIdx.x * blockDim.x + threadIdx.x;
   if (i >= total8) return;
   const int C8 = C >> 3;
@@ -576,14 +590,15 @@
     const size_t sm4 = (size_t)H * W * (CH / 8) * 16 + 16 * (CH + 1) * sizeof(float);
     static SmemOptIn opt4;
     opt4.ensure(dwconv4_se_mean_kernel<CH>, sm4);
-    dwconv4_se_mean_kernel<CH><<<dim3(B, (C + CH - 1) / CH), CH * 4, sm4, st>>>(in, w, scale, shift, out, mean, H, W, C, OH, OW,
-                                                                             stride, pad_t, pad_l, w1, w2, R * C);
+    launch_k(dwconv4_se_mean_kernel<CH>, dim3(B, (C + CH - 1) / CH), dim3(CH * 4), sm4, st, in, w, scale, shift, out, mean, H, W, C,
+             OH, OW, stride, pad_t, pad_l, w1, w2, R * C);
   } else {
     dwconv_se_mean_kernel<<<g, 256, smem, st>>>(in, w, scale, shift, out, mean, H, W, C, OH, OW, stride, pad_t, pad_l, w1, w2, R * C);
   }
-  se_fc_kernel<<<dim3((B + SE_IMGS - 1) / SE_IMGS, 2), 512, SE_IMGS * (C + R) * sizeof(float), st>>>(mean, w1, b1, w2, b2, gate, B, C, R);
+  launch_k(se_fc_kernel, dim3((B + SE_IMGS - 1) / SE_IMGS, 2), dim3(512), SE_IMGS * (C + R) * sizeof(float), st, mean, w1, b1, w2, b2,
+           gate, B, C, R);
   long long total8 = (long long)B * OH * OW * (C / 8);
-  se_apply_kernel<<<(unsigned)((total8 + 255) / 256), 256, 0, st>>>(out, gate, total8, OH * OW, C);
+  launch_k(se_apply_kernel, dim3((unsigned)((total8 + 255) / 256)), dim3(256), 0, st, out, gate, total8, OH * OW, C);
 }
 
 __device__ __forceinline__ uint32_t pack2(float lo, float hi) {
@@ -600,6 +615,8 @@
                                                              eh_t* __restrict__ out,
                                                              int D, int heads, float inv_temp) {
   constexpr int HD = 64, NT = S / 8;
+  pdl_launch_dependents();
+  pdl_wait();
   const int b = blockIdx.x / heads, hh = blockIdx.x % heads;
   const int warp = threadIdx.x >> 5, lane = threadIdx.x & 31, gid = lane >> 2, tig = lane & 3;
   const int ld = 3 * D;
@@ -674,8 +691,8 @@
 bool launch_enc_attn_mma_bf16(const float* qkv, eh_t* out, int B, int S, int D, int heads, cudaStream_t st) {
   if (D / heads != 64 || D % heads != 0) return false;
   const float inv_temp = 1.f / sqrtf((float)D);
-  if (S == 32) enc_attn_mma_kernel<32><<<B * heads, 64, 0, st>>>(qkv, out, D, heads, inv_temp);
-  else if (S == 128) enc_attn_mma_kernel<128><<<B * heads, 256, 0, st>>>(qkv, out, D, heads, inv_temp);
+  if (S == 32) launch_k(enc_attn_mma_kernel<32>, dim3(B * heads), dim3(64), 0, st, qkv, out, D, heads, inv_temp);
+  else if (S == 128) launch_k(enc_attn_mma_kernel<128>, dim3(B * heads), dim3(256), 0, st, qkv, out, D, heads, inv_temp);
   else return false;
   return true;
 }
@@ -692,6 +709,9 @@
   const int n = blockIdx.x / (tiles_x * tiles_y), t = blockIdx.x % (tiles_x * tiles_y);
   const int y0 = (t / tiles_x) * C24_TH, x0 = (t % tiles_x) * C24_TW;
   const eh_t* ip = in + (long long)n * H * W * C24;
+  pdl_launch_dependents();
+  for (int i = threadIdx.x; i < C24_KS * 3 * 32; i += 256) wsm[i] = __ldg(wfrag + i);
+  pdl_wait();
   for (int i = threadIdx.x; i < PH * PW * 3; i += 256) {
     const int pix = i / 3, ch = i - pix * 3;
     const int py = pix / PW, px = pix - py * PW;
@@ -700,7 +720,6 @@
     if (y >= 0 && y < H && x >= 0 && x < W) v = __ldg(reinterpret_cast<const uint4*>(ip + ((long long)y * W + x) * C24) + ch);
     reinterpret_cast<uint4*>(halo)[i] = v;
   }
-  for (int i = threadIdx.x; i < C24_KS * 3 * 32; i += 256) wsm[i] = __ldg(wfrag + i);
   __syncthreads();
   const int warp = threadIdx.x >> 5, lane = threadIdx.x & 31, gid = lane >> 2, tig = lane & 3;
   float acc[2][3][4];
@@ -767,7 +786,8 @@
 void launch_conv3x3_c24_bf16(const eh_t* in, const void* wfrag, const float* scale, const float* shift,
                              eh_t* out, int B, int H, int W, int add_res, cudaStream_t st) {
   const int tiles = ((W + C24_TW - 1) / C24_TW) * ((H + C24_TH - 1) / C24_TH);
-  conv3x3_c24_mma_kernel<<<B * tiles, 256, 0, st>>>(in, reinterpret_cast<const uint2*>(wfrag), scale, shift, out, H, W, add_res);
+  launch_k(conv3x3_c24_mma_kernel, dim3(B * tiles), dim3(256), 0, st, in, reinterpret_cast<const uint2*>(wfrag), scale, shift, out, H,
+           W, add_res);
 }
 
 __global__ void __launch_bounds__(256) lite_conv0_pool_bf16_kernel(const float* __restrict__ in, const float* __restrict__ w,
diff --git a/p4-fr-sorry-math-but-love-you_b200/csrc/kernels_f32.cu b/p4-fr-sorry-math-but-love-you_b200/csrc/kernels_f32.cu
--- a/p4-fr-sorry-math-but-love-you_b200/csrc/kernels_f32.cu
+++ b/p4-fr-sorry-math-but-love-you_b200/csrc/kernels_f32.cu
@@ -394,6 +394,8 @@
   float* mean = sm;
   float* hid = sm + C;
   float* g = hid + C / 2;
+  pdl_launch_dependents();
+  pdl_wait();
   const int S = h * w, n = blockIdx.x;
   const float* xp = x + (long long)n * S * C;
   const float inv = 1.f / (float)S;
@@ -432,7 +434,7 @@
                      const float* peh, const float* pew, float* out, int B, int h, int w, int C,
                      cudaStream_t st) {
   int smem = (C + C / 2 + 2 * C) * sizeof(float);
-  pe2d_f32_kernel<<<B, 1024, smem, st>>>(x, w0, b0, w1, b1, peh, pew, out, h, w, C);
+  launch_k(pe2d_f32_kernel, dim3(B), dim3(1024), smem, st, x, w0, b0, w1, b1, peh, pew, out, h, w, C);
 }
 
 __device__ __forceinline__ void store_as(float* p, float v) { *p = v; }
@@ -445,6 +447,8 @@
                                                             const float* __restrict__ beta,
                                                             OutT* __restrict__ out, int M, int C,
                                                             int scramble_S) {
+  pdl_launch_dependents();
+  pdl_wait();
   const int warp = threadIdx.x >> 5, lane = threadIdx.x & 31;
   const int m = blockIdx.x * 8 + warp;
   if (m >= M) return;
@@ -492,6 +496,8 @@
                                                             const float* __restrict__ beta,
                                                             OutT* __restrict__ out, int M, int C,
                                                             int scramble_S) {
+  pdl_launch_dependents();
+  pdl_wait();
   const int warp = threadIdx.x >> 5, lane = threadIdx.x & 31;
   const int m = blockIdx.x * 8 + warp;
   if (m >= M) return;
@@ -532,15 +538,15 @@
   const dim3 g((M + 7) / 8);
   const int per = C / 32;
   if (per <= 4 && per * 32 == C) {
-    if (per == 4) layernorm_f32_kernel<OutT, 4><<<g, 256, 0, st>>>(x, res, gamma, beta, out, M, C, scramble_S);
-    else if (per == 2) layernorm_f32_kernel<OutT, 2><<<g, 256, 0, st>>>(x, res, gamma, beta, out, M, C, scramble_S);
-    else if (per == 1) layernorm_f32_kernel<OutT, 1><<<g, 256, 0, st>>>(x, res, gamma, beta, out, M, C, scramble_S);
-    else layernorm_f32_kernel<OutT, 3><<<g, 256, 0, st>>>(x, res, gamma, beta, out, M, C, scramble_S);
-  } else if (per == 8) layernorm_f32_kernel<OutT, 8><<<g, 256, 0, st>>>(x, res, gamma, beta, out, M, C, scramble_S);
-  else if (per == 16) layernorm_f32_kernel<OutT, 16><<<g, 256, 0, st>>>(x, res, gamma, beta, out, M, C, scramble_S);
-  else if (per == 32) layernorm_f32_kernel<OutT, 32><<<g, 256, 0, st>>>(x, res, gamma, beta, out, M, C, scramble_S);
-  else if (per == 64) layernorm_f32_kernel<OutT, 64><<<g, 256, 0, st>>>(x, res, gamma, beta, out, M, C, scramble_S);
-  else layernorm_f32_generic_kernel<OutT><<<g, 256, 0, st>>>(x, res, gamma, beta, out, M, C, scramble_S);
+    if (per == 4) launch_k(layernorm_f32_kernel<OutT, 4>, g, dim3(256), 0, st, x, res, gamma, beta, out, M, C, scramble_S);
+    else if (per == 2) launch_k(layernorm_f32_kernel<OutT, 2>, g, dim3(256), 0, st, x, res, gamma, beta, out, M, C, scramble_S);
+    else if (per == 1) launch_k(layernorm_f32_kernel<OutT, 1>, g, dim3(256), 0, st, x, res, gamma, beta, out, M, C, scramble_S);
+    else launch_k(layernorm_f32_kernel<OutT, 3>, g, dim3(256), 0, st, x, res, gamma, beta, out, M, C, scramble_S);
+  } else if (per == 8) launch_k(layernorm_f32_kernel<OutT, 8>, g, dim3(256), 0, st, x, res, gamma, beta, out, M, C, scramble_S);
+  else if (per == 16) launch_k(layernorm_f32_kernel<OutT, 16>, g, dim3(256), 0, st, x, res, gamma, beta, out, M, C, scramble_S);
+  else if (per == 32) launch_k(layernorm_f32_kernel<OutT, 32>, g, dim3(256), 0, st, x, res, gamma, beta, out, M, C, scramble_S);
+  else if (per == 64) launch_k(layernorm_f32_kernel<OutT, 64>, g, dim3(256), 0, st, x, res, gamma, beta, out, M, C, scramble_S);
+  else launch_k(layernorm_f32_generic_kernel<OutT>, g, dim3(256), 0, st, x, res, gamma, beta, out, M, C, scramble_S);
 }
 
 void launch_layernorm_f32(const float* x, const float* res, const float* gamma, const float* beta,
@@ -553,6 +559,8 @@
                                                                       const float* __restrict__ beta,
                                                                       eh_t* __restrict__ out, int S, int C) {
   extern __shared__ eh_t ln_tile[];
+  pdl_launch_dependents();
+  pdl_wait();
   const int b = blockIdx.x, warp = threadIdx.x >> 5, lane = threadIdx.x & 31;
   const int per = C / 32, LD = S + 2;
   for (int qd = warp; qd < S; qd += 8) {
@@ -596,8 +604,7 @@
   static SmemOptIn scr_opt;
   if (scramble_S > 0 && C <= 512 && C % 32 == 0 && M % scramble_S == 0 && scr_smem <= 160 * 1024 &&
       scr_opt.ensure(layernorm_scramble_bf16_kernel, scr_smem) == cudaSuccess) {
-    layernorm_scramble_bf16_kernel<<<M / scramble_S, 256, scr_smem, st>>>(x, res, gamma, beta, out,
-                                                                                               scramble_S, C);
+    launch_k(layernorm_scramble_bf16_kernel, dim3(M / scramble_S), dim3(256), scr_smem, st, x, res, gamma, beta, out, scramble_S, C);
     return;
   }
   layernorm_launch<eh_t>(x, res, gamma, beta, out, M, C, scramble_S, st);
diff --git a/p4-fr-sorry-math-but-love-you_b200/csrc/kernels_tc.cu b/p4-fr-sorry-math-but-love-you_b200/csrc/kernels_tc.cu
--- a/p4-fr-sorry-math-but-love-you_b200/csrc/kernels_tc.cu
+++ b/p4-fr-sorry-math-but-love-you_b200/csrc/kernels_tc.cu
@@ -281,6 +281,8 @@
   __syncthreads();
   tc_fence_after();
   const uint32_t tmem = tmem_base_s;
+  pdl_launch_dependents();
+  pdl_wait();
 
   const int c = tid & 7, rbase = tid >> 3;
   const eh_t* a_ptr[4];
@@ -444,10 +446,22 @@
   __syncthreads();
   tc_fence_after();
   const uint32_t tmem = tmem_base_s;
+  pdl_launch_dependents();
+
+  const bool tma_thread = gather ? tid == 0 : (warp == WS_TMA_WARP && lane == 0);
+  const uint32_t tma_bytes = (uint32_t)BN * (TC_BK * 2) + (gather ? 0u : (uint32_t)TC_A_BYTES);
+  int w_early = 0;
+  if (tma_thread && (int)blockIdx.x < num_tiles) {
+    const int n0 = ((int)blockIdx.x % tiles_n) * BN;
+    w_early = KB < WS_STAGES ? KB : WS_STAGES;
+    for (int kb = 0; kb < w_early; ++kb) {
+      mbar_arrive_expect_tx(&full_bar[kb], tma_bytes);
+      tma_load_2d(smem0 + (uint32_t)kb * stage_bytes + TC_A_BYTES, &tmW, kb * TC_BK, n0, &full_bar[kb]);
+    }
+  }
+  pdl_wait();
 
   if (gather ? warp < WS_PROD_WARPS : warp == WS_TMA_WARP) {
-    const bool tma_thread = gather ? tid == 0 : lane == 0;
-    const uint32_t tma_bytes = (uint32_t)BN * (TC_BK * 2) + (gather ? 0u : (uint32_t)TC_A_BYTES);
     if (!gather && !tma_thread) {
     } else {
     const int c = tid & 7, rbase = tid >> 3;
@@ -487,8 +501,10 @@
         mbar_wait(&empty_bar[stage], (uint32_t)(((it / WS_STAGES) & 1) ^ 1));
         const uint32_t sa = smem0 + (uint32_t)stage * stage_bytes, sb = sa + TC_A_BYTES;
         if (tma_thread) {
-          mbar_arrive_expect_tx(&full_bar[stage], tma_bytes);
-          tma_load_2d(sb, &tmW, kb * TC_BK, n0, &full_bar[stage]);
+          if (it >= w_early) {
+            mbar_arrive_expect_tx(&full_bar[stage], tma_bytes);
+            tma_load_2d(sb, &tmW, kb * TC_BK, n0, &full_bar[stage]);
+          }
           if (p.im2col) tma_load_im2col(sa, &tmA, 0, bw, bh, bn, (uint16_t)(kb % p.KW), (uint16_t)(kb / p.KW), &full_bar[stage]);
           else if (!p.conv) tma_load_2d(sa, &tmA, kb * TC_BK, m0, &full_bar[stage]);
         }
@@ -597,7 +613,7 @@
     if (e != cudaSuccess) return (int)e;
   }
   dim3 grid((p.M + TC_BM - 1) / TC_BM, (p.N + p.BN - 1) / p.BN);
-  tc_igemm_kernel<NCOLS><<<grid, 256, smem, st>>>(p);
+  launch_k(tc_igemm_kernel<NCOLS>, grid, dim3(256), smem, st, p);
   return 0;
 }
 
@@ -686,8 +702,8 @@
   if (getenv("FRX_DEBUG"))
     fprintf(stderr, "[frx] tc gemm M=%d N=%d K=%d BN=%d conv=%d Cin=%d stride=%d -> %s, grid %d\n", p.M, p.N, p.K, p.BN, p.conv,
             p.Cin, p.stride, p.im2col ? "TMA im2col" : (p.conv ? "cp.async gather" : "TMA dense"), grid);
-  if (p.act == ACT_GELU) tc_igemm_ws_kernel<NCOLS, true><<<grid, WS_THREADS, smem, st>>>(p, tmA, tmW);
-  else tc_igemm_ws_kernel<NCOLS, false><<<grid, WS_THREADS, smem, st>>>(p, tmA, tmW);
+  if (p.act == ACT_GELU) launch_k(tc_igemm_ws_kernel<NCOLS, true>, dim3(grid), dim3(WS_THREADS), smem, st, p, tmA, tmW);
+  else launch_k(tc_igemm_ws_kernel<NCOLS, false>, dim3(grid), dim3(WS_THREADS), smem, st, p, tmA, tmW);
   return 0;
 }
 
@@ -723,6 +739,8 @@
 }
 
 __global__ void __launch_bounds__(256) f32_to_h16_kernel(const float* __restrict__ in, eh_t* __restrict__ out, long long n) {
+  pdl_launch_dependents();
+  pdl_wait();
   long long i = ((long long)blockIdx.x * blockDim.x + threadIdx.x) * 4;
   if (i + 3 < n) {
     float4 v = __ldg(reinterpret_cast<const float4*>(in + i));
@@ -733,7 +751,7 @@
 }
 
 void launch_f32_to_h16(const float* in, eh_t* out, long long n, cudaStream_t st) {
-  f32_to_h16_kernel<<<(unsigned)((n / 4 + 256) / 256), 256, 0, st>>>(in, out, n);
+  launch_k(f32_to_h16_kernel, dim3((unsigned)((n / 4 + 256) / 256)), dim3(256), 0, st, in, out, n);
 }
 
 
diff --git a/p4-fr-sorry-math-but-love-you_b200/csrc/runtime.cu b/p4-fr-sorry-math-but-love-you_b200/csrc/runtime.cu
--- a/p4-fr-sorry-math-but-love-you_b200/csrc/runtime.cu
+++ b/p4-fr-sorry-math-but-love-you_b200/csrc/runtime.cu
@@ -236,6 +236,8 @@
   else if (k == "dec_hpc") h->opt_dec_hpc = (value == 1 || value == 2) ? (int)value : 0;
   else if (k == "conv24") h->opt_conv24 = value != 0;
   else if (k == "enc_fp32") h->opt_enc_fp32 = value != 0;
+  else if (k == "pdl") h->opt_pdl = value != 0;
+  else if (k == "enc_graph") h->opt_enc_graph = value != 0;
   else if (k == "tc_ws") h->opt_tc_ws = value != 0;
   else if (k == "train_splitk") h->opt_train_splitk = value != 0;
   else if (k == "tc_im2col") h->opt_tc_im2col = value != 0;
@@ -250,6 +252,12 @@
     h->finalized = false;
   }
   else return fail(h, "unknown option '%s'", key);
+  if (k == "conv24" || k == "tc_ws" || k == "tc_im2col") {
+    for (auto it = h->graphs.begin(); it != h->graphs.end();) {
+      if (std::get<2>(it->first) == FRX_GRAPH_ENCODER) { cudaGraphExecDestroy(it->second.exec); it = h->graphs.erase(it); }
+      else ++it;
+    }
+  }
   return 0;
 }
 
@@ -854,6 +862,51 @@
   return 0;
 }
 
+static GraphEntry* find_graph(frx_handle* h, const GraphKey& key) {
+  auto it = h->graphs.find(key);
+  return it == h->graphs.end() ? nullptr : &it->second;
+}
+
+template <class Run>
+static GraphEntry* capture_graph(frx_handle* h, const GraphKey& key, cudaStream_t st, Run run) {
+  cudaStream_t cs;
+  cudaError_t e = cudaStreamCreateWithFlags(&cs, cudaStreamNonBlocking);
+  if (e != cudaSuccess) { fail(h, "cudaStreamCreate failed: %s", cudaGetErrorString(e)); return nullptr; }
+  const int64_t before = h->launches;
+  e = cudaStreamBeginCapture(cs, cudaStreamCaptureModeThreadLocal);
+  if (e != cudaSuccess) { cudaStreamDestroy(cs); fail(h, "graph capture failed: %s", cudaGetErrorString(e)); return nullptr; }
+  const int rc = run(cs);
+  cudaGraph_t graph = nullptr;
+  e = cudaStreamEndCapture(cs, &graph);
+  cudaStreamDestroy(cs);
+  GraphEntry ge{};
+  ge.nodes = h->launches - before;
+  h->launches = before;
+  if (rc) { if (graph) cudaGraphDestroy(graph); return nullptr; }
+  if (e != cudaSuccess) { fail(h, "graph capture failed: %s", cudaGetErrorString(e)); return nullptr; }
+  e = cudaGraphInstantiate(&ge.exec, graph, 0);
+  cudaGraphDestroy(graph);
+  if (e != cudaSuccess) { fail(h, "graph instantiate failed: %s", cudaGetErrorString(e)); return nullptr; }
+  if (h->graphs.size() >= FRX_MAX_GRAPHS) {
+    auto victim = h->graphs.begin();
+    for (auto g = h->graphs.begin(); g != h->graphs.end(); ++g)
+      if (g->second.last_use < victim->second.last_use) victim = g;
+    e = cudaStreamSynchronize(st);
+    if (e != cudaSuccess) { cudaGraphExecDestroy(ge.exec); fail(h, "cudaStreamSynchronize failed: %s", cudaGetErrorString(e)); return nullptr; }
+    cudaGraphExecDestroy(victim->second.exec);
+    h->graphs.erase(victim);
+  }
+  ge.last_use = ++h->graph_clock;
+  return &h->graphs.emplace(key, ge).first->second;
+}
+
+static int launch_graph(frx_handle* h, GraphEntry* ge, cudaStream_t st) {
+  ge->last_use = ++h->graph_clock;
+  CK(cudaGraphLaunch(ge->exec, st));
+  h->launches += ge->nodes;
+  return 0;
+}
+
 static int tap(frx_handle* h, const std::string& name, const float* src, int B, int H, int W, int C,
                cudaStream_t st) {
   if (!h->opt_taps) return 0;
@@ -1045,6 +1098,7 @@
   bf* m1 = (bf*)h->mid[1];
   launch_stem_conv_bf16(images, A + h->stem_w, A + h->stem_sc, A + h->stem_sh, x, B, c.in_ch, c.height, c.width, H, W, 24, st);
   CKL();
+  PdlScope pdl(h->opt_pdl);
   if (tap_bf16(h, "stem", x, B, H, W, 24, st)) return 1;
   for (const BlockW& b : h->blocks) {
     int OH, OW;
@@ -1230,8 +1284,13 @@
   cudaStream_t st = (cudaStream_t)stream;
   ON_DEVICE(c.device);
   if (c.network == FRX_NET_SWIN) return encode_swin(h, images, B, memory, st);
-  if (c.precision == FRX_PREC_BF16 && !h->opt_enc_fp32 && c.network == FRX_NET_EFFICIENT_SATRN)
-    return encode_bf16(h, images, B, memory, st);
+  if (c.precision == FRX_PREC_BF16 && !h->opt_enc_fp32 && c.network == FRX_NET_EFFICIENT_SATRN) {
+    if (!h->opt_enc_graph || h->opt_taps) return encode_bf16(h, images, B, memory, st);
+    const GraphKey key{B, h->opt_pdl ? 1 : 0, FRX_GRAPH_ENCODER, images, memory};
+    if (GraphEntry* ge = find_graph(h, key)) return launch_graph(h, ge, st);
+    if (encode_bf16(h, images, B, memory, st)) return 1;
+    return capture_graph(h, key, st, [&](cudaStream_t cs) { return encode_bf16(h, images, B, memory, cs); }) ? 0 : 1;
+  }
   const float* A = h->arena;
   float* t = nullptr;
   if (c.network == FRX_NET_LITE_SATRN) {
@@ -1504,38 +1563,11 @@
                               (const long long*)forced, st, nullptr, managed);
   if (forced) CK(cudaMemcpyAsync(h->forced_int, forced, (size_t)B * steps * 8, cudaMemcpyDeviceToDevice, st));
   if (h->opt_graphs) {
-    GraphKey key{B, steps, mode};
-    auto it = h->graphs.find(key);
-    if (it == h->graphs.end()) {
-      cudaStream_t cs;
-      CK(cudaStreamCreateWithFlags(&cs, cudaStreamNonBlocking));
-      int64_t before = h->launches;
-      CK(cudaStreamBeginCapture(cs, cudaStreamCaptureModeThreadLocal));
-      int rc = run_greedy_loop(h, B, steps, mode, cs);
-      cudaGraph_t graph = nullptr;
-      cudaError_t e = cudaStreamEndCapture(cs, &graph);
-      cudaStreamDestroy(cs);
-      if (rc) { if (graph) cudaGraphDestroy(graph); return 1; }
-      if (e != cudaSuccess) return fail(h, "graph capture failed: %s", cudaGetErrorString(e));
-      GraphEntry ge{};
-      ge.nodes = h->launches - before;
-      h->launches = before;
-      e = cudaGraphInstantiate(&ge.exec, graph, 0);
-      cudaGraphDestroy(graph);
-      if (e != cudaSuccess) return fail(h, "graph instantiate failed: %s", cudaGetErrorString(e));
-      if (h->graphs.size() >= FRX_MAX_GRAPHS) {
-        auto victim = h->graphs.begin();
-        for (auto g = h->graphs.begin(); g != h->graphs.end(); ++g)
-          if (g->second.last_use < victim->second.last_use) victim = g;
-        CK(cudaStreamSynchronize(st));
-        cudaGraphExecDestroy(victim->second.exec);
-        h->graphs.erase(victim);
-      }
-      it = h->graphs.emplace(key, ge).first;
-    }
-    it->second.last_use = ++h->graph_clock;
-    CK(cudaGraphLaunch(it->second.exec, st));
-    h->launches += it->second.nodes;
+    const GraphKey key{B, steps, mode, nullptr, nullptr};
+    GraphEntry* ge = find_graph(h, key);
+    if (!ge && !(ge = capture_graph(h, key, st, [&](cudaStream_t cs) { return run_greedy_loop(h, B, steps, mode, cs); })))
+      return 1;
+    if (launch_graph(h, ge, st)) return 1;
   } else if (run_greedy_loop(h, B, steps, mode, st)) {
     return 1;
   }
diff --git a/p4-fr-sorry-math-but-love-you_b200/csrc/runtime.h b/p4-fr-sorry-math-but-love-you_b200/csrc/runtime.h
--- a/p4-fr-sorry-math-but-love-you_b200/csrc/runtime.h
+++ b/p4-fr-sorry-math-but-love-you_b200/csrc/runtime.h
@@ -48,9 +48,10 @@
 struct SwinMergeW { int dim, res; size_t red_w, n_g, n_b; size_t red_wb = 0; };
 struct DecPackW { size_t w_o, w_q2, w_o2, w_f0, w_f1, w_next; };
 struct Tap { float* data = nullptr; size_t capacity = 0; int shape[4] = {0, 0, 0, 0}; };
-typedef std::tuple<int, int, int> GraphKey;
+typedef std::tuple<int, int, int, const void*, const void*> GraphKey;
+constexpr int FRX_GRAPH_ENCODER = 3;
 struct GraphEntry { cudaGraphExec_t exec; int64_t nodes; int64_t last_use = 0; };
-constexpr size_t FRX_MAX_GRAPHS = 4;
+constexpr size_t FRX_MAX_GRAPHS = 8;
 
 struct BeamWs {
   double *hscore = nullptr, *nlogp = nullptr;
@@ -79,6 +80,8 @@
   int opt_dec_hpc = 0;
   bool opt_conv24 = true;
   bool opt_enc_fp32 = false;
+  bool opt_pdl = true;
+  bool opt_enc_graph = true;
   long long* prof = nullptr;
   int opt_parts = 3;
   int feat_h = 0, feat_w = 0;
```

Measured after the change: 13180 (median of 6 runs). 1.8% higher.
